# ChenFengYe/motion-latent-diffusion

Measured on NVIDIA H100. Metric: motions/sec @ 50-step DDIM text-to-motion, batch 256, higher is better.
Workload: dtype f16x2-split (fp32-equivalent, fp32 accumulate)

## Files before the change

mld_b200/csrc/debug.cu:

```cuda
#include "engine.h"

#include <string.h>

#include "gemm_tc.h"
#include "misc_kernels.cuh"

extern "C" int mldb_profile_op(mldb_handle* h, const char* op, int32_t B, int32_t S_ctx, int32_t iters,
                               float* avg_ms_out) {
  TRY(check_ready(h, false));
  DeviceGuard guard(h->device);
  if (!op || !avg_ms_out || iters <= 0) FAIL(MLDB_ERR_INVALID, "bad argument");
  const mldb_config& c = h->cfg;
  if (c.num_layers == 0 || c.arch != MLDB_ARCH_TRANS_ENC) FAIL(MLDB_ERR_UNSUPPORTED, "needs the trans_enc denoiser");
  const bool cfg_on = c.guidance_scale > 1.0f;
  Plan* p = nullptr;
  TRY(enc_plan(h, PLAN_REVERSE, B, cfg_on ? 2 * B : B, S_ctx, &p));
  cudaStream_t st = h->cap_stream;
  StackWs& ws = p->ws;
  const EncW& w = h->den.enc[0];
  const int d = ws.d;
  SeqInfo si;
  auto run = [&]() -> int {
    if (!strcmp(op, "qkv")) {
      GemmArgs g; g.a1 = ws.x0; g.K1 = d; g.M = ws.M; g.w = w.in_proj; g.out = ws.qkv; op_gemm(h, g, st);
    } else if (!strcmp(op, "attn")) {
      AttnArgs a; a.q = ws.qkv; a.Lq = ws.L; a.kv = ws.qkv; a.k_col0 = d; a.v_col0 = 2 * d; a.Lk = ws.L;
      a.nseq = ws.nseq; a.heads = c.num_heads; a.hd = d / c.num_heads; a.out = ws.att; op_attn(h, a, st);
    } else if (!strcmp(op, "outproj_ln")) {
      out_proj_ln(h, w.out_proj, w.n1, ws.att, ws.x0, ws.x1, ws.M, d, ws.cf32, st);
    } else if (!strcmp(op, "ffn1")) {
      GemmArgs g; g.a1 = ws.x1; g.K1 = d; g.M = ws.M; g.w = w.l1; g.act = ACT_GELU; g.out = ws.h; op_gemm(h, g, st);
    } else if (!strcmp(op, "ffn2_ln")) {
      GemmArgs g; g.a1 = ws.h; g.K1 = ws.ff; g.M = ws.M; g.w = w.l2;
      LnArgs l; l.res = ws.x1; l.gamma = w.n2.g; l.beta = w.n2.b; l.M = ws.M; l.d = d; l.out = ws.cur[0];
      op_gemm_ln(h, g, l, ws.cf32, st);
    } else if (!strcmp(op, "ffn")) {
      ffn_block(h, w.l1, w.l2, w.n2, ws.x1, ws.cur[0], ws, ACT_GELU, st);
    } else if (!strcmp(op, "tail")) {
      op_tail(h, w.out_proj, w.n1, w.l1, w.l2, w.n2, ws.att, ws.x0, ws.x1, ws.h, ws.cur[0], ws.M, d, ws.ff, ws.cf32, st);
    } else if (!strcmp(op, "tail_fused")) {
      op_tail(h, w.out_proj, w.n1, w.l1, w.l2, w.n2, ws.att, ws.x0, ws.x1, ws.h, ws.cur[0], ws.M, d, ws.ff, ws.cf32, st, 2);
    } else if (!strcmp(op, "layer")) {
      enc_layer(h, h->den, w, ws.x0, ws.cur[0], ws, si, st);
    } else {
      FAIL(MLDB_ERR_INVALID, "unknown op %s", op);
    }
    return MLDB_OK;
  };
  cudaEvent_t e0, e1;
  CK(cudaEventCreate(&e0)); CK(cudaEventCreate(&e1));
  for (int i = 0; i < 3; ++i) TRY(run());
  CK(cudaEventRecord(e0, st));
  for (int i = 0; i < iters; ++i) TRY(run());
  CK(cudaEventRecord(e1, st));
  CK(cudaStreamSynchronize(st));
  float ms = 0.0f;
  CK(cudaEventElapsedTime(&ms, e0, e1));
  cudaEventDestroy(e0); cudaEventDestroy(e1);
  TRY(ops_done(h));
  *avg_ms_out = ms / (float)iters;
  return MLDB_OK;
}

extern "C" int mldb_profile_steps(mldb_handle* h, const void* cond, const float* init_noise, int32_t B, int32_t S_ctx,
                                  float* ms_out) {
  TRY(check_ready(h, true));
  DeviceGuard guard(h->device);
  if (!cond || !init_noise || !ms_out || B <= 0) FAIL(MLDB_ERR_INVALID, "bad argument");
  const mldb_config& c = h->cfg;
  if (c.num_layers == 0 || c.arch != MLDB_ARCH_TRANS_ENC) FAIL(MLDB_ERR_UNSUPPORTED, "needs the trans_enc denoiser");
  if (c.sched_kind != MLDB_SCHED_DDIM) FAIL(MLDB_ERR_UNSUPPORTED, "step profiling is built for the DDIM loop");
  const bool cfg_on = c.guidance_scale > 1.0f;
  Plan* p = nullptr;
  TRY(enc_plan(h, PLAN_REVERSE, B, cfg_on ? 2 * B : B, S_ctx, &p));
  cudaStream_t st = h->cap_stream;
  const int d = c.latent_dim, nsteps = (int)h->timesteps.size();
  const int64_t per = (int64_t)c.n_lat * d;
  TRY(place_condition(h, p, cond, st));
  CK(cudaMemcpyAsync(p->latents, init_noise, (size_t)B * per * sizeof(float), cudaMemcpyDeviceToDevice, st));
  std::vector<cudaEvent_t> ev(nsteps + 1);
  for (auto& e : ev) CK(cudaEventCreate(&e));
  CK(cudaEventRecord(ev[0], st));
  for (int i = 0; i < nsteps; ++i) {
    denoiser_pass(h, p, p->latents, B, h->d_tt + (size_t)i * d, p->eps, st);
    launch_pdl(k_cfg_sched, dim3(nblk(B * per)), dim3(256), 0, st, (const float*)p->eps, p->latents, (const float*)nullptr,
               (int64_t)(B * per), cfg_on ? 1 : 0, c.guidance_scale, (const StepCoef*)h->d_coefs, i, (const int*)nullptr);
    kcount(h, MLDB_KSTAT_MISC);
    CK(cudaEventRecord(ev[i + 1], st));
  }
  CK(cudaStreamSynchronize(st));
  for (int i = 0; i < nsteps; ++i) CK(cudaEventElapsedTime(&ms_out[i], ev[i], ev[i + 1]));
  for (auto& e : ev) cudaEventDestroy(e);
  return ops_done(h);
}

static int debug_exit(mldb_handle* h, size_t n_alloc0, cudaStream_t st, const char* what) {
  cudaError_t e = cudaStreamSynchronize(st);
  if (e == cudaSuccess) e = cudaGetLastError();
  while (h->allocs.size() > n_alloc0) { cudaFree(h->allocs.back()); h->allocs.pop_back(); }
  if (e != cudaSuccess) FAIL(MLDB_ERR_CUDA, "%s: %s", what, cudaGetErrorString(e));
  return check_ops(h);
}

extern "C" int mldb_debug_gemm(mldb_handle* h, const float* A, const float* W, const float* bias,
                               const float* gamma, const float* beta, const float* R, int32_t M, int32_t N,
                               int32_t K, int32_t K1, int32_t act, int32_t use_tc, int32_t split_out, float* out,
                               void* stream) {
  if (!h || !A || !W || !out || M <= 0 || N <= 0 || K <= 0) FAIL(MLDB_ERR_INVALID, "bad argument");
  DeviceGuard guard(h->device);
  cudaStream_t st = (cudaStream_t)stream;
  const size_t n_alloc0 = h->allocs.size();
  LinW w;
  TRY(pack_linear(h, W, N, K, bias, &w));
  if (K1 <= 0 || K1 >= K) K1 = K;
  ActBuf a1, a2{}, res{}, o{};
  TRY(alloc_act(h, M, K1, &a1));
  k_rows_to_split<<<nblk((int64_t)M * K1), 256, 0, st>>>(a1, A, K, M, K1, 1 << 30, 0, 0, 0, nullptr);
  if (K1 < K) {
    TRY(alloc_act(h, M, K - K1, &a2));
    k_rows_to_split<<<nblk((int64_t)M * (K - K1)), 256, 0, st>>>(a2, A + K1, K, M, K - K1, 1 << 30, 0, 0, 0, nullptr);
  }
  float *g = nullptr, *b = nullptr, *cf32 = nullptr;
  const bool saved = h->use_tc;
  h->use_tc = use_tc != 0;
  GemmArgs ga; ga.a1 = a1; ga.K1 = K1; ga.a2 = a2; ga.K2 = K - K1; ga.M = M; ga.w = w; ga.act = act; ga.wide_n = 1;
  if (gamma) {
    TRY(upload_f32(h, gamma, N, &g));
    TRY(upload_f32(h, beta, N, &b));
    TRY(dev_alloc(h, (void**)&cf32, (size_t)M * N * sizeof(float)));
    TRY(alloc_act(h, M, N, &o));
    if (R) {
      TRY(alloc_act(h, M, N, &res));
      k_rows_to_split<<<nblk((int64_t)M * N), 256, 0, st>>>(res, R, N, M, N, 1 << 30, 0, 0, 0, nullptr);
    }
    LnArgs l; l.res = res; l.gamma = g; l.beta = b; l.M = M; l.d = N; l.out = o;
    op_gemm_ln(h, ga, l, cf32, st);
    k_split_to_f32<<<nblk((int64_t)M * N), 256, 0, st>>>(o, out, (int64_t)M * N);
  } else if (R) {
    ga.res_f32 = R; ga.out_f32 = out; ga.ldc = N;
    op_gemm(h, ga, st);
  } else if (split_out && N % 8 == 0) {
    TRY(alloc_act(h, M, N, &o));
    ga.out = o;
    op_gemm(h, ga, st);
    k_split_to_f32<<<nblk((int64_t)M * N), 256, 0, st>>>(o, out, (int64_t)M * N);
  } else {
    ga.out_f32 = out; ga.ldc = N;
    op_gemm(h, ga, st);
  }
  h->use_tc = saved;
  return debug_exit(h, n_alloc0, st, "debug gemm");
}

extern "C" int mldb_debug_ffn(mldb_handle* h, const float* X, const float* W1, const float* b1, const float* W2,
                              const float* b2, const float* gamma, const float* beta, int32_t M, int32_t d,
                              int32_t ff, int32_t mode, float* out, void* stream) {
  if (!h || !X || !W1 || !W2 || !gamma || !beta || !out || M <= 0 || d <= 0 || ff <= 0)
    FAIL(MLDB_ERR_INVALID, "bad argument");
  DeviceGuard guard(h->device);
  cudaStream_t st = (cudaStream_t)stream;
  const size_t n_alloc0 = h->allocs.size();
  LinW l1, l2;
  LnW n;
  TRY(pack_linear(h, W1, ff, d, b1, &l1));
  TRY(pack_linear(h, W2, d, ff, b2, &l2));
  TRY(upload_f32(h, gamma, d, &n.g));
  TRY(upload_f32(h, beta, d, &n.b));
  StackWs ws;
  ws.M = M; ws.d = d; ws.ff = ff;
  ActBuf x, o;
  TRY(alloc_act(h, M, d, &x));
  TRY(alloc_act(h, M, d, &o));
  TRY(alloc_act(h, M, ff, &ws.h));
  TRY(dev_alloc(h, (void**)&ws.cf32, (size_t)M * d * sizeof(float)));
  k_rows_to_split<<<nblk((int64_t)M * d), 256, 0, st>>>(x, X, d, M, d, 1 << 30, 0, 0, 0, nullptr);
  const bool saved = h->use_tc;
  h->use_tc = mode != 0;
  const int saved_fused = tc_set_ffn_fused(h->tc, mode == 2);
  ffn_block(h, l1, l2, n, x, o, ws, ACT_GELU, st);
  h->use_tc = saved;
  tc_set_ffn_fused(h->tc, saved_fused);
  k_split_to_f32<<<nblk((int64_t)M * d), 256, 0, st>>>(o, out, (int64_t)M * d);
  return debug_exit(h, n_alloc0, st, "debug ffn");
}

extern "C" int mldb_debug_tail(mldb_handle* h, const float* att, const float* X, const float* Wo, const float* bo,
                               const float* gamma1, const float* beta1, const float* W1, const float* b1,
                               const float* W2, const float* b2, const float* gamma2, const float* beta2, int32_t M,
                               int32_t d, int32_t ff, int32_t mode, int32_t out_rows, float* out, void* stream) {
  if (!h || !att || !X || !Wo || !gamma1 || !beta1 || !W1 || !W2 || !gamma2 || !beta2 || !out || M <= 0 || d <= 0 ||
      ff <= 0 || out_rows < M)
    FAIL(MLDB_ERR_INVALID, "bad argument");
  DeviceGuard guard(h->device);
  cudaStream_t st = (cudaStream_t)stream;
  const size_t n_alloc0 = h->allocs.size();
  LinW wo, l1, l2;
  LnW n1, n2;
  TRY(pack_linear(h, Wo, d, d, bo, &wo));
  TRY(pack_linear(h, W1, ff, d, b1, &l1));
  TRY(pack_linear(h, W2, d, ff, b2, &l2));
  TRY(upload_f32(h, gamma1, d, &n1.g));
  TRY(upload_f32(h, beta1, d, &n1.b));
  TRY(upload_f32(h, gamma2, d, &n2.g));
  TRY(upload_f32(h, beta2, d, &n2.b));
  ActBuf a, x, x1, hb, o;
  float* cf32 = nullptr;
  TRY(alloc_act(h, M, d, &a));
  TRY(alloc_act(h, M, d, &x));
  TRY(alloc_act(h, M, d, &x1));
  TRY(alloc_act(h, M, ff, &hb));
  TRY(alloc_act(h, out_rows, d, &o));
  TRY(dev_alloc(h, (void**)&cf32, (size_t)M * d * sizeof(float)));
  k_rows_to_split<<<nblk((int64_t)out_rows * d), 256, 0, st>>>(o, out, d, out_rows, d, 1 << 30, 0, 0, 0, nullptr);
  k_rows_to_split<<<nblk((int64_t)M * d), 256, 0, st>>>(a, att, d, M, d, 1 << 30, 0, 0, 0, nullptr);
  k_rows_to_split<<<nblk((int64_t)M * d), 256, 0, st>>>(x, X, d, M, d, 1 << 30, 0, 0, 0, nullptr);
  const bool saved = h->use_tc;
  h->use_tc = mode != 0;
  const int saved_fused = tc_set_ffn_fused(h->tc, 1);
  op_tail(h, wo, n1, l1, l2, n2, a, x, x1, hb, o, M, d, ff, cf32, st, mode == 2 ? 2 : 0);
  h->use_tc = saved;
  tc_set_ffn_fused(h->tc, saved_fused);
  k_split_to_f32<<<nblk((int64_t)out_rows * d), 256, 0, st>>>(o, out, (int64_t)out_rows * d);
  return debug_exit(h, n_alloc0, st, "debug tail");
}

static int debug_attention(mldb_handle* h, const float* Q, const float* KV, const int32_t* lengths, int32_t kv_prefix,
                           int32_t nseq, int32_t Lq, int32_t Lk, int32_t heads, int32_t hd, int32_t mode, int causal,
                           float* out, void* stream) {
  if (!h || !Q || !out || nseq <= 0 || Lq <= 0 || Lk <= 0 || heads <= 0 || hd <= 0) FAIL(MLDB_ERR_INVALID, "bad argument");
  if (!KV && Lq != Lk) FAIL(MLDB_ERR_INVALID, "a packed QKV input is self-attention: Lq must equal Lk");
  if (causal && KV) FAIL(MLDB_ERR_INVALID, "causal attention is self-attention: pass a packed QKV input (KV == NULL)");
  DeviceGuard guard(h->device);
  cudaStream_t st = (cudaStream_t)stream;
  const size_t n_alloc0 = h->allocs.size();
  const int d = heads * hd, Mq = nseq * Lq, Mk = nseq * Lk;
  ActBuf qb, kvb, o;
  TRY(alloc_act(h, Mq, KV ? d : 3 * d, &qb));
  TRY(alloc_act(h, Mq, d, &o));
  rows_to_split(h, qb, Q, qb.cols, Mq, qb.cols, 1 << 30, 0, 0, 0, nullptr, 0, st);
  AttnArgs a; a.q = qb; a.q_col0 = 0; a.Lq = Lq; a.Lk = Lk;
  if (KV) {
    TRY(alloc_act(h, Mk, 2 * d, &kvb));
    rows_to_split(h, kvb, KV, 2 * d, Mk, 2 * d, 1 << 30, 0, 0, 0, nullptr, 0, st);
    a.kv = kvb; a.k_col0 = 0; a.v_col0 = d;
  } else {
    a.kv = qb; a.k_col0 = d; a.v_col0 = 2 * d;
  }
  a.nseq = nseq; a.heads = heads; a.hd = hd; a.lengths = lengths; a.kv_prefix = kv_prefix; a.out = o;
  a.causal = causal;
  int rc = MLDB_OK;
  if (mode == 0 && simt_attention_supported(hd)) { if (!simt_attention(a, st)) rc = MLDB_ERR_UNSUPPORTED; }
  else if (mode == 1 && mma_attention_supported(a)) mma_attention(a, st);
  else if (mode == 2 && tc_attention_supported(a)) { if (!tc_attention(a, h->sm_count, st)) rc = MLDB_ERR_CUDA; }
  else rc = MLDB_ERR_UNSUPPORTED;
  if (rc == MLDB_OK) k_split_to_f32<<<nblk((int64_t)Mq * d), 256, 0, st>>>(o, out, (int64_t)Mq * d);
  TRY(debug_exit(h, n_alloc0, st, "debug attention"));
  if (rc == MLDB_ERR_UNSUPPORTED) FAIL(rc, "attention mode %d does not support this shape", mode);
  return rc;
}
extern "C" int mldb_debug_attention(mldb_handle* h, const float* Q, const float* KV, const int32_t* lengths,
                                    int32_t kv_prefix, int32_t nseq, int32_t Lq, int32_t Lk, int32_t heads, int32_t hd,
                                    int32_t mode, float* out, void* stream) {
  return debug_attention(h, Q, KV, lengths, kv_prefix, nseq, Lq, Lk, heads, hd, mode, 0, out, stream);
}
extern "C" int mldb_debug_attention_causal(mldb_handle* h, const float* Q, const float* KV, const int32_t* lengths,
                                           int32_t kv_prefix, int32_t nseq, int32_t Lq, int32_t Lk, int32_t heads,
                                           int32_t hd, int32_t mode, float* out, void* stream) {
  return debug_attention(h, Q, KV, lengths, kv_prefix, nseq, Lq, Lk, heads, hd, mode, 1, out, stream);
}

static long long* g_timeline = nullptr;
namespace tc { long long* mldb_timeline_buffer() { return g_timeline; } }
extern "C" int mldb_debug_timeline(int32_t enable, int64_t* out, int32_t cap, int32_t* count) {
  constexpr int WARPS = 32, CAPW = 512;
  constexpr size_t BYTES = (size_t)WARPS * CAPW * 2 * sizeof(long long);
  if (enable) {
    if (!g_timeline && cudaMalloc((void**)&g_timeline, BYTES) != cudaSuccess) FAIL(MLDB_ERR_CUDA, "timeline buffer");
    CK(cudaMemset(g_timeline, 0, BYTES));
    return MLDB_OK;
  }
  if (!g_timeline) FAIL(MLDB_ERR_STATE, "no timeline is being recorded");
  if (!out || !count || cap <= 0) FAIL(MLDB_ERR_INVALID, "bad argument");
  CK(cudaDeviceSynchronize());
  std::vector<long long> hbuf((size_t)WARPS * CAPW * 2);
  CK(cudaMemcpy(hbuf.data(), g_timeline, BYTES, cudaMemcpyDeviceToHost));
  int n = 0;
  for (int w = 0; w < WARPS; ++w)
    for (int i = 0; i < CAPW && n < cap; ++i) {
      const long long tag = hbuf[((size_t)w * CAPW + i) * 2], clk = hbuf[((size_t)w * CAPW + i) * 2 + 1];
      if (clk == 0) break;
      out[2 * n] = tag | ((long long)w << 16);
      out[2 * n + 1] = clk;
      ++n;
    }
  *count = n;
  cudaFree(g_timeline);
  g_timeline = nullptr;
  return MLDB_OK;
}
```

mld_b200/csrc/engine.h:

```cpp
#pragma once
#include <cuda_runtime.h>
#include <stdio.h>

#include <functional>
#include <map>
#include <string>
#include <vector>

#include "../../include/mldb.h"
#include "ops.cuh"

#define CK(call)                                                                      \
  do {                                                                                \
    cudaError_t e__ = (call);                                                         \
    if (e__ != cudaSuccess) {                                                         \
      char buf__[512];                                                                \
      snprintf(buf__, sizeof buf__, "%s:%d: %s failed: %s", __FILE__, __LINE__, #call, \
               cudaGetErrorString(e__));                                              \
      mldb_set_err(buf__);                                                            \
      return MLDB_ERR_CUDA;                                                           \
    }                                                                                 \
  } while (0)

#define FAIL(code, ...)                         \
  do {                                          \
    char buf__[512];                            \
    snprintf(buf__, sizeof buf__, __VA_ARGS__); \
    mldb_set_err(buf__);                        \
    return (code);                              \
  } while (0)

#define TRY(expr)                 \
  do {                            \
    int rc__ = (expr);            \
    if (rc__ != MLDB_OK) return rc__; \
  } while (0)

struct DeviceGuard {
  int prev = -1;
  explicit DeviceGuard(int dev) {
    if (cudaGetDevice(&prev) != cudaSuccess) prev = -1;
    if (prev != dev) cudaSetDevice(dev); else prev = -1;
  }
  ~DeviceGuard() { if (prev >= 0) cudaSetDevice(prev); }
  DeviceGuard(const DeviceGuard&) = delete;
  DeviceGuard& operator=(const DeviceGuard&) = delete;
};

inline ActBuf split16_at(void* p, int rows, int cols) {
  const int64_t rp = ((int64_t)rows + 127) / 128 * 128;
  return ActBuf{(__half*)p, rp * cols, rows, cols};
}
inline size_t split16_bytes(int rows, int cols) { return 2 * sizeof(__half) * split16_at(nullptr, rows, cols).plane_stride; }
inline ActBuf rows_of(ActBuf b, int64_t row0, int rows) { b.hi += row0 * b.cols; b.rows = rows; return b; }
inline unsigned nblk(int64_t n, int t = 256) { return (unsigned)((n + t - 1) / t); }

struct GrowBuf {
  void* p = nullptr;
  size_t cap = 0;
  GrowBuf() = default;
  GrowBuf(const GrowBuf&) = delete;
  GrowBuf& operator=(const GrowBuf&) = delete;
  ~GrowBuf() { cudaFree(p); }
};

struct GruState { GrowBuf h_split, h_f32, gh; };

struct LnW { float* g = nullptr; float* b = nullptr; };

struct EncW {
  LinW in_proj, out_proj, l1, l2;
  LnW n1, n2;
  LinW q_only, kv_only;
};
struct DecW {
  LinW sa_in, sa_out, ca_q, ca_kv, ca_v, ca_out, l1, l2;
  LnW n1, n2, n3;
};
enum StackKind { STACK_SKIP_ENC = 0, STACK_SKIP_DEC = 1, STACK_PLAIN_DEC = 2, STACK_PLAIN_ENC = 3 };
struct StackW {
  int kind = STACK_SKIP_ENC;
  int d = 0, ff = 0, heads = 0, layers = 0;
  std::vector<EncW> enc;
  std::vector<DecW> dec;
  std::vector<LinW> skip;
  LnW norm;
};

struct TextLayerW {
  LinW qkv, out, fc1, fc2;
  LnW ln1, ln2;
};
struct TextW {
  bool on = false;
  mldb_text_config cfg{};
  std::vector<TextLayerW> layers;
  LnW final_ln;
  LinW proj;
  float* tok = nullptr;
  float* pos = nullptr;
  GrowBuf x;
  GrowBuf a, qkv, att, h;
  GrowBuf pooled;
};

struct GruW {
  int H = 0;
  LinW w_ih[2];
  LinW w_hh;
  float* b_hh = nullptr;
  float* h0 = nullptr;
  LinW head1, head2;
  LnW ln;
};
struct T2mW {
  bool on = false;
  mldb_t2m_config cfg{};
  LinW pos_emb, text_in;
  LinW conv1, conv2, move_out;
  LinW motion_in;
  GruW text_gru, motion_gru;
  int chunk = 0;
  GrowBuf in;
  GrowBuf f32;
  GrowBuf emb;
  GrowBuf mid;
  GrowBuf words;
  GruState gru;
  GrowBuf head_f32, head_ln;
};

struct A2mLayerW {
  LinW w_ih;
  LinW w_hh;
  float* b_hh = nullptr;
};
struct A2mW {
  bool on = false;
  mldb_a2m_config cfg{};
  std::vector<A2mLayerW> layers;
  float *l1w = nullptr, *l1b = nullptr, *l2w = nullptr, *l2b = nullptr;
  int chunk = 0;
  GrowBuf x;
  GrowBuf gi;
  GrowBuf seq;
  GruState gru;
};

constexpr int kStgcnBlocks = 10;
struct StgcnBlockW {
  LinW gcn;
  float* gcn_tab = nullptr;
  LinW tcn;
};
struct StgcnW {
  bool on = false;
  mldb_stgcn_config cfg{};
  StgcnBlockW blocks[kStgcnBlocks];
  float* adj = nullptr;
  float *bn_scale = nullptr, *bn_shift = nullptr;
  float *fcn_w = nullptr, *fcn_b = nullptr;
  int chunk = 0;
  GrowBuf z;
  GrowBuf y;
  GrowBuf x[2];
  GrowBuf last;
  GrowBuf col, acc;
};

struct RawTensor {
  std::vector<float> host;
  std::vector<int64_t> shape;
  bool loaded = false;
};

struct StackWs {
  int nseq = 0, L = 0, M = 0, d = 0, ff = 0, Lmem = 0;
  ActBuf x0, cur[2], x1, x2, att, qkv, qc, kvm, h, cat;
  int n_sel = 0;
  ActBuf sx, sq, satt, sx1, sh, sout;
  ActBuf vrow;
  float* cvec = nullptr;
  std::vector<ActBuf> ys;
  float* cf32 = nullptr;
};

struct TcCtx;

enum PlanKind {
  PLAN_REVERSE = 0,
  PLAN_VAE_DECODE = 1,
  PLAN_VAE_ENCODE = 2,
  PLAN_DENOISE = 3,
  PLAN_DENOISE_DEC = 4,
  PLAN_REVERSE_DEC = 5,
};

struct Plan {
  int kind = PLAN_REVERSE;
  int B = 0, S = 0, T = 0, Bx = 0, Ntok = 0;
  StackWs ws;
  ActBuf mem;
  float* latents = nullptr;
  float* eps = nullptr;
  float* stage_f32 = nullptr;
  float* tt_single = nullptr;
  float* feats = nullptr;
  ActBuf ctx_split;
  float* cond_f = nullptr;
  size_t cond_cap = 0;
  int64_t* cond_i = nullptr;
  float* noise_in = nullptr;
  float* step_noise = nullptr;
  size_t noise_cap = 0;
  const float* noise_ptr = nullptr;
  int* d_step = nullptr;
  ActBuf in_split;
  int32_t* lengths = nullptr;
  float* joints = nullptr;
  float* joints_all = nullptr;
  cudaGraphExec_t exec = nullptr;
  int64_t graph_nodes = 0;
  int sched_epoch = -1;
};

struct mldb_handle {
  mldb_config cfg;
  int device = 0;
  int sm_count = 0;
  bool finalized = false;
  std::map<std::string, RawTensor> raw;
  std::vector<void*> allocs;
  StackW den;
  StackW vdec, venc;
  LinW time_l1, time_l2, emb_proj, pose_embd, pose_proj, skel_emb, final_layer;
  float* action_emb = nullptr;
  float* query_pe = nullptr;
  float* mem_pe = nullptr;
  float* vae_dec_pe = nullptr;
  int vae_dec_pe_rows = 0;
  float* vae_enc_pe = nullptr;
  int vae_enc_pe_rows = 0;
  float* global_token = nullptr;
  float* mean = nullptr; float* stdv = nullptr; int nstat = 0;
  TextW text;
  T2mW t2m;
  A2mW a2m;
  StgcnW stgcn;
  std::vector<float> alphas_cumprod;
  std::vector<int64_t> timesteps;
  std::vector<StepCoef> coefs_host;
  int64_t* d_timesteps = nullptr;
  StepCoef* d_coefs = nullptr;
  float* d_tt = nullptr;
  float* d_tfeats = nullptr;
  float* d_thid = nullptr;
  int sched_epoch = 0;
  cudaStream_t cap_stream = nullptr;
  std::map<std::string, Plan*> plans;
  int64_t launches = 0;
  int64_t capture_nodes = 0;
  bool capturing = false;
  bool use_tc = true;
  bool use_graph = true;
  int branches = 2;
  int attn_kind = 0;
  int64_t kstat[MLDB_KSTAT_COUNT] = {};
  bool op_failed = false;
  static constexpr int MAX_BRANCHES = 4;
  cudaStream_t br_stream[MAX_BRANCHES - 1] = {};
  float* ffn_scratch[MAX_BRANCHES] = {};
  int* ffn_flags[MAX_BRANCHES] = {};
  cudaEvent_t ev_fork = nullptr, ev_join[MAX_BRANCHES - 1] = {};
  TcCtx* tc = nullptr;
  void* nccl_comm = nullptr;
  bool comm_owned = false;
  int comm_world = 1, comm_rank = 0;
  cudaStream_t comm_stream = nullptr;
  cudaEvent_t ev_local_done = nullptr, ev_gather_done[2] = {};
  int64_t gather_count = 0;
};

struct SeqInfo {
  const int32_t* lengths = nullptr;
  int kv_prefix = 0;
  int len_mod = 0;
};

inline void kcount(mldb_handle* h, int kind) {
  h->kstat[kind]++;
  if (h->capturing) h->capture_nodes++; else h->launches++;
}
int check_ready(mldb_handle* h, bool need_sched);
int check_ops(mldb_handle* h);
inline int ops_done(mldb_handle* h) {
  CK(cudaGetLastError());
  return check_ops(h);
}
int may_configure(const mldb_handle* h, int abi_version, int expected, bool on, const char* name, const char* what);
int check_configured(const mldb_handle* h, bool on, const char* name, const char* what);
int eval_chunk(int option, int B, size_t per_seq, int round);
int dev_alloc(mldb_handle* h, void** p, size_t bytes);
int grow(GrowBuf& b, size_t bytes);
int grow_act(GrowBuf& b, int rows, int cols, ActBuf* out);
int upload_f32(mldb_handle* h, const float* src, size_t n, float** out);
int upload_pe(mldb_handle* h, const std::string& key, float** out, int* rows = nullptr);
const RawTensor& rt(mldb_handle* h, const std::string& k);
void spec_add(mldb_handle* h, const std::string& key, std::vector<int64_t> shape);
void spec_ln(mldb_handle* h, const std::string& p, int d);
int pack_linear(mldb_handle* h, const float* W, int N, int K, const float* bias, LinW* out, int Kpad = 0);
int pack_named(mldb_handle* h, const std::string& wkey, const std::string& bkey, LinW* out, int row0 = 0,
               int nrows = -1, bool pad_k = false);
int pack_ln(mldb_handle* h, const std::string& p, int d, LnW* out);
int time_tokens(mldb_handle* h, const int64_t* d_ts, int64_t t_scalar, int n, const float* pe_row, float* out,
                float* scratch_feats, float* scratch_h, cudaStream_t st);
Plan* find_plan(mldb_handle* h, PlanKind kind, int B, int S, int T);
Plan* add_plan(mldb_handle* h, PlanKind kind, int B, int S, int T);
int run_graphed(mldb_handle* h, Plan* p, cudaStream_t st, const std::function<void(cudaStream_t)>& record);

void op_gemm(mldb_handle* h, const GemmArgs& g, cudaStream_t st);
void op_gemm_ln(mldb_handle* h, GemmArgs g, LnArgs l, float* cf32, cudaStream_t st);
void op_ln(mldb_handle* h, const LnArgs& l, cudaStream_t st);
void op_attn(mldb_handle* h, const AttnArgs& a, cudaStream_t st);
int op_gru(mldb_handle* h, ActBuf x, const LinW* w_ih, const LinW& w_hh, const float* b_hh, const float* h0,
           int64_t h0_ld, const int32_t* lengths, int n, int L, int H, int dirs, GrowBuf& gi, GruState& ws,
           ActBuf seq_out, ActBuf* fin, const float** fin_f32, cudaStream_t st);
void op_tail(mldb_handle* h, const LinW& wo, const LnW& n1, const LinW& l1, const LinW& l2, const LnW& n2, ActBuf att,
             ActBuf x, ActBuf x1, ActBuf hbuf, ActBuf xout, int M, int d, int ff, float* cf32, cudaStream_t st,
             int fuse = 1);
void rows_to_split(mldb_handle* h, ActBuf X, const float* src, int ld_src, int M, int d, int in_group, int out_group,
                   int out_off, int src_bcast, const float* tab, int relu, cudaStream_t st);
int alloc_act(mldb_handle* h, int rows, int cols, ActBuf* out);
int alloc_stack_ws(mldb_handle* h, const StackW& sw, int nseq, int L, int Lmem, StackWs* ws, int n_sel = 0);
StackWs ws_slice(const StackWs& ws, int s0, int n);
void out_proj_ln(mldb_handle* h, const LinW& w, const LnW& n, ActBuf att, ActBuf res, ActBuf xout, int M, int d,
                 float* cf32, cudaStream_t st);
void ffn_block(mldb_handle* h, const LinW& l1, const LinW& l2, const LnW& n, ActBuf xin, ActBuf xout, StackWs& ws,
               int act, cudaStream_t st);
void enc_layer(mldb_handle* h, const StackW& sw, const EncW& w, ActBuf xin, ActBuf xout, StackWs& ws,
               const SeqInfo& si, cudaStream_t st);
ActBuf run_stack(mldb_handle* h, const StackW& sw, ActBuf x0, ActBuf mem, StackWs& ws, const SeqInfo& si,
                 cudaStream_t st);

int enc_plan(mldb_handle* h, PlanKind kind, int B, int Bx, int S, Plan** out);
int place_condition(mldb_handle* h, Plan* p, const void* cond, cudaStream_t st);
void denoiser_pass(mldb_handle* h, Plan* p, const float* latents, int lat_mod, const float* tt, float* eps_out,
                   cudaStream_t st);
int dec_plan(mldb_handle* h, int B, int T, Plan** out);
int run_decode(mldb_handle* h, const float* z, const int32_t* lengths, int B, int T, float* feats_out, cudaStream_t st,
               Plan** plan_out);
int run_f2j(mldb_handle* h, const float* feats, int B, int T, float* joints, cudaStream_t st);
int pack_text(mldb_handle* h);
int pack_t2m(mldb_handle* h);
int pack_a2m(mldb_handle* h);
int pack_stgcn(mldb_handle* h);

void mldb_comm_release(mldb_handle* h);
int mldb_gather_begin(mldb_handle* h, cudaStream_t stream);
int mldb_gather_async(mldb_handle* h, float* global, int64_t count, cudaStream_t stream);
```

mld_b200/csrc/gemm_tc.cu:

```cuda
#include "gemm_tc.h"

#include <algorithm>

#include "tc_common.cuh"

namespace {
using namespace tc;

constexpr int BM = 128, BK = 64;
constexpr int NUM_THREADS = 384;
constexpr int MMA_THREADS = 256;
constexpr int CONSUMER_WARPS = 8;
constexpr int MAX_N = 1024;
constexpr int MAX_N_WIDE = 4096;

struct TcParams {
  int M, N, kblocks, kb1;
  int m_tiles, n_tiles;
  float inv_scale;
  const float* bias;
  const float* addtab;
  int act;
  __half* out_hi; __half* out_lo; int ld_out, out_col0;
  float* out_f32; int ldc;
  const float* res_f32;
  int in_group, out_group, out_off;
  const int32_t* zero_lengths;
  const __half* res_hi; const __half* res_lo; int ld_res;
  const float* gamma; const float* beta;
  long long* tl;
};

enum { EPI_FAST = 0, EPI_LN = 1, EPI_GENERIC = 2, EPI_RES = 3, EPI_F32 = 4 };

template <int BN>
struct TileCfg {
  static constexpr int A_BYTES = BM * BK * 2;
  static constexpr int W_BYTES = BN * BK * 2;
  static constexpr int STAGE_BYTES = 2 * A_BYTES + 2 * W_BYTES;
  static constexpr int STAGES = BN == 256 ? 2 : 3;
  static constexpr int SMEM_BYTES = STAGES * STAGE_BYTES + 256 + 1024;
  static_assert(SMEM_BYTES <= 232448, "shared memory budget");
};

__device__ __forceinline__ void store_split2(__half* hi, __half* lo, int64_t o, float x0, float x1) {
  uint32_t h, l;
  split2(x0, x1, h, l);
  *reinterpret_cast<uint32_t*>(hi + o) = h;
  *reinterpret_cast<uint32_t*>(lo + o) = l;
}

template <int ACT, int N>
__device__ __forceinline__ void fast_group(const float (&d)[N], int j, float sc, float2 b, float (&x)[4]) {
  x[0] = fmaf(d[4 * j], sc, b.x); x[1] = fmaf(d[4 * j + 1], sc, b.y);
  x[2] = fmaf(d[4 * j + 2], sc, b.x); x[3] = fmaf(d[4 * j + 3], sc, b.y);
#pragma unroll
  for (int e = 0; e < 4; ++e) {
    if (ACT == ACT_GELU) x[e] = gelu_fast(x[e]);
    if (ACT == ACT_QUICKGELU) x[e] = quick_gelu_f(x[e]);
    if (ACT == ACT_LEAKY) x[e] = apply_act(x[e], ACT_LEAKY);
  }
}

__device__ __forceinline__ void quad_transpose(uint32_t (&v)[4], int l) {
  const bool b2 = l & 2, b1 = l & 1;
  uint32_t r0 = __shfl_xor_sync(0xffffffffu, b2 ? v[0] : v[2], 2), r1 = __shfl_xor_sync(0xffffffffu, b2 ? v[1] : v[3], 2);
  if (b2) { v[0] = r0; v[1] = r1; } else { v[2] = r0; v[3] = r1; }
  r0 = __shfl_xor_sync(0xffffffffu, b1 ? v[0] : v[1], 1); r1 = __shfl_xor_sync(0xffffffffu, b1 ? v[2] : v[3], 1);
  if (b1) { v[0] = r0; v[2] = r1; } else { v[1] = r0; v[3] = r1; }
}

template <class Load>
__device__ __forceinline__ void ring_produce(int& q_next, int total, int need, const uint64_t* bar_empty, int stages,
                                             Load&& load) {
  while (q_next < total) {
    const uint32_t bar = smem_u32(&bar_empty[q_next % stages]), par = (((uint32_t)(q_next / stages)) & 1u) ^ 1u;
    if (q_next <= need) mbar_wait(bar, par);
    else if (!__shfl_sync(0xffffffffu, (int)mbar_test(bar, par), 0)) break;
    load(q_next++);
  }
}

template <class Res, class Out>
__device__ __forceinline__ void ln_rows(float (&d)[128], float sc, const float* bias, const float* gamma,
                                        const float* beta, int cp, Res&& res, Out&& out) {
  float s0 = 0.0f, s1 = 0.0f;
#pragma unroll
  for (int j = 0; j < 32; ++j) {
    const int n = 8 * j + cp;
    const float2 b = bias ? __ldg(reinterpret_cast<const float2*>(bias + n)) : make_float2(0.0f, 0.0f);
    float x[4] = {fmaf(d[4 * j], sc, b.x), fmaf(d[4 * j + 1], sc, b.y), fmaf(d[4 * j + 2], sc, b.x),
                  fmaf(d[4 * j + 3], sc, b.y)};
    res(j, x);
    d[4 * j] = x[0]; d[4 * j + 1] = x[1]; d[4 * j + 2] = x[2]; d[4 * j + 3] = x[3];
    s0 += x[0] + x[1]; s1 += x[2] + x[3];
  }
  const float mean0 = quad_sum(s0) * (1.0f / 256), mean1 = quad_sum(s1) * (1.0f / 256);
  float q0 = 0.0f, q1 = 0.0f;
#pragma unroll
  for (int j = 0; j < 32; ++j) {
    const float a0 = d[4 * j] - mean0, a1 = d[4 * j + 1] - mean0, a2 = d[4 * j + 2] - mean1, a3 = d[4 * j + 3] - mean1;
    d[4 * j] = a0; d[4 * j + 1] = a1; d[4 * j + 2] = a2; d[4 * j + 3] = a3;
    q0 = fmaf(a0, a0, fmaf(a1, a1, q0));
    q1 = fmaf(a2, a2, fmaf(a3, a3, q1));
  }
  const float rstd0 = rsqrtf(quad_sum(q0) * (1.0f / 256) + 1e-5f), rstd1 = rsqrtf(quad_sum(q1) * (1.0f / 256) + 1e-5f);
#pragma unroll
  for (int j = 0; j < 32; ++j) {
    const int n = 8 * j + cp;
    const float2 g = __ldg(reinterpret_cast<const float2*>(gamma + n)), be = __ldg(reinterpret_cast<const float2*>(beta + n));
    const float y[4] = {fmaf(d[4 * j] * rstd0, g.x, be.x), fmaf(d[4 * j + 1] * rstd0, g.y, be.y),
                        fmaf(d[4 * j + 2] * rstd1, g.x, be.x), fmaf(d[4 * j + 3] * rstd1, g.y, be.y)};
    out(j, y);
  }
}

__device__ __forceinline__ void ln_epilogue(float (&d)[128], float sc, const float* bias, const __half* res_hi,
                                            const __half* res_lo, int ld_res, const float* gamma, const float* beta,
                                            __half* out_hi, __half* out_lo, int ld_out, int r_lo, int M, int cp) {
  const bool ok0 = r_lo < M, ok1 = r_lo + 8 < M;
  ln_rows(d, sc, bias, gamma, beta, cp,
          [&](int j, float (&x)[4]) {
            if (!res_hi) return;
            const int n = 8 * j + cp;
            if (ok0) {
              const int64_t o = (int64_t)r_lo * ld_res + n;
              const float2 h = __half22float2(*reinterpret_cast<const __half2*>(res_hi + o));
              const float2 l = __half22float2(*reinterpret_cast<const __half2*>(res_lo + o));
              x[0] = (x[0] + h.x) + l.x; x[1] = (x[1] + h.y) + l.y;
            }
            if (ok1) {
              const int64_t o = (int64_t)(r_lo + 8) * ld_res + n;
              const float2 h = __half22float2(*reinterpret_cast<const __half2*>(res_hi + o));
              const float2 l = __half22float2(*reinterpret_cast<const __half2*>(res_lo + o));
              x[2] = (x[2] + h.x) + l.x; x[3] = (x[3] + h.y) + l.y;
            }
          },
          [&](int j, const float (&y)[4]) {
            const int n = 8 * j + cp;
            if (ok0) store_split2(out_hi, out_lo, (int64_t)r_lo * ld_out + n, y[0], y[1]);
            if (ok1) store_split2(out_hi, out_lo, (int64_t)(r_lo + 8) * ld_out + n, y[2], y[3]);
          });
}

__device__ __forceinline__ void ln_tile(float (&d)[128], float sc, const float* bias, const float* gamma,
                                        const float* beta, uint8_t* tile, int rl, int lane, int cp) {
  uint8_t* const row0 = tile + rl * 128 + cp * 2;
  const int sw = lane >> 2;
  auto at = [&](int j, int h, int plane) {
    return reinterpret_cast<__half2*>(row0 + plane * 65536 + h * 1024 + (j >> 3) * 16384 + (((j & 7) ^ sw) << 4));
  };
  ln_rows(d, sc, bias, gamma, beta, cp,
          [&](int j, float (&x)[4]) {
#pragma unroll
            for (int h = 0; h < 2; ++h) {
              const float2 hi = __half22float2(*at(j, h, 0)), lo = __half22float2(*at(j, h, 1));
              x[2 * h] = (x[2 * h] + hi.x) + lo.x; x[2 * h + 1] = (x[2 * h + 1] + hi.y) + lo.y;
            }
          },
          [&](int j, const float (&y)[4]) {
#pragma unroll
            for (int h = 0; h < 2; ++h) {
              uint32_t hi, lo;
              split2(y[2 * h], y[2 * h + 1], hi, lo);
              *reinterpret_cast<uint32_t*>(at(j, h, 0)) = hi;
              *reinterpret_cast<uint32_t*>(at(j, h, 1)) = lo;
            }
          });
}

template <int BN, int EPI, int ACT = ACT_NONE>
__global__ void __launch_bounds__(NUM_THREADS, 1)
k_gemm_tc(const __grid_constant__ CUtensorMap tmA1h, const __grid_constant__ CUtensorMap tmA1l,
          const __grid_constant__ CUtensorMap tmA2h, const __grid_constant__ CUtensorMap tmA2l,
          const __grid_constant__ CUtensorMap tmWh, const __grid_constant__ CUtensorMap tmWl, const TcParams p) {
  static_assert(EPI != EPI_LN || BN == 256, "the LayerNorm epilogue covers a full 256-wide row");
  using Cfg = TileCfg<BN>;
  constexpr int STAGES = Cfg::STAGES;
  extern __shared__ uint8_t smem_raw[];
  uint8_t* smem = smem_raw + smem_pad1024(smem_raw);
  uint64_t* bar_full = reinterpret_cast<uint64_t*>(smem + STAGES * Cfg::STAGE_BYTES);
  uint64_t* bar_empty = bar_full + STAGES;

  const int warp = __shfl_sync(0xffffffffu, (int)(threadIdx.x >> 5), 0), lane = threadIdx.x & 31;
  int tl_n = 0;
  tl_event(p.tl, tl_n, 40);
  const int ntiles = p.m_tiles * p.n_tiles;
  const int nlocal = (ntiles - (int)blockIdx.x + (int)gridDim.x - 1) / (int)gridDim.x;
  auto decode = [&](int j, int& m0, int& n0) {
    const int t = (int)blockIdx.x + j * (int)gridDim.x;
    m0 = (t / p.n_tiles) * BM;
    n0 = (t % p.n_tiles) * BN;
  };

  if (threadIdx.x == 0) {
    for (int s = 0; s < STAGES; ++s) {
      mbar_init(smem_u32(&bar_full[s]), 1);
      mbar_init(smem_u32(&bar_empty[s]), CONSUMER_WARPS);
    }
    asm volatile("fence.mbarrier_init.release.cluster;" ::: "memory");
    tma_prefetch_desc(&tmA1h); tma_prefetch_desc(&tmA1l); tma_prefetch_desc(&tmWh); tma_prefetch_desc(&tmWl);
  }
  pdl_trigger();
  __syncthreads();
  pdl_wait();
  tl_event(p.tl, tl_n, 41);

  if (warp < 4) {
    reg_dec<40>();
    if (warp != 0) return;
    int kbg = 0;
    for (int j = 0; j < nlocal; ++j) {
      int m0, n0;
      decode(j, m0, n0);
      tl_event(p.tl, tl_n, 1, j);
      for (int kb = 0; kb < p.kblocks; ++kb, ++kbg) {
        const int s = kbg % STAGES;
        mbar_wait(smem_u32(&bar_empty[s]), (((uint32_t)(kbg / STAGES)) & 1u) ^ 1u);
        if (elect_one()) {
          if (kb == 0 && j + 1 < nlocal) {
            int m1, n1;
            decode(j + 1, m1, n1);
            if (m1 != m0) {
              for (int k2 = 0; k2 < p.kblocks; ++k2) {
                if (k2 < p.kb1) { tma_prefetch_2d(&tmA1h, k2 * BK, m1); tma_prefetch_2d(&tmA1l, k2 * BK, m1); }
                else { tma_prefetch_2d(&tmA2h, (k2 - p.kb1) * BK, m1); tma_prefetch_2d(&tmA2l, (k2 - p.kb1) * BK, m1); }
              }
            }
          }
          const uint32_t full = smem_u32(&bar_full[s]);
          mbar_expect_tx(full, Cfg::STAGE_BYTES);
          const uint32_t sAh = smem_u32(smem + s * Cfg::STAGE_BYTES), sAl = sAh + Cfg::A_BYTES;
          const uint32_t sWh = sAl + Cfg::A_BYTES, sWl = sWh + Cfg::W_BYTES;
          if (kb < p.kb1) {
            tma_load_2d(sAh, &tmA1h, full, kb * BK, m0);
            tma_load_2d(sAl, &tmA1l, full, kb * BK, m0);
          } else {
            tma_load_2d(sAh, &tmA2h, full, (kb - p.kb1) * BK, m0);
            tma_load_2d(sAl, &tmA2l, full, (kb - p.kb1) * BK, m0);
          }
          tma_load_2d(sWh, &tmWh, full, kb * BK, n0);
          tma_load_2d(sWl, &tmWl, full, kb * BK, n0);
        }
        __syncwarp();
      }
    }
    return;
  }
  reg_inc<232>();
  const int cw = (warp >> 2) - 1;
  const int cp = 2 * (lane & 3);
  float d[BN / 2];
  int kbg = 0;
  for (int it = 0; it < nlocal; ++it) {
    int m0, n0;
    decode(it, m0, n0);
    tl_event(p.tl, tl_n, 2, it);
    for (int kb = 0; kb < p.kblocks; ++kb, ++kbg) {
      const int s = kbg % STAGES;
      mbar_wait(smem_u32(&bar_full[s]), ((uint32_t)(kbg / STAGES)) & 1u);
      const uint32_t sAh = smem_u32(smem + s * Cfg::STAGE_BYTES) + cw * (64 * 128), sAl = sAh + Cfg::A_BYTES;
      const uint32_t sWh = smem_u32(smem + s * Cfg::STAGE_BYTES) + 2 * Cfg::A_BYTES, sWl = sWh + Cfg::W_BYTES;
      wg_fence();
      kblock_ss<BN>(d, sAh, sAl, sWh, sWl, kb == 0);
      wg_commit();
      if (kb > 0) {
        wg_wait<1>();
        if (lane == 0) mbar_arrive(smem_u32(&bar_empty[(kbg - 1) % STAGES]));
      }
    }
    wg_wait<0>();
    acc_fence(d);
    if (lane == 0) mbar_arrive(smem_u32(&bar_empty[(kbg - 1) % STAGES]));
    tl_event(p.tl, tl_n, 4, it);

    const int r_lo = m0 + cw * 64 + (warp & 3) * 16 + (lane >> 2);
    if constexpr (EPI == EPI_LN) {
      ln_epilogue(d, p.inv_scale, p.bias, p.res_hi, p.res_lo, p.ld_res, p.gamma, p.beta, p.out_hi, p.out_lo, p.ld_out,
                  r_lo, p.M, cp);
    } else if constexpr (EPI == EPI_FAST) {
      const bool ok0 = r_lo < p.M, ok1 = r_lo + 8 < p.M;
      const int64_t o0 = (int64_t)r_lo * p.ld_out + p.out_col0 + n0 + cp, o1 = o0 + (int64_t)8 * p.ld_out;
#pragma unroll
      for (int j = 0; j < BN / 8; ++j) {
        float x[4];
        fast_group<ACT>(d, j, p.inv_scale, __ldg(reinterpret_cast<const float2*>(p.bias + n0 + 8 * j + cp)), x);
        if (ok0) store_split2(p.out_hi, p.out_lo, o0 + 8 * j, x[0], x[1]);
        if (ok1) store_split2(p.out_hi, p.out_lo, o1 + 8 * j, x[2], x[3]);
      }
    } else if constexpr (EPI == EPI_RES) {
      const float sc = p.inv_scale;
#pragma unroll
      for (int j = 0; j < BN / 8; ++j) {
        const int n = n0 + 8 * j + cp;
        if (n >= p.N) continue;
        const float2 b = p.bias ? __ldg(reinterpret_cast<const float2*>(p.bias + n)) : make_float2(0.0f, 0.0f);
#pragma unroll
        for (int h = 0; h < 2; ++h) {
          if (r_lo + 8 * h >= p.M) continue;
          const int64_t o = (int64_t)(r_lo + 8 * h) * p.ldc + n;
          const float2 r = *reinterpret_cast<const float2*>(p.res_f32 + o);
          *reinterpret_cast<float2*>(p.out_f32 + o) =
              make_float2(fmaf(d[4 * j + 2 * h], sc, b.x) + r.x, fmaf(d[4 * j + 2 * h + 1], sc, b.y) + r.y);
        }
      }
    } else if constexpr (EPI == EPI_F32) {
      const float sc = p.inv_scale;
#pragma unroll
      for (int j = 0; j < BN / 8; ++j) {
        const int n = n0 + 8 * j + cp;
        if (n >= p.N) continue;
        const float2 b = p.bias ? __ldg(reinterpret_cast<const float2*>(p.bias + n)) : make_float2(0.0f, 0.0f);
#pragma unroll
        for (int h = 0; h < 2; ++h) {
          if (r_lo + 8 * h >= p.M) continue;
          const float x0 = apply_act(fmaf(d[4 * j + 2 * h], sc, b.x), ACT), x1 = apply_act(fmaf(d[4 * j + 2 * h + 1], sc, b.y), ACT);
          *reinterpret_cast<float2*>(p.out_f32 + (int64_t)(r_lo + 8 * h) * p.ldc + n) = make_float2(x0, x1);
        }
      }
    } else {
#pragma unroll
      for (int h = 0; h < 2; ++h) {
        const int m = r_lo + 8 * h;
        if (m >= p.M) continue;
        int seq = 0, pos = m;
        if (p.in_group < p.M) { seq = m / p.in_group; pos = m - seq * p.in_group; }
        const int64_t orow = (int64_t)seq * p.out_group + p.out_off + pos;
        const bool zero = p.zero_lengths != nullptr && pos >= p.zero_lengths[seq];
        const float* tab = p.addtab ? p.addtab + (int64_t)(p.out_off + pos) * p.N : nullptr;
#pragma unroll
        for (int j = 0; j < BN / 8; ++j) {
#pragma unroll
          for (int e = 0; e < 2; ++e) {
            const int n = n0 + 8 * j + cp + e;
            if (n >= p.N) continue;
            float x = d[4 * j + 2 * h + e] * p.inv_scale + (p.bias ? p.bias[n] : 0.0f);
            if (tab) x += tab[n];
            x = zero ? 0.0f : apply_act(x, p.act);
            if (p.out_hi) {
              __half hh, ll;
              split_f32(x, hh, ll);
              const int64_t o = orow * p.ld_out + p.out_col0 + n;
              p.out_hi[o] = hh; p.out_lo[o] = ll;
            }
            if (p.out_f32) p.out_f32[orow * p.ldc + n] = x;
          }
        }
      }
    }
    tl_event(p.tl, tl_n, 5, it);
  }
  tl_event(p.tl, tl_n, 42);
}

struct FfnParams {
  int M, m_tiles, n_chunks;
  int full, left, parts;
  float* scratch;
  int* flags;
  int reverse;
  int prefix;
  long long* tl;
  float inv_s0, inv_s1, inv_s2;
  const float* b0; const float* gamma1; const float* beta1;
  const float* b1; const float* b2; const float* gamma; const float* beta;
};
struct FfnCfg {
  static constexpr int CHUNK = 64;
  static constexpr int X_BYTES = 2 * 4 * BM * 128;
  static constexpr int STAGE_BYTES = 32768, STAGES = 3;
  static constexpr int SMEM_BYTES = X_BYTES + STAGES * STAGE_BYTES + 256 + 1024;
  static_assert(SMEM_BYTES <= 232448, "shared memory budget");
};

__global__ void __launch_bounds__(MMA_THREADS, 1)
k_ffn_tc(const __grid_constant__ CUtensorMap tmXh, const __grid_constant__ CUtensorMap tmXl,
         const __grid_constant__ CUtensorMap tmW1h, const __grid_constant__ CUtensorMap tmW1l,
         const __grid_constant__ CUtensorMap tmW2h, const __grid_constant__ CUtensorMap tmW2l,
         const __grid_constant__ CUtensorMap tmAh, const __grid_constant__ CUtensorMap tmAl,
         const __grid_constant__ CUtensorMap tmWoh, const __grid_constant__ CUtensorMap tmWol,
         const __grid_constant__ CUtensorMap tmYh, const __grid_constant__ CUtensorMap tmYl, const FfnParams p) {
  using Cfg = FfnCfg;
  constexpr int STAGES = Cfg::STAGES;
  extern __shared__ uint8_t smem_raw[];
  uint8_t* smem = smem_raw + smem_pad1024(smem_raw);
  uint8_t* ring = smem + Cfg::X_BYTES;
  uint64_t* bar_full = reinterpret_cast<uint64_t*>(ring + STAGES * Cfg::STAGE_BYTES);
  uint64_t* bar_empty = bar_full + STAGES;
  uint64_t* bar_xfull = bar_empty + STAGES;
  uint64_t* bar_xempty = bar_xfull + 4;

  const int warp = __shfl_sync(0xffffffffu, (int)(threadIdx.x >> 5), 0), lane = threadIdx.x & 31;
  int tl_n = 0;
  tl_event(p.tl, tl_n, 40);
  const int ncta = (int)gridDim.x, cid = (int)blockIdx.x;
  const int NC = p.n_chunks;
  struct Item { int mt, c0, c1, mode, piece0; };
  auto rev = [&](int t) { return p.reverse ? p.m_tiles - 1 - t : t; };
  const int nlocal = p.full + (cid < p.left * p.parts ? 1 : 0);
  auto item = [&](int j) -> Item {
    if (j < p.full) return Item{rev(cid + j * ncta), 0, NC, 0, 0};
    const int t = cid / p.parts, part = cid - t * p.parts;
    const int c0 = (part * NC + p.parts - 1) / p.parts, c1 = ((part + 1) * NC + p.parts - 1) / p.parts;
    const int slot0 = t * (p.parts - 1);
    return Item{rev(p.full * ncta + t), c0, c1, p.parts == 1 ? 0 : (part == p.parts - 1 ? 2 : 1),
                p.parts == 1 ? 0 : slot0 + (part == p.parts - 1 ? 0 : part)};
  };
  const int PRE = p.prefix ? 8 : 0;
  const int per_tile = PRE + 4 * NC;
  int total = p.full * per_tile;
  if (nlocal > p.full) {
    const Item it = item(p.full);
    total += PRE + 4 * (it.c1 - it.c0);
  }
  const int XG = p.prefix ? 2 : 1;
  const int xtotal = nlocal * 4 * XG;

  if (threadIdx.x == 0) {
    for (int s = 0; s < STAGES; ++s) {
      mbar_init(smem_u32(&bar_full[s]), 1);
      mbar_init(smem_u32(&bar_empty[s]), CONSUMER_WARPS);
    }
    for (int kb = 0; kb < 4; ++kb) {
      mbar_init(smem_u32(&bar_xfull[kb]), 1);
      mbar_init(smem_u32(&bar_xempty[kb]), CONSUMER_WARPS);
    }
    asm volatile("fence.mbarrier_init.release.cluster;" ::: "memory");
    tma_prefetch_desc(&tmXh); tma_prefetch_desc(&tmXl); tma_prefetch_desc(&tmW1h);
    tma_prefetch_desc(&tmW1l); tma_prefetch_desc(&tmW2h); tma_prefetch_desc(&tmW2l);
    tma_prefetch_desc(&tmYh); tma_prefetch_desc(&tmYl);
    if (p.prefix) { tma_prefetch_desc(&tmAh); tma_prefetch_desc(&tmAl); tma_prefetch_desc(&tmWoh); tma_prefetch_desc(&tmWol); }
  }
  pdl_trigger();
  __syncthreads();
  pdl_wait();
  tl_event(p.tl, tl_n, 41);

  int q_next = 0, x_next = 0;
  auto load_slot = [&](int q) {
    const int j = min(q / per_tile, p.full);
    const Item it = item(j);
    const int r = q - j * per_tile;
    if (elect_one()) {
      const uint32_t full = smem_u32(&bar_full[q % STAGES]);
      const uint32_t dst = smem_u32(ring + (q % STAGES) * Cfg::STAGE_BYTES);
      mbar_expect_tx(full, Cfg::STAGE_BYTES);
      if (r < PRE) {
        tma_load_2d(dst, (r & 1) ? &tmWol : &tmWoh, full, (r >> 1) * BK, 0);
      } else {
        const int c = it.c0 + ((r - PRE) >> 2), k = (r - PRE) & 3;
        if (k < 2) {
          for (int kk = 0; kk < 2; ++kk) {
            tma_load_2d(dst + kk * 8192, &tmW1h, full, (2 * k + kk) * BK, c * Cfg::CHUNK);
            tma_load_2d(dst + 16384 + kk * 8192, &tmW1l, full, (2 * k + kk) * BK, c * Cfg::CHUNK);
          }
        } else {
          tma_load_2d(dst, k == 3 ? &tmW2l : &tmW2h, full, c * Cfg::CHUNK, 0);
        }
      }
    }
    __syncwarp();
  };
  auto load_x = [&](int v) {
    if (elect_one()) {
      const int j = v / (4 * XG), kb = v & 3;
      const bool att = p.prefix && (v >> 2) == j * XG;
      const int m0 = item(j).mt * BM;
      const uint32_t full = smem_u32(&bar_xfull[kb]);
      mbar_expect_tx(full, 2 * BM * 128);
      tma_load_2d(smem_u32(smem + kb * 16384), att ? &tmAh : &tmXh, full, kb * BK, m0);
      tma_load_2d(smem_u32(smem + 65536 + kb * 16384), att ? &tmAl : &tmXl, full, kb * BK, m0);
      if (att && kb == 0)
        for (int k2 = 0; k2 < 4; ++k2) { tma_prefetch_2d(&tmXh, k2 * BK, m0); tma_prefetch_2d(&tmXl, k2 * BK, m0); }
      if (v % (4 * XG) == 0 && j + 1 < nlocal) {
        const int m1 = item(j + 1).mt * BM;
        for (int k2 = 0; k2 < 4; ++k2) {
          tma_prefetch_2d(&tmXh, k2 * BK, m1); tma_prefetch_2d(&tmXl, k2 * BK, m1);
          if (p.prefix) { tma_prefetch_2d(&tmAh, k2 * BK, m1); tma_prefetch_2d(&tmAl, k2 * BK, m1); }
        }
      }
    }
    __syncwarp();
  };
  auto produce = [&](int need, int need_x) {
    ring_produce(x_next, xtotal, need_x, bar_xempty, 4, load_x);
    ring_produce(q_next, total, need, bar_empty, STAGES, load_slot);
  };

  const int cw = warp >> 2;
  const int cp = 2 * (lane & 3);
  const int rl = cw * 64 + (warp & 3) * 16 + (lane >> 2);
  const uint32_t sX = smem_u32(smem) + cw * (64 * 128);
  float acc2[128];
  float acc1[32];
  uint32_t hh[4][4], hl[4][4];
  int rc = 0;
  auto slot_full = [&](int r) { mbar_wait(smem_u32(&bar_full[r % STAGES]), ((uint32_t)(r / STAGES)) & 1u); };
  auto slot_free = [&](int r) { if (lane == 0) mbar_arrive(smem_u32(&bar_empty[r % STAGES])); };
  auto x_full = [&](int kb, uint32_t par) { mbar_wait(smem_u32(&bar_xfull[kb]), par); };
  auto x_free = [&](int kb) { if (lane == 0) mbar_arrive(smem_u32(&bar_xempty[kb])); };
  for (int j = 0; j < nlocal; ++j) {
    const Item it = item(j);
    const int m0 = it.mt * BM;
    const uint32_t xpar = (uint32_t)(j * XG) & 1u;
    if (warp == 0) produce(-1, 4 * j * XG + 3);
    if (p.prefix) {
#pragma unroll
      for (int kb = 0; kb < 4; ++kb) {
        if (warp == 0) produce(rc + 1, -1);
        x_full(kb, xpar);
        slot_full(rc); slot_full(rc + 1);
        const uint32_t wh = smem_u32(ring + (rc % STAGES) * Cfg::STAGE_BYTES);
        const uint32_t wl = smem_u32(ring + ((rc + 1) % STAGES) * Cfg::STAGE_BYTES);
        wg_fence();
        kblock_ss<256>(acc2, sX + kb * 16384, sX + 65536 + kb * 16384, wh, wl, kb == 0);
        wg_commit();
        wg_wait<0>();
        slot_free(rc); slot_free(rc + 1); x_free(kb);
        rc += 2;
        if (warp == 0) produce(-1, -1);
        tl_event(p.tl, tl_n, 60, kb);
      }
      acc_fence(acc2);
      if (warp == 0) produce(-1, 4 * j * XG + 7);
#pragma unroll
      for (int kb = 0; kb < 4; ++kb) x_full(kb, xpar ^ 1u);
      ln_tile(acc2, p.inv_s0, p.b0, p.gamma1, p.beta1, smem, rl, lane, cp);
      fence_async_smem();
      named_bar_sync(2 + cw, 128);
      tl_event(p.tl, tl_n, 61, j);
    } else {
#pragma unroll
      for (int kb = 0; kb < 4; ++kb) x_full(kb, xpar);
    }
    tl_event(p.tl, tl_n, 2, j);
    int pend = -1;
    for (int c = it.c0; c < it.c1; ++c) {
#pragma unroll
      for (int half = 0; half < 2; ++half) {
        if (warp == 0) produce(rc + half, -1);
        slot_full(rc + half);
        tl_event(p.tl, tl_n, 10 + half, c);
        const uint32_t w = smem_u32(ring + ((rc + half) % STAGES) * Cfg::STAGE_BYTES);
        wg_fence();
#pragma unroll
        for (int k = 0; k < 2; ++k) {
          const uint32_t xh = sX + (2 * half + k) * 16384;
          kblock_ss<64>(acc1, xh, xh + 65536, w + k * 8192, w + 16384 + k * 8192, half == 0 && k == 0);
        }
        wg_commit();
      }
      wg_wait<0>();
      acc_fence(acc1);
      tl_event(p.tl, tl_n, 13, c);
      if (pend >= 0) slot_free(pend);
      slot_free(rc); slot_free(rc + 1);
      rc += 2;
      if (c == it.c1 - 1 && it.mode == 1)
        for (int kb = 0; kb < 4; ++kb) x_free(kb);
      if (warp == 0) produce(-1, -1);
#pragma unroll
      for (int ks = 0; ks < 4; ++ks) {
#pragma unroll
        for (int g = 0; g < 2; ++g) {
          const int jj = 2 * ks + g, n = c * Cfg::CHUNK + 8 * jj + cp;
          const float2 b = p.b1 ? __ldg(reinterpret_cast<const float2*>(p.b1 + n)) : make_float2(0.0f, 0.0f);
          split2(gelu_fast(fmaf(acc1[4 * jj], p.inv_s1, b.x)), gelu_fast(fmaf(acc1[4 * jj + 1], p.inv_s1, b.y)),
                 hh[ks][2 * g], hl[ks][2 * g]);
          split2(gelu_fast(fmaf(acc1[4 * jj + 2], p.inv_s1, b.x)), gelu_fast(fmaf(acc1[4 * jj + 3], p.inv_s1, b.y)),
                 hh[ks][2 * g + 1], hl[ks][2 * g + 1]);
        }
      }
      tl_event(p.tl, tl_n, 14, c);
      if (warp == 0) produce(rc, -1);
      slot_full(rc);
      tl_event(p.tl, tl_n, 12, c);
      wg_fence();
      {
        const uint64_t wd = make_desc(smem_u32(ring + (rc % STAGES) * Cfg::STAGE_BYTES));
#pragma unroll
        for (int ks = 0; ks < 4; ++ks) {
          wgmma_rs_n256(acc2, hl[ks], wd + 2 * ks, (c == it.c0 && ks == 0) ? 0u : 1u);
          wgmma_rs_n256(acc2, hh[ks], wd + 2 * ks, 1u);
        }
      }
      wg_commit();
      if (warp == 0) produce(rc + 1, -1);
      slot_full(rc + 1);
      {
        const uint64_t wd = make_desc(smem_u32(ring + ((rc + 1) % STAGES) * Cfg::STAGE_BYTES));
#pragma unroll
        for (int ks = 0; ks < 4; ++ks) wgmma_rs_n256(acc2, hh[ks], wd + 2 * ks, 1u);
      }
      wg_commit();
      wg_wait<1>();
      slot_free(rc);
      pend = rc + 1;
      rc += 2;
      if (warp == 0) produce(-1, -1);
    }
    wg_wait<0>();
    acc_fence(acc2);
    if (pend >= 0) slot_free(pend);
    if (warp == 0) produce(-1, -1);
    tl_event(p.tl, tl_n, 4, j);
    if (it.mode == 1) {
      float* const dst = p.scratch + (size_t)it.piece0 * (BM * 256);
#pragma unroll
      for (int jj = 0; jj < 32; ++jj) {
        *reinterpret_cast<float2*>(dst + rl * 256 + 8 * jj + cp) = make_float2(acc2[4 * jj], acc2[4 * jj + 1]);
        *reinterpret_cast<float2*>(dst + (rl + 8) * 256 + 8 * jj + cp) = make_float2(acc2[4 * jj + 2], acc2[4 * jj + 3]);
      }
      __threadfence();
      named_bar_sync(1, MMA_THREADS);
      if (threadIdx.x == 0) asm volatile("st.release.gpu.global.u32 [%0], %1;" ::"l"(p.flags + it.piece0), "r"(1) : "memory");
      continue;
    }
    const int nparts = it.mode == 2 ? p.parts - 1 : 0;
    if (nparts > 0) {
      if (lane == 0) {
        for (int pp = 0; pp < nparts; ++pp) {
          const int* f = p.flags + it.piece0 + pp;
          uint32_t v = 0;
          long long t_end = clock64() + 4000000000ll;
          do {
            asm volatile("ld.acquire.gpu.global.u32 %0, [%1];" : "=r"(v) : "l"(f) : "memory");
            if (v == 0 && clock64() > t_end) __trap();
          } while (v == 0);
        }
      }
      __syncwarp();
      for (int pp = 0; pp < nparts; ++pp) {
        const float* src = p.scratch + (size_t)(it.piece0 + pp) * (BM * 256);
#pragma unroll
        for (int jj = 0; jj < 32; ++jj) {
          const float2 a = __ldcg(reinterpret_cast<const float2*>(src + rl * 256 + 8 * jj + cp));
          const float2 b = __ldcg(reinterpret_cast<const float2*>(src + (rl + 8) * 256 + 8 * jj + cp));
          acc2[4 * jj] += a.x; acc2[4 * jj + 1] += a.y; acc2[4 * jj + 2] += b.x; acc2[4 * jj + 3] += b.y;
        }
      }
      named_bar_sync(1, MMA_THREADS);
      if (threadIdx.x == 0)
        for (int pp = 0; pp < nparts; ++pp) p.flags[it.piece0 + pp] = 0;
    }
    ln_tile(acc2, p.inv_s2, p.b2, p.gamma, p.beta, smem, rl, lane, cp);
    fence_async_smem();
    named_bar_sync(2 + cw, 128);
    tl_event(p.tl, tl_n, 62, j);
    if ((warp & 3) == 0) {
      if (elect_one()) {
        if (m0 + cw * 64 < p.M) {
#pragma unroll
          for (int kb = 0; kb < 4; ++kb) {
            const uint32_t src = smem_u32(smem + kb * 16384 + cw * 8192);
            tma_store_2d(&tmYh, src, kb * BK, m0 + cw * 64);
            tma_store_2d(&tmYl, src + 65536, kb * BK, m0 + cw * 64);
          }
          bulk_commit();
          bulk_wait_read<0>();
        }
#pragma unroll
        for (int kb = 0; kb < 4; ++kb) mbar_arrive_cnt(smem_u32(&bar_xempty[kb]), 4);
      }
      __syncwarp();
      tl_event(p.tl, tl_n, 63, j);
    }
  }
  tl_event(p.tl, tl_n, 42);
}

struct ProjParams {
  int M, n_chunks, items;
  float inv_scale;
  const float* bias;
  __half* out_hi; __half* out_lo; int ld_out, out_col0;
  long long* tl;
};
struct ProjCfg {
  static constexpr int CHUNK = 128;
  static constexpr int A_BYTES = 2 * 4 * BM * 128;
  static constexpr int STAGE_BYTES = 2 * CHUNK * 128, STAGES = 3;
  static constexpr int SMEM_BYTES = A_BYTES + STAGES * STAGE_BYTES + 256 + 1024;
  static_assert(SMEM_BYTES <= 232448, "shared memory budget");
};

template <int ACT>
__global__ void __launch_bounds__(MMA_THREADS, 1)
k_proj_tc(const __grid_constant__ CUtensorMap tmAh, const __grid_constant__ CUtensorMap tmAl,
          const __grid_constant__ CUtensorMap tmWh, const __grid_constant__ CUtensorMap tmWl, const ProjParams p) {
  using Cfg = ProjCfg;
  constexpr int STAGES = Cfg::STAGES;
  extern __shared__ uint8_t smem_raw[];
  uint8_t* smem = smem_raw + smem_pad1024(smem_raw);
  uint8_t* ring = smem + Cfg::A_BYTES;
  uint64_t* bar_full = reinterpret_cast<uint64_t*>(ring + STAGES * Cfg::STAGE_BYTES);
  uint64_t* bar_empty = bar_full + STAGES;
  uint64_t* bar_afull = bar_empty + STAGES;
  uint64_t* bar_aempty = bar_afull + 4;

  const int warp = __shfl_sync(0xffffffffu, (int)(threadIdx.x >> 5), 0), lane = threadIdx.x & 31;
  int tl_n = 0;
  tl_event(p.tl, tl_n, 40);
  const int NC = p.n_chunks;
  const int t0 = (int)((long long)blockIdx.x * p.items / gridDim.x);
  const int n = (int)((long long)(blockIdx.x + 1) * p.items / gridDim.x) - t0;
  const int mt0 = t0 / NC, ntiles = (t0 + n - 1) / NC - mt0 + 1;
  auto tile_of = [&](int i) { return (t0 + i) / NC - mt0; };
  auto first_of_tile = [&](int i) { return i == 0 || (t0 + i) % NC == 0; };
  auto last_of_tile = [&](int i) { return i == n - 1 || (t0 + i + 1) % NC == 0; };

  if (threadIdx.x == 0) {
    for (int s = 0; s < STAGES; ++s) {
      mbar_init(smem_u32(&bar_full[s]), 1);
      mbar_init(smem_u32(&bar_empty[s]), CONSUMER_WARPS);
    }
    for (int k = 0; k < 4; ++k) {
      mbar_init(smem_u32(&bar_afull[k]), 1);
      mbar_init(smem_u32(&bar_aempty[k]), CONSUMER_WARPS);
    }
    asm volatile("fence.mbarrier_init.release.cluster;" ::: "memory");
    tma_prefetch_desc(&tmAh); tma_prefetch_desc(&tmAl); tma_prefetch_desc(&tmWh); tma_prefetch_desc(&tmWl);
  }
  pdl_trigger();
  __syncthreads();
  pdl_wait();
  tl_event(p.tl, tl_n, 41);

  int q_next = 0, a_next = 0;
  auto load_w = [&](int q) {
    if (elect_one()) {
      const int c = (t0 + (q >> 2)) % NC, k = q & 3;
      const uint32_t full = smem_u32(&bar_full[q % STAGES]);
      const uint32_t dst = smem_u32(ring + (q % STAGES) * Cfg::STAGE_BYTES);
      mbar_expect_tx(full, Cfg::STAGE_BYTES);
      tma_load_2d(dst, &tmWh, full, k * BK, c * Cfg::CHUNK);
      tma_load_2d(dst + Cfg::STAGE_BYTES / 2, &tmWl, full, k * BK, c * Cfg::CHUNK);
    }
    __syncwarp();
  };
  auto load_a = [&](int a) {
    if (elect_one()) {
      const int j = a >> 2, k = a & 3, m0 = (mt0 + j) * BM;
      const uint32_t full = smem_u32(&bar_afull[k]);
      mbar_expect_tx(full, 2 * BM * 128);
      tma_load_2d(smem_u32(smem + k * 16384), &tmAh, full, k * BK, m0);
      tma_load_2d(smem_u32(smem + 65536 + k * 16384), &tmAl, full, k * BK, m0);
      if (k == 0 && j + 1 < ntiles)
        for (int k2 = 0; k2 < 4; ++k2) { tma_prefetch_2d(&tmAh, k2 * BK, m0 + BM); tma_prefetch_2d(&tmAl, k2 * BK, m0 + BM); }
    }
    __syncwarp();
  };
  auto produce = [&](int need_w, int need_a) {
    ring_produce(a_next, 4 * ntiles, need_a, bar_aempty, 4, load_a);
    ring_produce(q_next, 4 * n, need_w, bar_empty, STAGES, load_w);
  };

  const int cw = warp >> 2;
  const int cp = 2 * (lane & 3);
  const uint32_t sA = smem_u32(smem) + cw * (64 * 128);
  float acc0[64], acc1[64];
  auto retire = [&](int q) {
    if (lane == 0) {
      mbar_arrive(smem_u32(&bar_empty[q % STAGES]));
      if (last_of_tile(q >> 2)) mbar_arrive(smem_u32(&bar_aempty[q & 3]));
    }
  };
  auto epilogue = [&](const float (&d)[64], int i) {
    const int t = t0 + i, r_lo = (t / NC) * BM + cw * 64 + (warp & 3) * 16 + (lane >> 2), n0 = (t % NC) * Cfg::CHUNK;
    const int l = lane & 3;
    const bool ok0 = r_lo < p.M, ok1 = r_lo + 8 < p.M;
    const int64_t o0 = (int64_t)r_lo * p.ld_out + p.out_col0 + n0 + 8 * l, o1 = o0 + (int64_t)8 * p.ld_out;
    tl_event(p.tl, tl_n, 52, i);
#pragma unroll
    for (int jb = 0; jb < Cfg::CHUNK / 32; ++jb) {
      uint32_t h0[4], l0[4], h1[4], l1[4];
#pragma unroll
      for (int g = 0; g < 4; ++g) {
        const int j = 4 * jb + g;
        float x[4];
        fast_group<ACT>(d, j, p.inv_scale, __ldg(reinterpret_cast<const float2*>(p.bias + n0 + 8 * j + cp)), x);
        split2(x[0], x[1], h0[g], l0[g]);
        split2(x[2], x[3], h1[g], l1[g]);
      }
      quad_transpose(h0, l); quad_transpose(l0, l); quad_transpose(h1, l); quad_transpose(l1, l);
      if (ok0) {
        *reinterpret_cast<uint4*>(p.out_hi + o0 + 32 * jb) = make_uint4(h0[0], h0[1], h0[2], h0[3]);
        *reinterpret_cast<uint4*>(p.out_lo + o0 + 32 * jb) = make_uint4(l0[0], l0[1], l0[2], l0[3]);
      }
      if (ok1) {
        *reinterpret_cast<uint4*>(p.out_hi + o1 + 32 * jb) = make_uint4(h1[0], h1[1], h1[2], h1[3]);
        *reinterpret_cast<uint4*>(p.out_lo + o1 + 32 * jb) = make_uint4(l1[0], l1[1], l1[2], l1[3]);
      }
    }
    tl_event(p.tl, tl_n, 53, i);
  };
  auto step = [&](int i, float (&cur)[64], float (&prev)[64]) {
    const bool fresh = first_of_tile(i);
    const int j = tile_of(i);
    tl_event(p.tl, tl_n, 50, i);
#pragma unroll
    for (int k = 0; k < 4; ++k) {
      const int q = 4 * i + k;
      if (warp == 0) produce(q, fresh ? 4 * j + k : -1);
      if (fresh) {
        mbar_wait(smem_u32(&bar_afull[k]), (uint32_t)j & 1u);
        if (k == 0) tl_event(p.tl, tl_n, 51, j);
      }
      mbar_wait(smem_u32(&bar_full[q % STAGES]), ((uint32_t)(q / STAGES)) & 1u);
      const uint32_t w = smem_u32(ring + (q % STAGES) * Cfg::STAGE_BYTES), a = sA + k * 16384;
      wg_fence();
      kblock_ss<128>(cur, a, a + 65536, w, w + Cfg::STAGE_BYTES / 2, k == 0);
      wg_commit();
      if (k == 2) {
        if (warp == 0) produce(q + 1, -1);
        if (i > 0) epilogue(prev, i - 1);
      }
      if (q > 0) {
        wg_wait<1>();
        retire(q - 1);
      }
      if (k == 0 && i > 0) acc_fence(prev);
    }
  };
  for (int i = 0; i < n; i += 2) {
    step(i, acc0, acc1);
    if (i + 1 < n) step(i + 1, acc1, acc0);
  }
  wg_wait<0>();
  retire(4 * n - 1);
  if ((n - 1) & 1) {
    acc_fence(acc1);
    epilogue(acc1, n - 1);
  } else {
    acc_fence(acc0);
    epilogue(acc0, n - 1);
  }
  tl_event(p.tl, tl_n, 42);
}

}

struct TcCtx {
  int device = 0;
  int sm_count = 132;
  int ffn_fused = 1;
  int ffn_split = 1;
};

TcCtx* tc_create(int device) {
  if (!tc::tmap_encoder()) return nullptr;
  TcCtx* c = new TcCtx();
  c->device = device;
  cudaDeviceGetAttribute(&c->sm_count, cudaDevAttrMultiProcessorCount, device);
  bool ok = true;
  auto opt_in = [&](auto kernel, int bytes) { ok = ok && smem_opt_in(kernel, bytes, "k_gemm_tc"); };
  opt_in(k_gemm_tc<256, EPI_FAST>, TileCfg<256>::SMEM_BYTES); opt_in(k_gemm_tc<128, EPI_FAST>, TileCfg<128>::SMEM_BYTES);
  opt_in(k_gemm_tc<256, EPI_FAST, ACT_GELU>, TileCfg<256>::SMEM_BYTES); opt_in(k_gemm_tc<128, EPI_FAST, ACT_GELU>, TileCfg<128>::SMEM_BYTES);
  opt_in(k_gemm_tc<256, EPI_GENERIC>, TileCfg<256>::SMEM_BYTES); opt_in(k_gemm_tc<128, EPI_GENERIC>, TileCfg<128>::SMEM_BYTES);
  opt_in(k_gemm_tc<256, EPI_FAST, ACT_QUICKGELU>, TileCfg<256>::SMEM_BYTES);
  opt_in(k_gemm_tc<128, EPI_FAST, ACT_QUICKGELU>, TileCfg<128>::SMEM_BYTES);
  opt_in(k_gemm_tc<256, EPI_RES>, TileCfg<256>::SMEM_BYTES); opt_in(k_gemm_tc<128, EPI_RES>, TileCfg<128>::SMEM_BYTES);
  opt_in(k_gemm_tc<256, EPI_LN>, TileCfg<256>::SMEM_BYTES);
  opt_in(k_gemm_tc<256, EPI_FAST, ACT_LEAKY>, TileCfg<256>::SMEM_BYTES); opt_in(k_gemm_tc<128, EPI_FAST, ACT_LEAKY>, TileCfg<128>::SMEM_BYTES);
  opt_in(k_gemm_tc<256, EPI_F32>, TileCfg<256>::SMEM_BYTES); opt_in(k_gemm_tc<128, EPI_F32>, TileCfg<128>::SMEM_BYTES);
  opt_in(k_gemm_tc<256, EPI_F32, ACT_LEAKY>, TileCfg<256>::SMEM_BYTES); opt_in(k_gemm_tc<128, EPI_F32, ACT_LEAKY>, TileCfg<128>::SMEM_BYTES);
  opt_in(k_ffn_tc, FfnCfg::SMEM_BYTES);
  opt_in(k_proj_tc<ACT_NONE>, ProjCfg::SMEM_BYTES); opt_in(k_proj_tc<ACT_GELU>, ProjCfg::SMEM_BYTES);
  opt_in(k_proj_tc<ACT_QUICKGELU>, ProjCfg::SMEM_BYTES); opt_in(k_proj_tc<ACT_LEAKY>, ProjCfg::SMEM_BYTES);
  if (!ok) {
    delete c;
    return nullptr;
  }
  return c;
}
void tc_destroy(TcCtx* c) { delete c; }

static int pick_bn(const GemmArgs& g) { return (g.w.N % 256 == 0) ? 256 : 128; }

bool tc_gemm_supported(const TcCtx* c, const GemmArgs& g) {
  if (!c) return false;
  if (g.a_kind != A_SPLIT || g.M < 1 || g.w.N > (g.wide_n ? MAX_N_WIDE : MAX_N)) return false;
  if (g.K1 <= 0 || g.K1 % BK || g.K2 % BK || g.a1.cols != g.K1) return false;
  if (g.K2 > 0 && g.a2.cols != g.K2) return false;
  if (g.w.K != g.K1 + g.K2) return false;
  if (((uintptr_t)g.a1.hi & 15) || ((uintptr_t)g.w.w & 15)) return false;
  if (g.out.hi && ((g.out.cols % 8) || (g.out_col0 % 8))) return false;
  if (g.res_f32 && (!g.out_f32 || g.out.hi || g.act != ACT_NONE || g.addtab || g.zero_lengths || g.in_group < g.M ||
                    g.out_group != 0 || g.out_off != 0 || (g.w.N % 2) || (g.ldc % 2) || ((uintptr_t)g.out_f32 & 7) ||
                    ((uintptr_t)g.res_f32 & 7)))
    return false;
  return true;
}

bool tc_gemm_ln_supported(const TcCtx* c, const GemmArgs& g, const LnArgs& l) {
  if (!tc_gemm_supported(c, g)) return false;
  if (g.w.N != 256 || l.d != 256 || g.act != ACT_NONE) return false;
  if (l.in_group != 0 || l.c != nullptr || l.out_f32 != nullptr || !l.out.hi) return false;
  if (l.out.cols != 256 || (l.res.hi && l.res.cols != 256)) return false;
  if (l.gamma2 || l.rowvec) return false;
  if (g.addtab || g.zero_lengths || g.in_group < g.M || g.out_group != 0 || g.out_off != 0) return false;
  return true;
}

static void fill_params(const GemmArgs& g, const LnArgs* ln, int bn, TcParams* out) {
  TcParams p{};
  p.M = g.M; p.N = g.w.N; p.kblocks = g.w.K / BK; p.kb1 = g.K1 / BK;
  p.inv_scale = g.w.inv_scale; p.bias = g.w.bias; p.addtab = g.addtab; p.act = g.act;
  p.in_group = g.in_group; p.out_group = g.out_group; p.out_off = g.out_off; p.zero_lengths = g.zero_lengths;
  if (ln) {
    p.out_hi = ln->out.hi; p.out_lo = ln->out.lo(); p.ld_out = ln->out.cols; p.out_col0 = 0;
    p.res_hi = ln->res.hi; p.res_lo = ln->res.hi ? ln->res.lo() : nullptr; p.ld_res = ln->res.cols;
    p.gamma = ln->gamma; p.beta = ln->beta;
  } else {
    p.out_hi = g.out.hi; p.out_lo = g.out.hi ? g.out.lo() : nullptr; p.ld_out = g.out.cols; p.out_col0 = g.out_col0;
    p.out_f32 = g.out_f32; p.ldc = g.ldc; p.res_f32 = g.res_f32;
  }
  p.m_tiles = (g.M + BM - 1) / BM;
  p.n_tiles = (g.w.N + bn - 1) / bn;
  p.tl = tc::mldb_timeline_buffer();
  *out = p;
}

static bool tc_proj(TcCtx* c, const GemmArgs& g, cudaStream_t st) {
  CUtensorMap mAh, mAl, mWh, mWl;
  const bool ok = make_map(&mAh, g.a1.hi, g.M, g.K1, BM) && make_map(&mAl, g.a1.lo(), g.M, g.K1, BM) &&
                  make_map(&mWh, g.w.w, g.w.N, g.w.K, ProjCfg::CHUNK) &&
                  make_map(&mWl, g.w.w + g.w.plane_stride, g.w.N, g.w.K, ProjCfg::CHUNK);
  if (!ok) return false;
  ProjParams p{};
  p.M = g.M; p.n_chunks = g.w.N / ProjCfg::CHUNK; p.items = (g.M + BM - 1) / BM * p.n_chunks;
  p.inv_scale = g.w.inv_scale; p.bias = g.w.bias;
  p.out_hi = g.out.hi; p.out_lo = g.out.lo(); p.ld_out = g.out.cols; p.out_col0 = g.out_col0;
  p.tl = tc::mldb_timeline_buffer();
  const dim3 grid(p.items < c->sm_count ? p.items : c->sm_count);
  switch (g.act) {
    case ACT_GELU: launch_pdl(k_proj_tc<ACT_GELU>, grid, dim3(MMA_THREADS), ProjCfg::SMEM_BYTES, st, mAh, mAl, mWh, mWl, p); break;
    case ACT_QUICKGELU: launch_pdl(k_proj_tc<ACT_QUICKGELU>, grid, dim3(MMA_THREADS), ProjCfg::SMEM_BYTES, st, mAh, mAl, mWh, mWl, p); break;
    case ACT_LEAKY: launch_pdl(k_proj_tc<ACT_LEAKY>, grid, dim3(MMA_THREADS), ProjCfg::SMEM_BYTES, st, mAh, mAl, mWh, mWl, p); break;
    default: launch_pdl(k_proj_tc<ACT_NONE>, grid, dim3(MMA_THREADS), ProjCfg::SMEM_BYTES, st, mAh, mAl, mWh, mWl, p); break;
  }
  return true;
}

bool tc_gemm(TcCtx* c, const GemmArgs& g, const LnArgs* ln, cudaStream_t st) {
  const int bn = ln ? 256 : pick_bn(g);
  const bool fast = !ln && g.out.hi && !g.out_f32 && !g.addtab && !g.zero_lengths && g.in_group >= g.M &&
                    g.out_group == 0 && g.out_off == 0 && g.w.N % bn == 0 && g.w.bias != nullptr &&
                    (g.act == ACT_NONE || g.act == ACT_GELU || g.act == ACT_QUICKGELU || g.act == ACT_LEAKY);
  if (fast && g.K1 == 256 && g.K2 == 0 && ((uintptr_t)g.out.hi & 15) == 0 && ((uintptr_t)g.out.lo() & 15) == 0)
    return tc_proj(c, g, st);
  CUtensorMap mA1h, mA1l, mA2h, mA2l, mWh, mWl;
  bool ok = make_map(&mA1h, g.a1.hi, g.M, g.K1, BM) && make_map(&mA1l, g.a1.lo(), g.M, g.K1, BM);
  if (g.K2 > 0) ok = ok && make_map(&mA2h, g.a2.hi, g.M, g.K2, BM) && make_map(&mA2l, g.a2.lo(), g.M, g.K2, BM);
  else { mA2h = mA1h; mA2l = mA1l; }
  ok = ok && make_map(&mWh, g.w.w, g.w.N, g.w.K, bn) && make_map(&mWl, g.w.w + g.w.plane_stride, g.w.N, g.w.K, bn);
  if (!ok) return false;
  TcParams p;
  fill_params(g, ln, bn, &p);
  const bool f32 = !ln && g.vec_f32 && !g.out.hi && g.out_f32 && !g.res_f32 && !g.addtab && !g.zero_lengths &&
                   g.in_group >= g.M && g.out_group == 0 && g.out_off == 0 && g.w.N % 2 == 0 && g.ldc % 2 == 0 &&
                   ((uintptr_t)g.out_f32 & 7) == 0 && (g.act == ACT_NONE || g.act == ACT_LEAKY);
  const int ntiles = p.m_tiles * p.n_tiles;
  dim3 grid(ntiles < c->sm_count ? ntiles : c->sm_count);
#define MLDB_LAUNCH(BN_, ...)                                                                                      \
  launch_pdl(k_gemm_tc<BN_, __VA_ARGS__>, grid, dim3(NUM_THREADS), TileCfg<BN_>::SMEM_BYTES, st, mA1h, mA1l, mA2h, \
             mA2l, mWh, mWl, p)
#define MLDB_LAUNCH_SHAPE(...)                                                       \
  do {                                                                               \
    if (bn == 256) MLDB_LAUNCH(256, __VA_ARGS__); else MLDB_LAUNCH(128, __VA_ARGS__); \
  } while (0)
  if (ln)                             MLDB_LAUNCH(256, EPI_LN);
  else if (g.res_f32)                 MLDB_LAUNCH_SHAPE(EPI_RES);
  else if (fast && g.act == ACT_GELU) MLDB_LAUNCH_SHAPE(EPI_FAST, ACT_GELU);
  else if (fast && g.act == ACT_QUICKGELU) MLDB_LAUNCH_SHAPE(EPI_FAST, ACT_QUICKGELU);
  else if (fast && g.act == ACT_LEAKY) MLDB_LAUNCH_SHAPE(EPI_FAST, ACT_LEAKY);
  else if (f32 && g.act == ACT_LEAKY) MLDB_LAUNCH_SHAPE(EPI_F32, ACT_LEAKY);
  else if (f32)                       MLDB_LAUNCH_SHAPE(EPI_F32);
  else if (fast)                      MLDB_LAUNCH_SHAPE(EPI_FAST);
  else                                MLDB_LAUNCH_SHAPE(EPI_GENERIC);
#undef MLDB_LAUNCH_SHAPE
#undef MLDB_LAUNCH
  return true;
}

int tc_set_ffn_split(TcCtx* c, int on) {
  if (!c) return 0;
  const int old = c->ffn_split;
  c->ffn_split = on;
  return old;
}
int tc_set_ffn_fused(TcCtx* c, int on) {
  if (!c) return 0;
  const int old = c->ffn_fused;
  c->ffn_fused = on;
  return old;
}
static bool planes_aligned16(const ActBuf& b) { return ((uintptr_t)b.hi & 15) == 0 && ((uintptr_t)b.lo() & 15) == 0; }

bool tc_ffn_supported(const TcCtx* c, const GemmArgs& g1, const GemmArgs& g2, const LnArgs& l2) {
  if (!c || !c->ffn_fused) return false;
  if (!tc_gemm_supported(c, g1) || !tc_gemm_ln_supported(c, g2, l2)) return false;
  if (g1.K1 != 256 || g1.K2 > 0 || g2.K2 > 0 || g1.M != g2.M) return false;
  if (g1.w.N % FfnCfg::CHUNK || g1.w.N > MAX_N || g1.w.N != g2.K1) return false;
  if (g1.act != ACT_GELU || g1.out_f32 || g1.addtab || g1.zero_lengths) return false;
  if (g1.in_group < g1.M || g1.out_group != 0 || g1.out_off != 0) return false;
  if (l2.res.hi != g1.a1.hi || l2.res.plane_stride != g1.a1.plane_stride) return false;
  if (!planes_aligned16(g1.a1) || !planes_aligned16(l2.out)) return false;
  return true;
}
bool tc_tail_supported(const TcCtx* c, const GemmArgs& go, const LnArgs& l1, const GemmArgs& g1, const GemmArgs& g2,
                       const LnArgs& l2) {
  if (!tc_gemm_ln_supported(c, go, l1) || !tc_ffn_supported(c, g1, g2, l2)) return false;
  if (go.K1 != 256 || go.K2 > 0 || go.M != g1.M || !l1.res.hi) return false;
  if (g1.a1.hi != l1.out.hi || g1.a1.plane_stride != l1.out.plane_stride) return false;
  return planes_aligned16(go.a1) && planes_aligned16(l1.res);
}

static bool launch_ffn(TcCtx* c, const GemmArgs* go, const LnArgs* l1, const GemmArgs& g1, const GemmArgs& g2,
                       const LnArgs& l2, float* scratch, int* flags, cudaStream_t st) {
  CUtensorMap mXh, mXl, mW1h, mW1l, mW2h, mW2l, mAh, mAl, mWoh, mWol, mYh, mYl;
  const int M = g1.M, m_tiles = (M + BM - 1) / BM;
  const ActBuf x = go ? l1->res : g1.a1;
  bool ok = make_map(&mXh, x.hi, M, 256, BM) && make_map(&mXl, x.lo(), M, 256, BM) &&
            make_map(&mW1h, g1.w.w, g1.w.N, g1.w.K, FfnCfg::CHUNK) &&
            make_map(&mW1l, g1.w.w + g1.w.plane_stride, g1.w.N, g1.w.K, FfnCfg::CHUNK) &&
            make_map(&mW2h, g2.w.w, g2.w.N, g2.w.K, 256) &&
            make_map(&mW2l, g2.w.w + g2.w.plane_stride, g2.w.N, g2.w.K, 256) &&
            make_map(&mYh, l2.out.hi, M, 256, 64) && make_map(&mYl, l2.out.lo(), M, 256, 64);
  if (go) {
    ok = ok && make_map(&mAh, go->a1.hi, M, 256, BM) && make_map(&mAl, go->a1.lo(), M, 256, BM) &&
         make_map(&mWoh, go->w.w, go->w.N, go->w.K, 256) && make_map(&mWol, go->w.w + go->w.plane_stride, go->w.N, go->w.K, 256);
  } else {
    mAh = mXh; mAl = mXl; mWoh = mW2h; mWol = mW2l;
  }
  if (!ok) return false;
  FfnParams p{};
  p.M = M; p.m_tiles = m_tiles; p.n_chunks = g1.w.N / FfnCfg::CHUNK;
  p.tl = tc::mldb_timeline_buffer();
  p.prefix = go ? 1 : 0;
  if (go) { p.inv_s0 = go->w.inv_scale; p.b0 = go->w.bias; p.gamma1 = l1->gamma; p.beta1 = l1->beta; }
  p.inv_s1 = g1.w.inv_scale; p.inv_s2 = g2.w.inv_scale;
  p.b1 = g1.w.bias; p.b2 = g2.w.bias; p.gamma = l2.gamma; p.beta = l2.beta;
  const int ncta_max = c->sm_count;
  p.full = m_tiles / ncta_max; p.left = m_tiles % ncta_max; p.parts = 1;
  p.scratch = scratch; p.flags = flags;
  if (p.left > 0 && scratch && flags && c->ffn_split) {
    const int parts = std::min(p.n_chunks, ncta_max / p.left);
    if (parts >= 2 && (size_t)p.left * (parts - 1) * (BM * 256 * 4) <= TC_FFN_SCRATCH_BYTES) p.parts = parts;
  }
  const int ncta = p.full > 0 ? ncta_max : p.left * p.parts;
  p.reverse = tc::snake_order();
  launch_pdl(k_ffn_tc, dim3(ncta), dim3(MMA_THREADS), FfnCfg::SMEM_BYTES, st, mXh, mXl, mW1h, mW1l, mW2h, mW2l, mAh,
             mAl, mWoh, mWol, mYh, mYl, p);
  return true;
}
bool tc_ffn(TcCtx* c, const GemmArgs& g1, const GemmArgs& g2, const LnArgs& l2, float* scratch, int* flags, cudaStream_t st) {
  return launch_ffn(c, nullptr, nullptr, g1, g2, l2, scratch, flags, st);
}
bool tc_tail(TcCtx* c, const GemmArgs& go, const LnArgs& l1, const GemmArgs& g1, const GemmArgs& g2, const LnArgs& l2,
             float* scratch, int* flags, cudaStream_t st) {
  return launch_ffn(c, &go, &l1, g1, g2, l2, scratch, flags, st);
}
```

mld_b200/csrc/gemm_tc.h:

```cpp
#pragma once
#include "ops.cuh"

struct TcCtx;
TcCtx* tc_create(int device);
void tc_destroy(TcCtx* c);
bool tc_gemm_supported(const TcCtx* c, const GemmArgs& g);
bool tc_gemm_ln_supported(const TcCtx* c, const GemmArgs& g, const LnArgs& l);
bool tc_gemm(TcCtx* c, const GemmArgs& g, const LnArgs* ln, cudaStream_t st);
bool tc_ffn_supported(const TcCtx* c, const GemmArgs& g1, const GemmArgs& g2, const LnArgs& l2);
constexpr size_t TC_FFN_SCRATCH_BYTES = (size_t)160 * 128 * 256 * 4, TC_FFN_FLAG_BYTES = 160 * 4;
bool tc_ffn(TcCtx* c, const GemmArgs& g1, const GemmArgs& g2, const LnArgs& l2, float* scratch, int* flags, cudaStream_t st);
bool tc_tail_supported(const TcCtx* c, const GemmArgs& go, const LnArgs& l1, const GemmArgs& g1, const GemmArgs& g2,
                       const LnArgs& l2);
bool tc_tail(TcCtx* c, const GemmArgs& go, const LnArgs& l1, const GemmArgs& g1, const GemmArgs& g2, const LnArgs& l2,
             float* scratch, int* flags, cudaStream_t st);
int tc_set_ffn_split(TcCtx* c, int on);
int tc_set_ffn_fused(TcCtx* c, int on);
```

mld_b200/csrc/ops.cuh:

```cuda
#pragma once
#include "common.cuh"

struct LinW {
  __half* w = nullptr;
  int64_t plane_stride = 0;
  float* bias = nullptr;
  int N = 0, K = 0;
  float inv_scale = 1.0f;
  int id = -1;
};

enum AKind { A_SPLIT = 0, A_F32 = 1, A_F32_RELU = 2 };

struct GemmArgs {
  int a_kind = A_SPLIT;
  ActBuf a1{}; int K1 = 0;
  ActBuf a2{}; int K2 = 0;
  const float* a_f32 = nullptr; int lda = 0;
  int M = 0;
  LinW w{};
  int act = ACT_NONE;
  ActBuf out{};
  int out_col0 = 0;
  float* out_f32 = nullptr; int ldc = 0;
  int in_group = 1 << 30, out_group = 0, out_off = 0;
  const float* addtab = nullptr;
  const int32_t* zero_lengths = nullptr;
  const float* res_f32 = nullptr;
  int wide_n = 0;
  int vec_f32 = 0;
};

struct LnArgs {
  const float* c = nullptr; int ldc = 0;
  ActBuf res{};
  const float* rowvec = nullptr; int rv_group = 1;
  const float* gamma = nullptr; const float* beta = nullptr;
  const float* gamma2 = nullptr; const float* beta2 = nullptr;
  int M = 0, d = 0;
  int sel_group = 1 << 30, in_group = 0;
  ActBuf out{}; float* out_f32 = nullptr; int ld_out = 0;
  int act = ACT_NONE;
};

struct AttnArgs {
  ActBuf q{}; int q_col0 = 0; int Lq = 0;
  ActBuf kv{}; int k_col0 = 0, v_col0 = 0; int Lk = 0;
  int nseq = 0, heads = 0, hd = 0;
  const int32_t* lengths = nullptr;
  int kv_prefix = 0;
  int len_mod = 0;
  int seq0 = 0;
  int causal = 0;
  ActBuf out{};
};

struct StepCoef {
  float c0, c1, c2, c3;
  float sigma;
  int kind;
  int clip;
};

void simt_gemm(const GemmArgs& a, cudaStream_t st);
void simt_ln(const LnArgs& a, cudaStream_t st);
bool simt_attention(const AttnArgs& a, cudaStream_t st);
bool simt_attention_supported(int hd);
bool mma_attention_supported(const AttnArgs& a);
bool mma_attention_init();
void mma_attention(const AttnArgs& a, cudaStream_t st);
bool tc_attention_init();
bool tc_attention_supported(const AttnArgs& a);
bool tc_attention(const AttnArgs& a, int sm_count, cudaStream_t st);
bool simt_init();
enum TextLnMode { TEXT_LN_ROWS = 0, TEXT_LN_EMBED = 1, TEXT_LN_EOS = 2 };
struct TextLnArgs {
  int mode = TEXT_LN_ROWS;
  float* x = nullptr;
  const int64_t* ids = nullptr; int L = 0;
  const float* tok = nullptr; const float* pos = nullptr; int vocab = 0;
  int eos_id = 0;
  const float* gamma = nullptr; const float* beta = nullptr; float eps = 1e-5f;
  int M = 0, d = 0;
  ActBuf out{};
  float* out_f32 = nullptr;
};
bool text_ln_supported(int d);
void text_ln(const TextLnArgs& a, cudaStream_t st);
struct GruStepArgs {
  ActBuf h_in{}, h_out{};
  const float* hf_in = nullptr;
  float* hf_out = nullptr;
  const float* gi = nullptr;
  const float* gh = nullptr;
  const float* b_hh = nullptr;
  const int32_t* lengths = nullptr;
  const __half* w_hh = nullptr;
  int64_t w_plane_stride = 0;
  float w_inv_scale = 1.0f;
  int rows = 0, rows_pad = 0, L = 0, H = 0, step = 0;
  int dirs = 2;
  int64_t h0_ld = 0;
  ActBuf seq_out{};
};
struct GruSeqArgs {
  const float* gi = nullptr;
  const float* b_hh = nullptr;
  const float* h0 = nullptr;
  const int32_t* lengths = nullptr;
  const __half* w_hh = nullptr;
  int64_t w_plane_stride = 0;
  float w_inv_scale = 1.0f;
  ActBuf seq_out{};
  float* h_last = nullptr;
  int rows = 0, L = 0, H = 0;
};
__host__ __device__ __forceinline__ int gru_packed_col(int g, int u) {
  const int t = u >> 5, uu = u & 31;
  return t * 96 + (3 * (uu >> 3) + g) * 8 + (uu & 7);
}
bool gru_tc_init();
bool gru_shape_supported(int H);
bool gru_step_tc(const GruStepArgs& a, cudaStream_t st);
void gru_gate_simt(const GruStepArgs& a, cudaStream_t st);
void gru_init_state(const GruStepArgs& a, const float* h0, cudaStream_t st);
bool gru_seq_supported(int H);
bool gru_seq_tc(const GruSeqArgs& a, int sm_count, cudaStream_t st);
void im2col_k4s2(ActBuf X, const float* src, int64_t ld, int T_in, int C, int Cp, int T_out, int rows, cudaStream_t st);
struct TconvArgs {
  ActBuf x{};
  ActBuf res{};
  int res_conv = 0;
  LinW w{};
  int nseq = 0, T_in = 0, T_out = 0, C = 0, C_res = 0, stride = 1;
  ActBuf out{};
  float* out_f32 = nullptr;
};
bool tconv_tc_init();
bool tconv_tc_supported(const TconvArgs& a);
bool tconv_tc(const TconvArgs& a, int sm_count, cudaStream_t st);
struct TcCtx;
```

mld_b200/csrc/stack.cu:

```cuda
#include "engine.h"
#include "gemm_tc.h"
#include "misc_kernels.cuh"

void op_gemm(mldb_handle* h, const GemmArgs& g, cudaStream_t st) {
  if (h->use_tc && tc_gemm_supported(h->tc, g)) {
    if (!tc_gemm(h->tc, g, nullptr, st)) h->op_failed = true;
    kcount(h, MLDB_KSTAT_GEMM_TC);
    return;
  }
  simt_gemm(g, st);
  kcount(h, MLDB_KSTAT_GEMM_SIMT);
}
void op_gemm_ln(mldb_handle* h, GemmArgs g, LnArgs l, float* cf32, cudaStream_t st) {
  if (h->use_tc && tc_gemm_ln_supported(h->tc, g, l)) {
    if (!tc_gemm(h->tc, g, &l, st)) h->op_failed = true;
    kcount(h, MLDB_KSTAT_GEMM_LN_TC);
    return;
  }
  g.out = ActBuf{}; g.out_f32 = cf32; g.ldc = g.w.N;
  op_gemm(h, g, st);
  l.c = cf32; l.ldc = g.w.N;
  simt_ln(l, st);
  kcount(h, h->use_tc ? MLDB_KSTAT_LN_UNFUSED : MLDB_KSTAT_LN_SIMT);
}
void op_ln(mldb_handle* h, const LnArgs& l, cudaStream_t st) { simt_ln(l, st); kcount(h, MLDB_KSTAT_LN_SIMT); }
void op_attn(mldb_handle* h, const AttnArgs& a, cudaStream_t st) {
  if (h->use_tc && h->attn_kind == 0 && tc_attention_supported(a)) {
    if (!tc_attention(a, h->sm_count, st)) h->op_failed = true;
    kcount(h, MLDB_KSTAT_ATTN_TC);
  } else if (h->use_tc && h->attn_kind <= 1 && mma_attention_supported(a)) {
    mma_attention(a, st);
    kcount(h, MLDB_KSTAT_ATTN_MMA);
  } else {
    if (!simt_attention(a, st)) {
      mldb_set_err("CUDA-core attention: head_dim " + std::to_string(a.hd) + " does not fit shared memory");
      h->op_failed = true;
    }
    kcount(h, MLDB_KSTAT_ATTN_SIMT);
  }
}
int op_gru(mldb_handle* h, ActBuf x, const LinW* w_ih, const LinW& w_hh, const float* b_hh, const float* h0,
           int64_t h0_ld, const int32_t* lengths, int n, int L, int H, int dirs, GrowBuf& gi, GruState& ws,
           ActBuf seq_out, ActBuf* fin, const float** fin_f32, cudaStream_t st) {
  TRY(grow(gi, (size_t)n * L * dirs * 3 * H * sizeof(float)));
  float* gif = (float*)gi.p;
  for (int d = 0; d < dirs; ++d) {
    GemmArgs g; g.a1 = x; g.K1 = x.cols; g.M = n * L; g.w = w_ih[d]; g.out_f32 = gif + (size_t)d * 3 * H;
    g.ldc = dirs * 3 * H; g.wide_n = 1; g.vec_f32 = 1;
    op_gemm(h, g, st);
  }
  if (h->use_tc && dirs == 1) {
    GruSeqArgs s;
    s.gi = gif; s.b_hh = b_hh; s.h0 = h0; s.lengths = lengths; s.w_hh = w_hh.w; s.w_plane_stride = w_hh.plane_stride;
    s.w_inv_scale = w_hh.inv_scale; s.rows = n; s.L = L; s.H = H; s.seq_out = seq_out;
    if (fin_f32) {
      TRY(grow(ws.h_f32, (size_t)n * H * sizeof(float)));
      *fin_f32 = s.h_last = (float*)ws.h_f32.p;
    }
    if (!gru_seq_supported(H) || !gru_seq_tc(s, h->sm_count, st)) h->op_failed = true;
    kcount(h, MLDB_KSTAT_GRU_TC);
    return MLDB_OK;
  }
  const int rows_pad = (n + 127) / 128 * 128;
  const size_t plane = (size_t)dirs * rows_pad * H, state_bytes = split16_bytes(dirs * rows_pad, H);
  TRY(grow(ws.h_split, 2 * state_bytes));
  TRY(grow(ws.h_f32, 2 * plane * sizeof(float)));
  if (!h->use_tc) TRY(grow(ws.gh, plane * 3 * sizeof(float)));
  float *hf = (float*)ws.h_f32.p, *gh = (float*)ws.gh.p;
  auto state = [&](int b) { return split16_at((char*)ws.h_split.p + b * state_bytes, dirs * rows_pad, H); };
  GruStepArgs a;
  a.gi = gif; a.gh = gh; a.b_hh = b_hh; a.lengths = lengths; a.w_hh = w_hh.w; a.w_plane_stride = w_hh.plane_stride;
  a.w_inv_scale = w_hh.inv_scale; a.rows = n; a.rows_pad = rows_pad; a.L = L; a.H = H; a.dirs = dirs; a.h0_ld = h0_ld;
  a.seq_out = seq_out;
  a.h_out = state(0); a.hf_out = hf;
  gru_init_state(a, h0, st);
  kcount(h, MLDB_KSTAT_MISC);
  for (int s = 0; s < L; ++s) {
    a.step = s;
    a.h_in = state(s & 1); a.hf_in = hf + (s & 1) * plane;
    a.h_out = state((s + 1) & 1); a.hf_out = hf + ((s + 1) & 1) * plane;
    if (h->use_tc) {
      if (!gru_step_tc(a, st)) h->op_failed = true;
      kcount(h, MLDB_KSTAT_GRU_TC);
    } else {
      for (int d = 0; d < dirs; ++d) {
        LinW w = w_hh;
        w.w += (size_t)d * 3 * H * H; w.N = 3 * H;
        GemmArgs g; g.a1 = rows_of(a.h_in, (int64_t)d * rows_pad, n); g.K1 = H; g.M = n; g.w = w;
        g.out_f32 = gh + (size_t)d * rows_pad * 3 * H; g.ldc = 3 * H; g.wide_n = 1;
        op_gemm(h, g, st);
      }
      gru_gate_simt(a, st);
      kcount(h, MLDB_KSTAT_MISC);
    }
  }
  if (fin) *fin = state(L & 1);
  if (fin_f32) *fin_f32 = hf + (L & 1) * plane;
  return MLDB_OK;
}
static int ffn_scratch_slot(const mldb_handle* h, cudaStream_t st) {
  int k = 0;
  for (int i = 0; i < mldb_handle::MAX_BRANCHES - 1; ++i) if (st == h->br_stream[i]) k = i + 1;
  return k;
}
static void op_ffn(mldb_handle* h, const GemmArgs& g1, const GemmArgs& g2, const LnArgs& l2, float* cf32, cudaStream_t st) {
  if (h->use_tc && tc_ffn_supported(h->tc, g1, g2, l2)) {
    const int k = ffn_scratch_slot(h, st);
    if (!tc_ffn(h->tc, g1, g2, l2, h->ffn_scratch[k], h->ffn_flags[k], st)) h->op_failed = true;
    kcount(h, MLDB_KSTAT_FFN_TC);
    return;
  }
  op_gemm(h, g1, st);
  op_gemm_ln(h, g2, l2, cf32, st);
}
void op_tail(mldb_handle* h, const LinW& wo, const LnW& n1, const LinW& l1, const LinW& l2, const LnW& n2, ActBuf att,
             ActBuf x, ActBuf x1, ActBuf hbuf, ActBuf xout, int M, int d, int ff, float* cf32, cudaStream_t st, int fuse) {
  GemmArgs go; go.a1 = att; go.K1 = d; go.M = M; go.w = wo;
  LnArgs ln1; ln1.res = x; ln1.gamma = n1.g; ln1.beta = n1.b; ln1.M = M; ln1.d = d; ln1.out = x1;
  GemmArgs g1; g1.a1 = x1; g1.K1 = d; g1.M = M; g1.w = l1; g1.act = ACT_GELU; g1.out = hbuf;
  GemmArgs g2; g2.a1 = hbuf; g2.K1 = ff; g2.M = M; g2.w = l2;
  LnArgs ln2; ln2.res = x1; ln2.gamma = n2.g; ln2.beta = n2.b; ln2.M = M; ln2.d = d; ln2.out = xout;
  constexpr int FUSE_MAX_TILES = 2;
  const bool small = (M + 127) / 128 <= FUSE_MAX_TILES;
  if (fuse && (fuse == 2 || small) && h->use_tc && tc_tail_supported(h->tc, go, ln1, g1, g2, ln2)) {
    const int k = ffn_scratch_slot(h, st);
    if (!tc_tail(h->tc, go, ln1, g1, g2, ln2, h->ffn_scratch[k], h->ffn_flags[k], st)) h->op_failed = true;
    kcount(h, MLDB_KSTAT_FFN_TC);
    return;
  }
  op_gemm_ln(h, go, ln1, cf32, st);
  op_ffn(h, g1, g2, ln2, cf32, st);
}
void rows_to_split(mldb_handle* h, ActBuf X, const float* src, int ld_src, int M, int d, int in_group, int out_group,
                   int out_off, int src_bcast, const float* tab, int relu, cudaStream_t st) {
  const bool vec = d % 8 == 0 && X.cols % 8 == 0 && (!src || (ld_src % 4 == 0 && ((uintptr_t)src & 15) == 0)) &&
                   (!tab || ((uintptr_t)tab & 15) == 0) && ((uintptr_t)X.hi & 15) == 0 && X.plane_stride % 8 == 0;
  if (vec)
    k_rows_to_split8<<<nblk((int64_t)M * (d / 8)), 256, 0, st>>>(X, src, ld_src, M, d, in_group, out_group, out_off,
                                                                 src_bcast, tab, relu);
  else
    k_rows_to_split<<<nblk((int64_t)M * d), 256, 0, st>>>(X, src, ld_src, M, d, in_group, out_group, out_off, src_bcast,
                                                          tab, relu);
  kcount(h, MLDB_KSTAT_MISC);
}

int alloc_act(mldb_handle* h, int rows, int cols, ActBuf* out) {
  void* p = nullptr;
  TRY(dev_alloc(h, &p, split16_bytes(rows, cols)));
  CK(cudaMemset(p, 0, split16_bytes(rows, cols)));
  *out = split16_at(p, rows, cols);
  return MLDB_OK;
}
int alloc_stack_ws(mldb_handle* h, const StackW& sw, int nseq, int L, int Lmem, StackWs* ws, int n_sel) {
  ws->nseq = nseq; ws->L = L; ws->M = nseq * L; ws->d = sw.d; ws->ff = sw.ff; ws->Lmem = Lmem;
  const int M = ws->M, d = sw.d;
  TRY(alloc_act(h, M, d, &ws->x0));
  TRY(alloc_act(h, M, d, &ws->cur[0]));
  TRY(alloc_act(h, M, d, &ws->cur[1]));
  TRY(alloc_act(h, M, d, &ws->x1));
  TRY(alloc_act(h, M, d, &ws->att));
  TRY(alloc_act(h, M, 3 * d, &ws->qkv));
  TRY(alloc_act(h, M, sw.ff, &ws->h));
  const bool enc = sw.kind == STACK_SKIP_ENC || sw.kind == STACK_PLAIN_ENC;
  if (!enc) {
    TRY(alloc_act(h, M, d, &ws->x2));
    TRY(alloc_act(h, M, d, &ws->qc));
    TRY(alloc_act(h, nseq * Lmem, 2 * d, &ws->kvm));
    TRY(alloc_act(h, nseq, d, &ws->vrow));
    TRY(dev_alloc(h, (void**)&ws->cvec, (size_t)nseq * d * sizeof(float)));
  }
  if (sw.kind == STACK_SKIP_ENC || sw.kind == STACK_SKIP_DEC) {
    TRY(alloc_act(h, M, d, &ws->cat));
    const int nb = (sw.layers - 1) / 2;
    ws->ys.resize(nb);
    for (int i = 0; i < nb; ++i) TRY(alloc_act(h, M, d, &ws->ys[i]));
  }
  TRY(dev_alloc(h, (void**)&ws->cf32, (size_t)M * d * sizeof(float)));
  if (enc && n_sel > 0) {
    ws->n_sel = n_sel;
    const int R = nseq * n_sel;
    TRY(alloc_act(h, R, d, &ws->sx));
    TRY(alloc_act(h, R, d, &ws->sq));
    TRY(alloc_act(h, R, d, &ws->satt));
    TRY(alloc_act(h, R, d, &ws->sx1));
    TRY(alloc_act(h, R, sw.ff, &ws->sh));
    TRY(alloc_act(h, R, d, &ws->sout));
  }
  return MLDB_OK;
}

StackWs ws_slice(const StackWs& ws, int s0, int n) {
  StackWs w = ws;
  w.nseq = n; w.M = n * ws.L;
  auto tok = [&](ActBuf b) { return b.hi ? rows_of(b, (int64_t)s0 * ws.L, n * ws.L) : b; };
  auto sel = [&](ActBuf b) { return b.hi ? rows_of(b, (int64_t)s0 * ws.n_sel, n * ws.n_sel) : b; };
  w.x0 = tok(ws.x0); w.cur[0] = tok(ws.cur[0]); w.cur[1] = tok(ws.cur[1]); w.x1 = tok(ws.x1); w.x2 = tok(ws.x2);
  w.att = tok(ws.att); w.qkv = tok(ws.qkv); w.qc = tok(ws.qc); w.h = tok(ws.h); w.cat = tok(ws.cat);
  for (auto& y : w.ys) y = tok(y);
  if (ws.kvm.hi) w.kvm = rows_of(ws.kvm, (int64_t)s0 * ws.Lmem, n * ws.Lmem);
  if (ws.vrow.hi) w.vrow = rows_of(ws.vrow, s0, n);
  if (ws.cvec) w.cvec = ws.cvec + (size_t)s0 * ws.d;
  if (ws.cf32) w.cf32 = ws.cf32 + (size_t)s0 * ws.L * ws.d;
  w.sx = sel(ws.sx); w.sq = sel(ws.sq); w.satt = sel(ws.satt); w.sx1 = sel(ws.sx1); w.sh = sel(ws.sh); w.sout = sel(ws.sout);
  return w;
}
void out_proj_ln(mldb_handle* h, const LinW& w, const LnW& n, ActBuf att, ActBuf res, ActBuf xout, int M, int d,
                 float* cf32, cudaStream_t st) {
  GemmArgs g; g.a1 = att; g.K1 = d; g.M = M; g.w = w;
  LnArgs l; l.res = res; l.gamma = n.g; l.beta = n.b; l.M = M; l.d = d; l.out = xout;
  op_gemm_ln(h, g, l, cf32, st);
}
static void self_attn(mldb_handle* h, const LinW& in_proj, ActBuf xin, StackWs& ws, const SeqInfo& si, int heads,
                      cudaStream_t st) {
  const int d = ws.d;
  GemmArgs g; g.a1 = xin; g.K1 = d; g.M = ws.M; g.w = in_proj; g.out = ws.qkv;
  op_gemm(h, g, st);
  AttnArgs a; a.q = ws.qkv; a.q_col0 = 0; a.Lq = ws.L; a.kv = ws.qkv; a.k_col0 = d; a.v_col0 = 2 * d;
  a.Lk = ws.L; a.nseq = ws.nseq; a.heads = heads; a.hd = d / heads;
  a.lengths = si.lengths; a.kv_prefix = si.kv_prefix; a.len_mod = si.len_mod; a.seq0 = 0; a.out = ws.att;
  op_attn(h, a, st);
}
static void self_attn_block(mldb_handle* h, const LinW& in_proj, const LinW& out_proj, const LnW& n,
                            ActBuf xin, ActBuf xout, StackWs& ws, const SeqInfo& si, int heads,
                            cudaStream_t st) {
  self_attn(h, in_proj, xin, ws, si, heads, st);
  out_proj_ln(h, out_proj, n, ws.att, xin, xout, ws.M, ws.d, ws.cf32, st);
}
void ffn_block(mldb_handle* h, const LinW& l1, const LinW& l2, const LnW& n, ActBuf xin, ActBuf xout, StackWs& ws,
               int act, cudaStream_t st) {
  GemmArgs g; g.a1 = xin; g.K1 = ws.d; g.M = ws.M; g.w = l1; g.act = act; g.out = ws.h;
  GemmArgs g2; g2.a1 = ws.h; g2.K1 = ws.ff; g2.M = ws.M; g2.w = l2;
  LnArgs l; l.res = xin; l.gamma = n.g; l.beta = n.b; l.M = ws.M; l.d = ws.d; l.out = xout;
  op_ffn(h, g, g2, l, ws.cf32, st);
}
void enc_layer(mldb_handle* h, const StackW& sw, const EncW& w, ActBuf xin, ActBuf xout, StackWs& ws,
               const SeqInfo& si, cudaStream_t st) {
  self_attn(h, w.in_proj, xin, ws, si, sw.heads, st);
  op_tail(h, w.out_proj, w.n1, w.l1, w.l2, w.n2, ws.att, xin, ws.x1, ws.h, xout, ws.M, ws.d, ws.ff, ws.cf32, st);
}
static void dec_layer(mldb_handle* h, const StackW& sw, const DecW& w, ActBuf xin, ActBuf xout,
                      ActBuf mem, StackWs& ws, const SeqInfo& si, cudaStream_t st) {
  const int d = ws.d;
  self_attn_block(h, w.sa_in, w.sa_out, w.n1, xin, ws.x1, ws, si, sw.heads, st);
  if (ws.Lmem == 1) {
    GemmArgs gv; gv.a1 = mem; gv.K1 = d; gv.M = ws.nseq; gv.w = w.ca_v; gv.out = ws.vrow;
    op_gemm(h, gv, st);
    GemmArgs gc; gc.a1 = ws.vrow; gc.K1 = d; gc.M = ws.nseq; gc.w = w.ca_out; gc.out_f32 = ws.cvec; gc.ldc = d;
    op_gemm(h, gc, st);
    LnArgs lc; lc.res = ws.x1; lc.rowvec = ws.cvec; lc.rv_group = ws.L; lc.gamma = w.n2.g; lc.beta = w.n2.b;
    lc.M = ws.M; lc.d = d; lc.out = ws.x2;
    op_ln(h, lc, st);
    ffn_block(h, w.l1, w.l2, w.n3, ws.x2, xout, ws, ACT_GELU, st);
    return;
  }
  GemmArgs gq; gq.a1 = ws.x1; gq.K1 = d; gq.M = ws.M; gq.w = w.ca_q; gq.out = ws.qc;
  op_gemm(h, gq, st);
  GemmArgs gk; gk.a1 = mem; gk.K1 = d; gk.M = ws.nseq * ws.Lmem; gk.w = w.ca_kv; gk.out = ws.kvm;
  op_gemm(h, gk, st);
  AttnArgs a; a.q = ws.qc; a.q_col0 = 0; a.Lq = ws.L; a.kv = ws.kvm; a.k_col0 = 0; a.v_col0 = d;
  a.Lk = ws.Lmem; a.nseq = ws.nseq; a.heads = sw.heads; a.hd = d / sw.heads; a.out = ws.att;
  op_attn(h, a, st);
  out_proj_ln(h, w.ca_out, w.n2, ws.att, ws.x1, ws.x2, ws.M, d, ws.cf32, st);
  ffn_block(h, w.l1, w.l2, w.n3, ws.x2, xout, ws, ACT_GELU, st);
}
static void any_layer(mldb_handle* h, const StackW& sw, int li, ActBuf xin, ActBuf xout, ActBuf mem,
                      StackWs& ws, const SeqInfo& si, cudaStream_t st) {
  if (sw.kind == STACK_SKIP_ENC) enc_layer(h, sw, sw.enc[li], xin, xout, ws, si, st);
  else dec_layer(h, sw, sw.dec[li], xin, xout, mem, ws, si, st);
}
__global__ void k_gather_rows(ActBuf src, ActBuf dst, int L, int n_sel, int nrows_out, int d) {
  pdl_trigger();
  pdl_wait();
  const int64_t idx = (int64_t)blockIdx.x * blockDim.x + threadIdx.x;
  if (idx >= (int64_t)nrows_out * (d / 8)) return;
  const int c = (int)(idx % (d / 8));
  const int r = (int)(idx / (d / 8));
  const int64_t srow = (int64_t)(r / n_sel) * L + r % n_sel;
  const uint4* sh = reinterpret_cast<const uint4*>(src.hi + srow * src.cols) + c;
  const uint4* sl = reinterpret_cast<const uint4*>(src.lo() + srow * src.cols) + c;
  reinterpret_cast<uint4*>(dst.hi + (int64_t)r * dst.cols)[c] = *sh;
  reinterpret_cast<uint4*>(dst.lo() + (int64_t)r * dst.cols)[c] = *sl;
}

static ActBuf enc_layer_selected(mldb_handle* h, const StackW& sw, const EncW& w, ActBuf xin, StackWs& ws,
                                 const SeqInfo& si, cudaStream_t st) {
  const int d = ws.d, R = ws.nseq * ws.n_sel;
  GemmArgs gk; gk.a1 = xin; gk.K1 = d; gk.M = ws.M; gk.w = w.kv_only; gk.out = ws.qkv;
  op_gemm(h, gk, st);
  launch_pdl(k_gather_rows, dim3(nblk((int64_t)R * (d / 8))), dim3(256), 0, st, xin, ws.sx, ws.L, ws.n_sel, R, d);
  kcount(h, MLDB_KSTAT_MISC);
  GemmArgs gq; gq.a1 = ws.sx; gq.K1 = d; gq.M = R; gq.w = w.q_only; gq.out = ws.sq;
  op_gemm(h, gq, st);
  AttnArgs a; a.q = ws.sq; a.q_col0 = 0; a.Lq = ws.n_sel; a.kv = ws.qkv; a.k_col0 = 0; a.v_col0 = d;
  a.Lk = ws.L; a.nseq = ws.nseq; a.heads = sw.heads; a.hd = d / sw.heads; a.lengths = si.lengths;
  a.kv_prefix = si.kv_prefix; a.len_mod = si.len_mod; a.out = ws.satt;
  op_attn(h, a, st);
  op_tail(h, w.out_proj, w.n1, w.l1, w.l2, w.n2, ws.satt, ws.sx, ws.sx1, ws.sh, ws.sout, R, d, ws.ff, ws.cf32, st);
  return ws.sout;
}

ActBuf run_stack(mldb_handle* h, const StackW& sw, ActBuf x0, ActBuf mem, StackWs& ws, const SeqInfo& si,
                 cudaStream_t st) {
  if (sw.kind == STACK_PLAIN_ENC) {
    ActBuf x = x0;
    for (int i = 0; i + 1 < sw.layers; ++i) {
      enc_layer(h, sw, sw.enc[i], x, ws.cur[i & 1], ws, si, st);
      x = ws.cur[i & 1];
    }
    return enc_layer_selected(h, sw, sw.enc.back(), x, ws, si, st);
  }
  if (sw.kind == STACK_PLAIN_DEC) {
    ActBuf x = x0;
    for (int i = 0; i < sw.layers; ++i) {
      any_layer(h, sw, i, x, ws.cur[i & 1], mem, ws, si, st);
      x = ws.cur[i & 1];
    }
    return x;
  }
  const int nb = (sw.layers - 1) / 2;
  ActBuf x = x0;
  for (int i = 0; i < nb; ++i) {
    any_layer(h, sw, i, x, ws.ys[i], mem, ws, si, st);
    x = ws.ys[i];
  }
  any_layer(h, sw, nb, x, ws.cur[0], mem, ws, si, st);
  x = ws.cur[0];
  for (int i = 0; i < nb; ++i) {
    GemmArgs g; g.a1 = x; g.K1 = sw.d; g.a2 = ws.ys[nb - 1 - i]; g.K2 = sw.d; g.M = ws.M;
    g.w = sw.skip[i]; g.out = ws.cat;
    op_gemm(h, g, st);
    if (i == nb - 1 && sw.kind == STACK_SKIP_ENC && ws.n_sel > 0)
      return enc_layer_selected(h, sw, sw.enc[nb + 1 + i], ws.cat, ws, si, st);
    any_layer(h, sw, nb + 1 + i, ws.cat, ws.cur[(i + 1) & 1], mem, ws, si, st);
    x = ws.cur[(i + 1) & 1];
  }
  return x;
}
```

mld_b200/csrc/tc_common.cuh:

```cuda
#pragma once
#include <cuda.h>
#include <stdio.h>
#include <stdlib.h>
#include <string.h>

#include <string>

#include "common.cuh"

namespace tc {

__device__ __forceinline__ uint32_t smem_u32(const void* p) { return (uint32_t)__cvta_generic_to_shared(p); }
__device__ __forceinline__ uint32_t smem_pad1024(const void* raw) { return (1024u - (smem_u32(raw) & 1023u)) & 1023u; }

__device__ __forceinline__ void mbar_init(uint32_t bar, uint32_t count) {
  asm volatile("mbarrier.init.shared::cta.b64 [%0], %1;" ::"r"(bar), "r"(count) : "memory");
}
__device__ __forceinline__ void mbar_expect_tx(uint32_t bar, uint32_t bytes) {
  asm volatile("mbarrier.arrive.expect_tx.shared::cta.b64 _, [%0], %1;" ::"r"(bar), "r"(bytes) : "memory");
}
__device__ __forceinline__ void mbar_arrive(uint32_t bar) {
  asm volatile("mbarrier.arrive.shared::cta.b64 _, [%0];" ::"r"(bar) : "memory");
}
__device__ __forceinline__ void mbar_arrive_cnt(uint32_t bar, uint32_t n) {
  asm volatile("mbarrier.arrive.shared::cta.b64 _, [%0], %1;" ::"r"(bar), "r"(n) : "memory");
}
__device__ __forceinline__ void mbar_wait(uint32_t bar, uint32_t parity) {
  uint32_t done = 0, spins = 0;
  long long t0 = 0;
  do {
    asm volatile(
        "{\n\t.reg .pred p;\n\t"
        "mbarrier.try_wait.parity.shared::cta.b64 p, [%1], %2;\n\t"
        "selp.u32 %0, 1, 0, p;\n\t}"
        : "=r"(done)
        : "r"(bar), "r"(parity)
        : "memory");
    if (!done && (++spins & 1023u) == 0) {
      const long long now = clock64();
      if (t0 == 0) t0 = now;
      else if (now - t0 > 4000000000ll) __trap();
    }
  } while (!done);
}
__device__ __forceinline__ bool mbar_test(uint32_t bar, uint32_t parity) {
  uint32_t done;
  asm volatile(
      "{\n\t.reg .pred p;\n\t"
      "mbarrier.test_wait.parity.shared::cta.b64 p, [%1], %2;\n\t"
      "selp.u32 %0, 1, 0, p;\n\t}"
      : "=r"(done)
      : "r"(bar), "r"(parity)
      : "memory");
  return done != 0;
}

__device__ __forceinline__ void tma_load_2d(uint32_t dst, const CUtensorMap* map, uint32_t bar, int c0, int c1) {
  asm volatile(
      "cp.async.bulk.tensor.2d.shared::cluster.global.mbarrier::complete_tx::bytes [%0], [%1, {%3, %4}], [%2];"
      ::"r"(dst), "l"(reinterpret_cast<uint64_t>(map)), "r"(bar), "r"(c0), "r"(c1)
      : "memory");
}
__device__ __forceinline__ void tma_load_3d(uint32_t dst, const CUtensorMap* map, uint32_t bar, int c0, int c1, int c2) {
  asm volatile(
      "cp.async.bulk.tensor.3d.shared::cluster.global.mbarrier::complete_tx::bytes [%0], [%1, {%3, %4, %5}], [%2];"
      ::"r"(dst), "l"(reinterpret_cast<uint64_t>(map)), "r"(bar), "r"(c0), "r"(c1), "r"(c2)
      : "memory");
}
__device__ __forceinline__ void tma_load_4d(uint32_t dst, const CUtensorMap* map, uint32_t bar, int c0, int c1, int c2,
                                            int c3) {
  asm volatile(
      "cp.async.bulk.tensor.4d.shared::cluster.global.mbarrier::complete_tx::bytes [%0], [%1, {%3, %4, %5, %6}], [%2];"
      ::"r"(dst), "l"(reinterpret_cast<uint64_t>(map)), "r"(bar), "r"(c0), "r"(c1), "r"(c2), "r"(c3)
      : "memory");
}
__device__ __forceinline__ void tma_prefetch_2d(const CUtensorMap* map, int c0, int c1) {
  asm volatile("cp.async.bulk.prefetch.tensor.2d.L2.global.tile [%0, {%1, %2}];"
               ::"l"(reinterpret_cast<uint64_t>(map)), "r"(c0), "r"(c1) : "memory");
}
__device__ __forceinline__ void tma_prefetch_desc(const CUtensorMap* map) {
  asm volatile("prefetch.tensormap [%0];" ::"l"(reinterpret_cast<uint64_t>(map)) : "memory");
}
__device__ __forceinline__ void tma_store_2d(const CUtensorMap* map, uint32_t src, int c0, int c1) {
  asm volatile("cp.async.bulk.tensor.2d.global.shared::cta.bulk_group [%0, {%2, %3}], [%1];"
               ::"l"(reinterpret_cast<uint64_t>(map)), "r"(src), "r"(c0), "r"(c1) : "memory");
}
__device__ __forceinline__ void bulk_commit() { asm volatile("cp.async.bulk.commit_group;" ::: "memory"); }
template <int N> __device__ __forceinline__ void bulk_wait_read() {
  asm volatile("cp.async.bulk.wait_group.read %0;" ::"n"(N) : "memory");
}
__device__ __forceinline__ void fence_async_smem() { asm volatile("fence.proxy.async.shared::cta;" ::: "memory"); }

__device__ __forceinline__ bool elect_one() {
  uint32_t pred;
  asm volatile("{\n\t.reg .pred p;\n\telect.sync _|p, 0xffffffff;\n\tselp.u32 %0, 1, 0, p;\n\t}" : "=r"(pred));
  return pred != 0;
}

template <int N> __device__ __forceinline__ void reg_dec() { asm volatile("setmaxnreg.dec.sync.aligned.u32 %0;" ::"n"(N)); }
template <int N> __device__ __forceinline__ void reg_inc() { asm volatile("setmaxnreg.inc.sync.aligned.u32 %0;" ::"n"(N)); }
__device__ __forceinline__ void named_bar_sync(int id, int threads) {
  asm volatile("bar.sync %0, %1;" ::"r"(id), "r"(threads) : "memory");
}

__device__ __forceinline__ void wg_fence() { asm volatile("wgmma.fence.sync.aligned;" ::: "memory"); }
__device__ __forceinline__ void wg_commit() { asm volatile("wgmma.commit_group.sync.aligned;" ::: "memory"); }
template <int N> __device__ __forceinline__ void wg_wait() { asm volatile("wgmma.wait_group.sync.aligned %0;" ::"n"(N) : "memory"); }

template <int N> __device__ __forceinline__ void acc_fence(float (&d)[N]) {
#pragma unroll
  for (int i = 0; i < N; ++i) asm volatile("" : "+f"(d[i])::"memory");
}

__device__ __forceinline__ uint64_t make_desc(uint32_t saddr) {
  return (uint64_t)((saddr >> 4) & 0x3FFF) | ((uint64_t)1 << 16) | ((uint64_t)(1024 >> 4) << 32) | ((uint64_t)1 << 62);
}
__device__ __forceinline__ void wgmma_ss_n256(float (&d)[128], uint64_t adesc, uint64_t bdesc, uint32_t acc) {
  asm volatile(
      "{\n\t.reg .pred p;\n\t"
      "setp.ne.b32 p, %130, 0;\n\t"
      "wgmma.mma_async.sync.aligned.m64n256k16.f32.f16.f16 "
      "{%0, %1, %2, %3, %4, %5, %6, %7, %8, %9, %10, %11, %12, %13, %14, %15, "
      "%16, %17, %18, %19, %20, %21, %22, %23, %24, %25, %26, %27, %28, %29, %30, %31, "
      "%32, %33, %34, %35, %36, %37, %38, %39, %40, %41, %42, %43, %44, %45, %46, %47, "
      "%48, %49, %50, %51, %52, %53, %54, %55, %56, %57, %58, %59, %60, %61, %62, %63, "
      "%64, %65, %66, %67, %68, %69, %70, %71, %72, %73, %74, %75, %76, %77, %78, %79, "
      "%80, %81, %82, %83, %84, %85, %86, %87, %88, %89, %90, %91, %92, %93, %94, %95, "
      "%96, %97, %98, %99, %100, %101, %102, %103, %104, %105, %106, %107, %108, %109, %110, %111, "
      "%112, %113, %114, %115, %116, %117, %118, %119, %120, %121, %122, %123, %124, %125, %126, %127}, "
      "%128, %129, p, 1, 1, 0, 0;\n\t}"
      : "+f"(d[0]), "+f"(d[1]), "+f"(d[2]), "+f"(d[3]), "+f"(d[4]), "+f"(d[5]), "+f"(d[6]), "+f"(d[7]),
        "+f"(d[8]), "+f"(d[9]), "+f"(d[10]), "+f"(d[11]), "+f"(d[12]), "+f"(d[13]), "+f"(d[14]), "+f"(d[15]),
        "+f"(d[16]), "+f"(d[17]), "+f"(d[18]), "+f"(d[19]), "+f"(d[20]), "+f"(d[21]), "+f"(d[22]), "+f"(d[23]),
        "+f"(d[24]), "+f"(d[25]), "+f"(d[26]), "+f"(d[27]), "+f"(d[28]), "+f"(d[29]), "+f"(d[30]), "+f"(d[31]),
        "+f"(d[32]), "+f"(d[33]), "+f"(d[34]), "+f"(d[35]), "+f"(d[36]), "+f"(d[37]), "+f"(d[38]), "+f"(d[39]),
        "+f"(d[40]), "+f"(d[41]), "+f"(d[42]), "+f"(d[43]), "+f"(d[44]), "+f"(d[45]), "+f"(d[46]), "+f"(d[47]),
        "+f"(d[48]), "+f"(d[49]), "+f"(d[50]), "+f"(d[51]), "+f"(d[52]), "+f"(d[53]), "+f"(d[54]), "+f"(d[55]),
        "+f"(d[56]), "+f"(d[57]), "+f"(d[58]), "+f"(d[59]), "+f"(d[60]), "+f"(d[61]), "+f"(d[62]), "+f"(d[63]),
        "+f"(d[64]), "+f"(d[65]), "+f"(d[66]), "+f"(d[67]), "+f"(d[68]), "+f"(d[69]), "+f"(d[70]), "+f"(d[71]),
        "+f"(d[72]), "+f"(d[73]), "+f"(d[74]), "+f"(d[75]), "+f"(d[76]), "+f"(d[77]), "+f"(d[78]), "+f"(d[79]),
        "+f"(d[80]), "+f"(d[81]), "+f"(d[82]), "+f"(d[83]), "+f"(d[84]), "+f"(d[85]), "+f"(d[86]), "+f"(d[87]),
        "+f"(d[88]), "+f"(d[89]), "+f"(d[90]), "+f"(d[91]), "+f"(d[92]), "+f"(d[93]), "+f"(d[94]), "+f"(d[95]),
        "+f"(d[96]), "+f"(d[97]), "+f"(d[98]), "+f"(d[99]), "+f"(d[100]), "+f"(d[101]), "+f"(d[102]), "+f"(d[103]),
        "+f"(d[104]), "+f"(d[105]), "+f"(d[106]), "+f"(d[107]), "+f"(d[108]), "+f"(d[109]), "+f"(d[110]), "+f"(d[111]),
        "+f"(d[112]), "+f"(d[113]), "+f"(d[114]), "+f"(d[115]), "+f"(d[116]), "+f"(d[117]), "+f"(d[118]), "+f"(d[119]),
        "+f"(d[120]), "+f"(d[121]), "+f"(d[122]), "+f"(d[123]), "+f"(d[124]), "+f"(d[125]), "+f"(d[126]), "+f"(d[127])
      : "l"(adesc), "l"(bdesc), "r"(acc)
      : "memory");
}
__device__ __forceinline__ void wgmma_ss_n128(float (&d)[64], uint64_t adesc, uint64_t bdesc, uint32_t acc) {
  asm volatile(
      "{\n\t.reg .pred p;\n\t"
      "setp.ne.b32 p, %66, 0;\n\t"
      "wgmma.mma_async.sync.aligned.m64n128k16.f32.f16.f16 "
      "{%0, %1, %2, %3, %4, %5, %6, %7, %8, %9, %10, %11, %12, %13, %14, %15, "
      "%16, %17, %18, %19, %20, %21, %22, %23, %24, %25, %26, %27, %28, %29, %30, %31, "
      "%32, %33, %34, %35, %36, %37, %38, %39, %40, %41, %42, %43, %44, %45, %46, %47, "
      "%48, %49, %50, %51, %52, %53, %54, %55, %56, %57, %58, %59, %60, %61, %62, %63}, "
      "%64, %65, p, 1, 1, 0, 0;\n\t}"
      : "+f"(d[0]), "+f"(d[1]), "+f"(d[2]), "+f"(d[3]), "+f"(d[4]), "+f"(d[5]), "+f"(d[6]), "+f"(d[7]),
        "+f"(d[8]), "+f"(d[9]), "+f"(d[10]), "+f"(d[11]), "+f"(d[12]), "+f"(d[13]), "+f"(d[14]), "+f"(d[15]),
        "+f"(d[16]), "+f"(d[17]), "+f"(d[18]), "+f"(d[19]), "+f"(d[20]), "+f"(d[21]), "+f"(d[22]), "+f"(d[23]),
        "+f"(d[24]), "+f"(d[25]), "+f"(d[26]), "+f"(d[27]), "+f"(d[28]), "+f"(d[29]), "+f"(d[30]), "+f"(d[31]),
        "+f"(d[32]), "+f"(d[33]), "+f"(d[34]), "+f"(d[35]), "+f"(d[36]), "+f"(d[37]), "+f"(d[38]), "+f"(d[39]),
        "+f"(d[40]), "+f"(d[41]), "+f"(d[42]), "+f"(d[43]), "+f"(d[44]), "+f"(d[45]), "+f"(d[46]), "+f"(d[47]),
        "+f"(d[48]), "+f"(d[49]), "+f"(d[50]), "+f"(d[51]), "+f"(d[52]), "+f"(d[53]), "+f"(d[54]), "+f"(d[55]),
        "+f"(d[56]), "+f"(d[57]), "+f"(d[58]), "+f"(d[59]), "+f"(d[60]), "+f"(d[61]), "+f"(d[62]), "+f"(d[63])
      : "l"(adesc), "l"(bdesc), "r"(acc)
      : "memory");
}
__device__ __forceinline__ void wgmma_ss_n96(float (&d)[48], uint64_t adesc, uint64_t bdesc, uint32_t acc) {
  asm volatile(
      "{\n\t.reg .pred p;\n\t"
      "setp.ne.b32 p, %50, 0;\n\t"
      "wgmma.mma_async.sync.aligned.m64n96k16.f32.f16.f16 "
      "{%0, %1, %2, %3, %4, %5, %6, %7, %8, %9, %10, %11, %12, %13, %14, %15, "
      "%16, %17, %18, %19, %20, %21, %22, %23, %24, %25, %26, %27, %28, %29, %30, %31, "
      "%32, %33, %34, %35, %36, %37, %38, %39, %40, %41, %42, %43, %44, %45, %46, %47}, "
      "%48, %49, p, 1, 1, 0, 0;\n\t}"
      : "+f"(d[0]), "+f"(d[1]), "+f"(d[2]), "+f"(d[3]), "+f"(d[4]), "+f"(d[5]), "+f"(d[6]), "+f"(d[7]),
        "+f"(d[8]), "+f"(d[9]), "+f"(d[10]), "+f"(d[11]), "+f"(d[12]), "+f"(d[13]), "+f"(d[14]), "+f"(d[15]),
        "+f"(d[16]), "+f"(d[17]), "+f"(d[18]), "+f"(d[19]), "+f"(d[20]), "+f"(d[21]), "+f"(d[22]), "+f"(d[23]),
        "+f"(d[24]), "+f"(d[25]), "+f"(d[26]), "+f"(d[27]), "+f"(d[28]), "+f"(d[29]), "+f"(d[30]), "+f"(d[31]),
        "+f"(d[32]), "+f"(d[33]), "+f"(d[34]), "+f"(d[35]), "+f"(d[36]), "+f"(d[37]), "+f"(d[38]), "+f"(d[39]),
        "+f"(d[40]), "+f"(d[41]), "+f"(d[42]), "+f"(d[43]), "+f"(d[44]), "+f"(d[45]), "+f"(d[46]), "+f"(d[47])
      : "l"(adesc), "l"(bdesc), "r"(acc)
      : "memory");
}
__device__ __forceinline__ void wgmma_ss_n64(float (&d)[32], uint64_t adesc, uint64_t bdesc, uint32_t acc) {
  asm volatile(
      "{\n\t.reg .pred p;\n\t"
      "setp.ne.b32 p, %34, 0;\n\t"
      "wgmma.mma_async.sync.aligned.m64n64k16.f32.f16.f16 "
      "{%0, %1, %2, %3, %4, %5, %6, %7, %8, %9, %10, %11, %12, %13, %14, %15, "
      "%16, %17, %18, %19, %20, %21, %22, %23, %24, %25, %26, %27, %28, %29, %30, %31}, "
      "%32, %33, p, 1, 1, 0, 0;\n\t}"
      : "+f"(d[0]), "+f"(d[1]), "+f"(d[2]), "+f"(d[3]), "+f"(d[4]), "+f"(d[5]), "+f"(d[6]), "+f"(d[7]),
        "+f"(d[8]), "+f"(d[9]), "+f"(d[10]), "+f"(d[11]), "+f"(d[12]), "+f"(d[13]), "+f"(d[14]), "+f"(d[15]),
        "+f"(d[16]), "+f"(d[17]), "+f"(d[18]), "+f"(d[19]), "+f"(d[20]), "+f"(d[21]), "+f"(d[22]), "+f"(d[23]),
        "+f"(d[24]), "+f"(d[25]), "+f"(d[26]), "+f"(d[27]), "+f"(d[28]), "+f"(d[29]), "+f"(d[30]), "+f"(d[31])
      : "l"(adesc), "l"(bdesc), "r"(acc)
      : "memory");
}
__device__ __forceinline__ void wgmma_rs_n256(float (&d)[128], const uint32_t (&a)[4], uint64_t bdesc, uint32_t acc) {
  asm volatile(
      "{\n\t.reg .pred p;\n\t"
      "setp.ne.b32 p, %133, 0;\n\t"
      "wgmma.mma_async.sync.aligned.m64n256k16.f32.f16.f16 "
      "{%0, %1, %2, %3, %4, %5, %6, %7, %8, %9, %10, %11, %12, %13, %14, %15, "
      "%16, %17, %18, %19, %20, %21, %22, %23, %24, %25, %26, %27, %28, %29, %30, %31, "
      "%32, %33, %34, %35, %36, %37, %38, %39, %40, %41, %42, %43, %44, %45, %46, %47, "
      "%48, %49, %50, %51, %52, %53, %54, %55, %56, %57, %58, %59, %60, %61, %62, %63, "
      "%64, %65, %66, %67, %68, %69, %70, %71, %72, %73, %74, %75, %76, %77, %78, %79, "
      "%80, %81, %82, %83, %84, %85, %86, %87, %88, %89, %90, %91, %92, %93, %94, %95, "
      "%96, %97, %98, %99, %100, %101, %102, %103, %104, %105, %106, %107, %108, %109, %110, %111, "
      "%112, %113, %114, %115, %116, %117, %118, %119, %120, %121, %122, %123, %124, %125, %126, %127}, "
      "{%128, %129, %130, %131}, %132, p, 1, 1, 0;\n\t}"
      : "+f"(d[0]), "+f"(d[1]), "+f"(d[2]), "+f"(d[3]), "+f"(d[4]), "+f"(d[5]), "+f"(d[6]), "+f"(d[7]),
        "+f"(d[8]), "+f"(d[9]), "+f"(d[10]), "+f"(d[11]), "+f"(d[12]), "+f"(d[13]), "+f"(d[14]), "+f"(d[15]),
        "+f"(d[16]), "+f"(d[17]), "+f"(d[18]), "+f"(d[19]), "+f"(d[20]), "+f"(d[21]), "+f"(d[22]), "+f"(d[23]),
        "+f"(d[24]), "+f"(d[25]), "+f"(d[26]), "+f"(d[27]), "+f"(d[28]), "+f"(d[29]), "+f"(d[30]), "+f"(d[31]),
        "+f"(d[32]), "+f"(d[33]), "+f"(d[34]), "+f"(d[35]), "+f"(d[36]), "+f"(d[37]), "+f"(d[38]), "+f"(d[39]),
        "+f"(d[40]), "+f"(d[41]), "+f"(d[42]), "+f"(d[43]), "+f"(d[44]), "+f"(d[45]), "+f"(d[46]), "+f"(d[47]),
        "+f"(d[48]), "+f"(d[49]), "+f"(d[50]), "+f"(d[51]), "+f"(d[52]), "+f"(d[53]), "+f"(d[54]), "+f"(d[55]),
        "+f"(d[56]), "+f"(d[57]), "+f"(d[58]), "+f"(d[59]), "+f"(d[60]), "+f"(d[61]), "+f"(d[62]), "+f"(d[63]),
        "+f"(d[64]), "+f"(d[65]), "+f"(d[66]), "+f"(d[67]), "+f"(d[68]), "+f"(d[69]), "+f"(d[70]), "+f"(d[71]),
        "+f"(d[72]), "+f"(d[73]), "+f"(d[74]), "+f"(d[75]), "+f"(d[76]), "+f"(d[77]), "+f"(d[78]), "+f"(d[79]),
        "+f"(d[80]), "+f"(d[81]), "+f"(d[82]), "+f"(d[83]), "+f"(d[84]), "+f"(d[85]), "+f"(d[86]), "+f"(d[87]),
        "+f"(d[88]), "+f"(d[89]), "+f"(d[90]), "+f"(d[91]), "+f"(d[92]), "+f"(d[93]), "+f"(d[94]), "+f"(d[95]),
        "+f"(d[96]), "+f"(d[97]), "+f"(d[98]), "+f"(d[99]), "+f"(d[100]), "+f"(d[101]), "+f"(d[102]), "+f"(d[103]),
        "+f"(d[104]), "+f"(d[105]), "+f"(d[106]), "+f"(d[107]), "+f"(d[108]), "+f"(d[109]), "+f"(d[110]), "+f"(d[111]),
        "+f"(d[112]), "+f"(d[113]), "+f"(d[114]), "+f"(d[115]), "+f"(d[116]), "+f"(d[117]), "+f"(d[118]), "+f"(d[119]),
        "+f"(d[120]), "+f"(d[121]), "+f"(d[122]), "+f"(d[123]), "+f"(d[124]), "+f"(d[125]), "+f"(d[126]), "+f"(d[127])
      : "r"(a[0]), "r"(a[1]), "r"(a[2]), "r"(a[3]), "l"(bdesc), "r"(acc)
      : "memory");
}
__device__ __forceinline__ void wgmma_rs_n48(float (&d)[24], const uint32_t (&a)[4], uint64_t bdesc, uint32_t acc) {
  asm volatile(
      "{\n\t.reg .pred p;\n\t"
      "setp.ne.b32 p, %29, 0;\n\t"
      "wgmma.mma_async.sync.aligned.m64n48k16.f32.f16.f16 "
      "{%0, %1, %2, %3, %4, %5, %6, %7, %8, %9, %10, %11, %12, %13, %14, %15, %16, %17, %18, %19, %20, %21, %22, %23}, "
      "{%24, %25, %26, %27}, %28, p, 1, 1, 0;\n\t}"
      : "+f"(d[0]), "+f"(d[1]), "+f"(d[2]), "+f"(d[3]), "+f"(d[4]), "+f"(d[5]), "+f"(d[6]), "+f"(d[7]),
        "+f"(d[8]), "+f"(d[9]), "+f"(d[10]), "+f"(d[11]), "+f"(d[12]), "+f"(d[13]), "+f"(d[14]), "+f"(d[15]),
        "+f"(d[16]), "+f"(d[17]), "+f"(d[18]), "+f"(d[19]), "+f"(d[20]), "+f"(d[21]), "+f"(d[22]), "+f"(d[23])
      : "r"(a[0]), "r"(a[1]), "r"(a[2]), "r"(a[3]), "l"(bdesc), "r"(acc)
      : "memory");
}
__device__ __forceinline__ void wgmma_rs_n64_tb(float (&d)[32], const uint32_t (&a)[4], uint64_t bdesc, uint32_t acc) {
  asm volatile(
      "{\n\t.reg .pred p;\n\t"
      "setp.ne.b32 p, %37, 0;\n\t"
      "wgmma.mma_async.sync.aligned.m64n64k16.f32.f16.f16 "
      "{%0, %1, %2, %3, %4, %5, %6, %7, %8, %9, %10, %11, %12, %13, %14, %15, "
      "%16, %17, %18, %19, %20, %21, %22, %23, %24, %25, %26, %27, %28, %29, %30, %31}, "
      "{%32, %33, %34, %35}, %36, p, 1, 1, 1;\n\t}"
      : "+f"(d[0]), "+f"(d[1]), "+f"(d[2]), "+f"(d[3]), "+f"(d[4]), "+f"(d[5]), "+f"(d[6]), "+f"(d[7]),
        "+f"(d[8]), "+f"(d[9]), "+f"(d[10]), "+f"(d[11]), "+f"(d[12]), "+f"(d[13]), "+f"(d[14]), "+f"(d[15]),
        "+f"(d[16]), "+f"(d[17]), "+f"(d[18]), "+f"(d[19]), "+f"(d[20]), "+f"(d[21]), "+f"(d[22]), "+f"(d[23]),
        "+f"(d[24]), "+f"(d[25]), "+f"(d[26]), "+f"(d[27]), "+f"(d[28]), "+f"(d[29]), "+f"(d[30]), "+f"(d[31])
      : "r"(a[0]), "r"(a[1]), "r"(a[2]), "r"(a[3]), "l"(bdesc), "r"(acc)
      : "memory");
}

template <int N>
__device__ __forceinline__ void wgmma_ss(float (&d)[N / 2], uint64_t a, uint64_t b, uint32_t acc) {
  static_assert(N == 256 || N == 128 || N == 96 || N == 64, "wgmma_ss width");
  if constexpr (N == 256) wgmma_ss_n256(d, a, b, acc);
  else if constexpr (N == 128) wgmma_ss_n128(d, a, b, acc);
  else if constexpr (N == 96) wgmma_ss_n96(d, a, b, acc);
  else wgmma_ss_n64(d, a, b, acc);
}
template <int N>
__device__ __forceinline__ void kblock_ss(float (&d)[N / 2], uint32_t sAh, uint32_t sAl, uint32_t sWh, uint32_t sWl, bool first) {
  uint64_t ah = make_desc(sAh), al = make_desc(sAl), wh = make_desc(sWh), wl = make_desc(sWl);
#pragma unroll
  for (int kk = 0; kk < 4; ++kk) {
    wgmma_ss<N>(d, al, wh, (first && kk == 0) ? 0u : 1u);
    wgmma_ss<N>(d, ah, wl, 1u);
    wgmma_ss<N>(d, ah, wh, 1u);
    ah += 2; al += 2; wh += 2; wl += 2;
  }
}

__device__ __forceinline__ float quad_sum(float v) {
  v += __shfl_xor_sync(0xffffffffu, v, 1);
  return v + __shfl_xor_sync(0xffffffffu, v, 2);
}

__device__ __forceinline__ void split2(float x0, float x1, uint32_t& hi, uint32_t& lo) {
  const __half2 h2 = __floats2half2_rn(x0, x1);
  const float2 hf = __half22float2(h2);
  const __half2 l2 = __floats2half2_rn(x0 - hf.x, x1 - hf.y);
  hi = *reinterpret_cast<const uint32_t*>(&h2);
  lo = *reinterpret_cast<const uint32_t*>(&l2);
}

constexpr int TL_CAPW = 512;
__device__ __forceinline__ void tl_event(long long* tl, int& n, int tag, int aux = 0) {
  if (tl != nullptr && blockIdx.x == 0 && (threadIdx.x & 31) == 0 && n < TL_CAPW) {
    long long* e = tl + ((size_t)(threadIdx.x >> 5) * TL_CAPW + n) * 2;
    e[0] = (long long)tag | ((long long)aux << 24);
    e[1] = clock64();
    ++n;
  }
}
long long* mldb_timeline_buffer();

typedef CUresult (*PFN_tmapEncodeTiled)(CUtensorMap*, CUtensorMapDataType, cuuint32_t, void*, const cuuint64_t*,
                                        const cuuint64_t*, const cuuint32_t*, const cuuint32_t*,
                                        CUtensorMapInterleave, CUtensorMapSwizzle, CUtensorMapL2promotion,
                                        CUtensorMapFloatOOBfill);

inline PFN_tmapEncodeTiled tmap_encoder() {
  static const PFN_tmapEncodeTiled fn = [] {
    void* p = nullptr;
    cudaDriverEntryPointQueryResult q;
    const cudaError_t e = cudaGetDriverEntryPoint("cuTensorMapEncodeTiled", &p, cudaEnableDefault, &q);
    return e == cudaSuccess && q == cudaDriverEntryPointSuccess ? (PFN_tmapEncodeTiled)p : nullptr;
  }();
  if (!fn) mldb_set_err("cuTensorMapEncodeTiled is not available from the driver");
  return fn;
}

inline bool encode_plane_map(CUtensorMap* m, const __half* base, int rank, const cuuint64_t* dims,
                             const cuuint64_t* strides, const cuuint32_t* box, const cuuint32_t* estr = nullptr) {
  const PFN_tmapEncodeTiled encode = tmap_encoder();
  if (!encode) return false;
  const cuuint32_t ones[5] = {1, 1, 1, 1, 1};
  const CUresult r = encode(m, CU_TENSOR_MAP_DATA_TYPE_FLOAT16, (cuuint32_t)rank, (void*)base, dims, strides, box,
                            estr ? estr : ones, CU_TENSOR_MAP_INTERLEAVE_NONE, CU_TENSOR_MAP_SWIZZLE_128B,
                            CU_TENSOR_MAP_L2_PROMOTION_L2_256B, CU_TENSOR_MAP_FLOAT_OOB_FILL_NONE);
  if (r != CUDA_SUCCESS) {
    std::string shape;
    for (int i = rank - 1; i >= 0; --i) shape += std::to_string(dims[i]) + (i ? " x " : "");
    char buf[96];
    snprintf(buf, sizeof buf, "(CUresult %d): fp16 plane at %p", (int)r, (const void*)base);
    mldb_set_err("cuTensorMapEncodeTiled failed " + std::string(buf) + ", [" + shape + "], box " +
                 std::to_string(box[1]) + " rows");
  }
  return r == CUDA_SUCCESS;
}
inline bool make_map(CUtensorMap* m, const __half* base, int rows, int cols, int box_rows) {
  const cuuint64_t dims[2] = {(cuuint64_t)cols, (cuuint64_t)rows};
  const cuuint64_t strides[1] = {(cuuint64_t)cols * sizeof(__half)};
  const cuuint32_t box[2] = {64u, (cuuint32_t)box_rows};
  return encode_plane_map(m, base, 2, dims, strides, box);
}
inline bool make_seq_map(CUtensorMap* m, const __half* base, int nseq, int L, int cols, int box_rows) {
  const cuuint64_t dims[3] = {(cuuint64_t)cols, (cuuint64_t)L, (cuuint64_t)nseq};
  const cuuint64_t strides[2] = {(cuuint64_t)cols * sizeof(__half), (cuuint64_t)L * cols * sizeof(__half)};
  const cuuint32_t box[3] = {64u, (cuuint32_t)box_rows, 1u};
  return encode_plane_map(m, base, 3, dims, strides, box);
}

inline int snake_order() {
  static const int on = [] { const char* e = getenv("MLDB_SNAKE"); return (e && !strcmp(e, "0")) ? 0 : 1; }();
  return on;
}

}
```

Measured before the change: 858.7.

## Move first LayerNorm from out-proj epilogue into fused FFN kernel for large M

For large row counts, the out-projection GEMM now adds the split16 residual and writes a plain fp32 pre-norm sum. A new FFN kernel variant loads that fp32 tile by TMA, applies LayerNorm1 in shared memory, and splits it to hi/lo planes before the FFN GEMMs. This removes the separate GEMM+LN pass and the round trip of the normalized x1 through global memory. In exchange it adds a template kernel variant, an fp32 tensor map and extra per-tile LN work inside the FFN kernel, and it relies on the new swizzled tile indexing being correct.

New measurement: 860.0, median of 6. About the same (+0.2%).

```diff
diff --git a/mld_b200/csrc/debug.cu b/mld_b200/csrc/debug.cu
--- a/mld_b200/csrc/debug.cu
+++ b/mld_b200/csrc/debug.cu
@@ -20,6 +20,11 @@
   const EncW& w = h->den.enc[0];
   const int d = ws.d;
   SeqInfo si;
+  auto tail = [&](int fuse, int part) {
+    op_tail(h, w.out_proj, w.n1, w.l1, w.l2, w.n2, ws.att, ws.x0, ws.x1, ws.h, ws.cur[0], ws.M, d, ws.ff, ws.cf32, st,
+            fuse, part);
+  };
+  if (!strcmp(op, "ffn")) tail(1, TAIL_OUTPROJ);
   auto run = [&]() -> int {
     if (!strcmp(op, "qkv")) {
       GemmArgs g; g.a1 = ws.x0; g.K1 = d; g.M = ws.M; g.w = w.in_proj; g.out = ws.qkv; op_gemm(h, g, st);
@@ -27,7 +32,7 @@
       AttnArgs a; a.q = ws.qkv; a.Lq = ws.L; a.kv = ws.qkv; a.k_col0 = d; a.v_col0 = 2 * d; a.Lk = ws.L;
       a.nseq = ws.nseq; a.heads = c.num_heads; a.hd = d / c.num_heads; a.out = ws.att; op_attn(h, a, st);
     } else if (!strcmp(op, "outproj_ln")) {
-      out_proj_ln(h, w.out_proj, w.n1, ws.att, ws.x0, ws.x1, ws.M, d, ws.cf32, st);
+      tail(1, TAIL_OUTPROJ);
     } else if (!strcmp(op, "ffn1")) {
       GemmArgs g; g.a1 = ws.x1; g.K1 = d; g.M = ws.M; g.w = w.l1; g.act = ACT_GELU; g.out = ws.h; op_gemm(h, g, st);
     } else if (!strcmp(op, "ffn2_ln")) {
@@ -35,11 +40,11 @@
       LnArgs l; l.res = ws.x1; l.gamma = w.n2.g; l.beta = w.n2.b; l.M = ws.M; l.d = d; l.out = ws.cur[0];
       op_gemm_ln(h, g, l, ws.cf32, st);
     } else if (!strcmp(op, "ffn")) {
-      ffn_block(h, w.l1, w.l2, w.n2, ws.x1, ws.cur[0], ws, ACT_GELU, st);
+      tail(1, TAIL_FFN);
     } else if (!strcmp(op, "tail")) {
-      op_tail(h, w.out_proj, w.n1, w.l1, w.l2, w.n2, ws.att, ws.x0, ws.x1, ws.h, ws.cur[0], ws.M, d, ws.ff, ws.cf32, st);
+      tail(1, TAIL_ALL);
     } else if (!strcmp(op, "tail_fused")) {
-      op_tail(h, w.out_proj, w.n1, w.l1, w.l2, w.n2, ws.att, ws.x0, ws.x1, ws.h, ws.cur[0], ws.M, d, ws.ff, ws.cf32, st, 2);
+      tail(2, TAIL_ALL);
     } else if (!strcmp(op, "layer")) {
       enc_layer(h, h->den, w, ws.x0, ws.cur[0], ws, si, st);
     } else {
diff --git a/mld_b200/csrc/engine.h b/mld_b200/csrc/engine.h
--- a/mld_b200/csrc/engine.h
+++ b/mld_b200/csrc/engine.h
@@ -325,9 +325,10 @@
 int op_gru(mldb_handle* h, ActBuf x, const LinW* w_ih, const LinW& w_hh, const float* b_hh, const float* h0,
            int64_t h0_ld, const int32_t* lengths, int n, int L, int H, int dirs, GrowBuf& gi, GruState& ws,
            ActBuf seq_out, ActBuf* fin, const float** fin_f32, cudaStream_t st);
+enum { TAIL_ALL = 0, TAIL_OUTPROJ = 1, TAIL_FFN = 2 };
 void op_tail(mldb_handle* h, const LinW& wo, const LnW& n1, const LinW& l1, const LinW& l2, const LnW& n2, ActBuf att,
              ActBuf x, ActBuf x1, ActBuf hbuf, ActBuf xout, int M, int d, int ff, float* cf32, cudaStream_t st,
-             int fuse = 1);
+             int fuse = 1, int part = TAIL_ALL);
 void rows_to_split(mldb_handle* h, ActBuf X, const float* src, int ld_src, int M, int d, int in_group, int out_group,
                    int out_off, int src_bcast, const float* tab, int relu, cudaStream_t st);
 int alloc_act(mldb_handle* h, int rows, int cols, ActBuf* out);
diff --git a/mld_b200/csrc/gemm_tc.cu b/mld_b200/csrc/gemm_tc.cu
--- a/mld_b200/csrc/gemm_tc.cu
+++ b/mld_b200/csrc/gemm_tc.cu
@@ -166,6 +166,38 @@
               *reinterpret_cast<uint32_t*>(at(j, h, 0)) = hi;
               *reinterpret_cast<uint32_t*>(at(j, h, 1)) = lo;
             }
+          });
+}
+
+__device__ __forceinline__ __half2* tile_at(uint8_t* tile, int rl, int lane, int cp, int j, int h, int plane) {
+  return reinterpret_cast<__half2*>(tile + rl * 128 + cp * 2 + plane * 65536 + h * 1024 + (j >> 3) * 16384 +
+                                    (((j & 7) ^ (lane >> 2)) << 4));
+}
+__device__ __forceinline__ void tile_store(uint8_t* tile, int rl, int lane, int cp, int j, const float (&y)[4]) {
+#pragma unroll
+  for (int h = 0; h < 2; ++h) {
+    uint32_t hi, lo;
+    split2(y[2 * h], y[2 * h + 1], hi, lo);
+    *reinterpret_cast<uint32_t*>(tile_at(tile, rl, lane, cp, j, h, 0)) = hi;
+    *reinterpret_cast<uint32_t*>(tile_at(tile, rl, lane, cp, j, h, 1)) = lo;
+  }
+}
+__device__ __forceinline__ void ln1_tile(float (&d)[128], const float* gamma, const float* beta, uint8_t* tile, int rl,
+                                         int lane, int cp) {
+  const uint8_t* const row0 = tile + rl * 128 + (cp & 3) * 4;
+  const int sw = lane >> 2;
+  ln_rows(d, 1.0f, nullptr, gamma, beta, cp,
+          [&](int j, float (&x)[4]) {
+#pragma unroll
+            for (int h = 0; h < 2; ++h) {
+              const float2 z = *reinterpret_cast<const float2*>(row0 + ((j >> 2) & 1) * 65536 + (j >> 3) * 16384 +
+                                                                h * 1024 + (((2 * (j & 3) + (cp >> 2)) ^ sw) << 4));
+              x[2 * h] = z.x; x[2 * h + 1] = z.y;
+            }
+          },
+          [&](int j, const float (&y)[4]) {
+            if (j == 0) __syncwarp();
+            tile_store(tile, rl, lane, cp, j, y);
           });
 }
 
@@ -373,14 +405,14 @@
   static_assert(SMEM_BYTES <= 232448, "shared memory budget");
 };
 
-__global__ void __launch_bounds__(MMA_THREADS, 1)
-k_ffn_tc(const __grid_constant__ CUtensorMap tmXh, const __grid_constant__ CUtensorMap tmXl,
-         const __grid_constant__ CUtensorMap tmW1h, const __grid_constant__ CUtensorMap tmW1l,
-         const __grid_constant__ CUtensorMap tmW2h, const __grid_constant__ CUtensorMap tmW2l,
-         const __grid_constant__ CUtensorMap tmAh, const __grid_constant__ CUtensorMap tmAl,
-         const __grid_constant__ CUtensorMap tmWoh, const __grid_constant__ CUtensorMap tmWol,
-         const __grid_constant__ CUtensorMap tmYh, const __grid_constant__ CUtensorMap tmYl, const FfnParams p) {
+template <bool LN1>
+__device__ __forceinline__ void ffn_tc(const CUtensorMap& tmXh, const CUtensorMap& tmXl, const CUtensorMap& tmW1h,
+                                       const CUtensorMap& tmW1l, const CUtensorMap& tmW2h, const CUtensorMap& tmW2l,
+                                       const CUtensorMap& tmAh, const CUtensorMap& tmAl, const CUtensorMap& tmWoh,
+                                       const CUtensorMap& tmWol, const CUtensorMap& tmYh, const CUtensorMap& tmYl,
+                                       const FfnParams& p) {
   using Cfg = FfnCfg;
+  const bool prefix = !LN1 && p.prefix;
   constexpr int STAGES = Cfg::STAGES;
   extern __shared__ uint8_t smem_raw[];
   uint8_t* smem = smem_raw + smem_pad1024(smem_raw);
@@ -406,14 +438,14 @@
     return Item{rev(p.full * ncta + t), c0, c1, p.parts == 1 ? 0 : (part == p.parts - 1 ? 2 : 1),
                 p.parts == 1 ? 0 : slot0 + (part == p.parts - 1 ? 0 : part)};
   };
-  const int PRE = p.prefix ? 8 : 0;
+  const int PRE = prefix ? 8 : 0;
   const int per_tile = PRE + 4 * NC;
   int total = p.full * per_tile;
   if (nlocal > p.full) {
     const Item it = item(p.full);
     total += PRE + 4 * (it.c1 - it.c0);
   }
-  const int XG = p.prefix ? 2 : 1;
+  const int XG = prefix ? 2 : 1;
   const int xtotal = nlocal * 4 * XG;
 
   if (threadIdx.x == 0) {
@@ -429,7 +461,7 @@
     tma_prefetch_desc(&tmXh); tma_prefetch_desc(&tmXl); tma_prefetch_desc(&tmW1h);
     tma_prefetch_desc(&tmW1l); tma_prefetch_desc(&tmW2h); tma_prefetch_desc(&tmW2l);
     tma_prefetch_desc(&tmYh); tma_prefetch_desc(&tmYl);
-    if (p.prefix) { tma_prefetch_desc(&tmAh); tma_prefetch_desc(&tmAl); tma_prefetch_desc(&tmWoh); tma_prefetch_desc(&tmWol); }
+    if (prefix) { tma_prefetch_desc(&tmAh); tma_prefetch_desc(&tmAl); tma_prefetch_desc(&tmWoh); tma_prefetch_desc(&tmWol); }
   }
   pdl_trigger();
   __syncthreads();
@@ -464,19 +496,26 @@
   auto load_x = [&](int v) {
     if (elect_one()) {
       const int j = v / (4 * XG), kb = v & 3;
-      const bool att = p.prefix && (v >> 2) == j * XG;
+      const bool att = prefix && (v >> 2) == j * XG;
       const int m0 = item(j).mt * BM;
       const uint32_t full = smem_u32(&bar_xfull[kb]);
       mbar_expect_tx(full, 2 * BM * 128);
-      tma_load_2d(smem_u32(smem + kb * 16384), att ? &tmAh : &tmXh, full, kb * BK, m0);
-      tma_load_2d(smem_u32(smem + 65536 + kb * 16384), att ? &tmAl : &tmXl, full, kb * BK, m0);
-      if (att && kb == 0)
-        for (int k2 = 0; k2 < 4; ++k2) { tma_prefetch_2d(&tmXh, k2 * BK, m0); tma_prefetch_2d(&tmXl, k2 * BK, m0); }
-      if (v % (4 * XG) == 0 && j + 1 < nlocal) {
-        const int m1 = item(j + 1).mt * BM;
-        for (int k2 = 0; k2 < 4; ++k2) {
-          tma_prefetch_2d(&tmXh, k2 * BK, m1); tma_prefetch_2d(&tmXl, k2 * BK, m1);
-          if (p.prefix) { tma_prefetch_2d(&tmAh, k2 * BK, m1); tma_prefetch_2d(&tmAl, k2 * BK, m1); }
+      if constexpr (LN1) {
+        tma_load_2d(smem_u32(smem + kb * 16384), &tmXh, full, kb * BK, m0);
+        tma_load_2d(smem_u32(smem + 65536 + kb * 16384), &tmXh, full, kb * BK + 32, m0);
+        if (v % 4 == 0 && j + 1 < nlocal)
+          for (int c = 0; c < 8; ++c) tma_prefetch_2d(&tmXh, c * 32, item(j + 1).mt * BM);
+      } else {
+        tma_load_2d(smem_u32(smem + kb * 16384), att ? &tmAh : &tmXh, full, kb * BK, m0);
+        tma_load_2d(smem_u32(smem + 65536 + kb * 16384), att ? &tmAl : &tmXl, full, kb * BK, m0);
+        if (att && kb == 0)
+          for (int k2 = 0; k2 < 4; ++k2) { tma_prefetch_2d(&tmXh, k2 * BK, m0); tma_prefetch_2d(&tmXl, k2 * BK, m0); }
+        if (v % (4 * XG) == 0 && j + 1 < nlocal) {
+          const int m1 = item(j + 1).mt * BM;
+          for (int k2 = 0; k2 < 4; ++k2) {
+            tma_prefetch_2d(&tmXh, k2 * BK, m1); tma_prefetch_2d(&tmXl, k2 * BK, m1);
+            if (prefix) { tma_prefetch_2d(&tmAh, k2 * BK, m1); tma_prefetch_2d(&tmAl, k2 * BK, m1); }
+          }
         }
       }
     }
@@ -504,7 +543,7 @@
     const int m0 = it.mt * BM;
     const uint32_t xpar = (uint32_t)(j * XG) & 1u;
     if (warp == 0) produce(-1, 4 * j * XG + 3);
-    if (p.prefix) {
+    if (prefix) {
 #pragma unroll
       for (int kb = 0; kb < 4; ++kb) {
         if (warp == 0) produce(rc + 1, -1);
@@ -529,6 +568,13 @@
       fence_async_smem();
       named_bar_sync(2 + cw, 128);
       tl_event(p.tl, tl_n, 61, j);
+    } else if (LN1) {
+#pragma unroll
+      for (int kb = 0; kb < 4; ++kb) x_full(kb, xpar);
+      ln1_tile(acc2, p.gamma1, p.beta1, smem, rl, lane, cp);
+      fence_async_smem();
+      named_bar_sync(2 + cw, 128);
+      tl_event(p.tl, tl_n, 61, j);
     } else {
 #pragma unroll
       for (int kb = 0; kb < 4; ++kb) x_full(kb, xpar);
@@ -669,11 +715,28 @@
   tl_event(p.tl, tl_n, 42);
 }
 
+#define MLDB_FFN_PARAMS                                                                                          \
+  const __grid_constant__ CUtensorMap tmXh, const __grid_constant__ CUtensorMap tmXl,                          \
+      const __grid_constant__ CUtensorMap tmW1h, const __grid_constant__ CUtensorMap tmW1l,                    \
+      const __grid_constant__ CUtensorMap tmW2h, const __grid_constant__ CUtensorMap tmW2l,                    \
+      const __grid_constant__ CUtensorMap tmAh, const __grid_constant__ CUtensorMap tmAl,                      \
+      const __grid_constant__ CUtensorMap tmWoh, const __grid_constant__ CUtensorMap tmWol,                    \
+      const __grid_constant__ CUtensorMap tmYh, const __grid_constant__ CUtensorMap tmYl, const FfnParams p
+__global__ void __launch_bounds__(MMA_THREADS, 1) k_ffn_tc(MLDB_FFN_PARAMS) {
+  ffn_tc<false>(tmXh, tmXl, tmW1h, tmW1l, tmW2h, tmW2l, tmAh, tmAl, tmWoh, tmWol, tmYh, tmYl, p);
+}
+__global__ void __launch_bounds__(MMA_THREADS, 1) k_ffn_ln1_tc(MLDB_FFN_PARAMS) {
+  ffn_tc<true>(tmXh, tmXl, tmW1h, tmW1l, tmW2h, tmW2l, tmAh, tmAl, tmWoh, tmWol, tmYh, tmYl, p);
+}
+#undef MLDB_FFN_PARAMS
+
 struct ProjParams {
   int M, n_chunks, items;
   float inv_scale;
   const float* bias;
   __half* out_hi; __half* out_lo; int ld_out, out_col0;
+  const __half* res_hi; const __half* res_lo; int ld_res;
+  float* out_f32; int ldc;
   long long* tl;
 };
 struct ProjCfg {
@@ -684,10 +747,9 @@
   static_assert(SMEM_BYTES <= 232448, "shared memory budget");
 };
 
-template <int ACT>
-__global__ void __launch_bounds__(MMA_THREADS, 1)
-k_proj_tc(const __grid_constant__ CUtensorMap tmAh, const __grid_constant__ CUtensorMap tmAl,
-          const __grid_constant__ CUtensorMap tmWh, const __grid_constant__ CUtensorMap tmWl, const ProjParams p) {
+template <int ACT, bool RES>
+__device__ __forceinline__ void proj_tc(const CUtensorMap& tmAh, const CUtensorMap& tmAl, const CUtensorMap& tmWh,
+                                        const CUtensorMap& tmWl, const ProjParams& p) {
   using Cfg = ProjCfg;
   constexpr int STAGES = Cfg::STAGES;
   extern __shared__ uint8_t smem_raw[];
@@ -770,29 +832,65 @@
     const int l = lane & 3;
     const bool ok0 = r_lo < p.M, ok1 = r_lo + 8 < p.M;
     const int64_t o0 = (int64_t)r_lo * p.ld_out + p.out_col0 + n0 + 8 * l, o1 = o0 + (int64_t)8 * p.ld_out;
-    tl_event(p.tl, tl_n, 52, i);
-#pragma unroll
-    for (int jb = 0; jb < Cfg::CHUNK / 32; ++jb) {
-      uint32_t h0[4], l0[4], h1[4], l1[4];
-#pragma unroll
-      for (int g = 0; g < 4; ++g) {
-        const int j = 4 * jb + g;
-        float x[4];
-        fast_group<ACT>(d, j, p.inv_scale, __ldg(reinterpret_cast<const float2*>(p.bias + n0 + 8 * j + cp)), x);
-        split2(x[0], x[1], h0[g], l0[g]);
-        split2(x[2], x[3], h1[g], l1[g]);
-      }
-      quad_transpose(h0, l); quad_transpose(l0, l); quad_transpose(h1, l); quad_transpose(l1, l);
-      if (ok0) {
-        *reinterpret_cast<uint4*>(p.out_hi + o0 + 32 * jb) = make_uint4(h0[0], h0[1], h0[2], h0[3]);
-        *reinterpret_cast<uint4*>(p.out_lo + o0 + 32 * jb) = make_uint4(l0[0], l0[1], l0[2], l0[3]);
-      }
-      if (ok1) {
-        *reinterpret_cast<uint4*>(p.out_hi + o1 + 32 * jb) = make_uint4(h1[0], h1[1], h1[2], h1[3]);
-        *reinterpret_cast<uint4*>(p.out_lo + o1 + 32 * jb) = make_uint4(l1[0], l1[1], l1[2], l1[3]);
-      }
-    }
-    tl_event(p.tl, tl_n, 53, i);
+    tl_event(p.tl, tl_n, RES ? 54 : 52, i);
+    if constexpr (RES) {
+      const int64_t r0 = (int64_t)r_lo * p.ld_res + n0 + 8 * l, r1 = r0 + (int64_t)8 * p.ld_res;
+      float* const z0 = p.out_f32 + (int64_t)r_lo * p.ldc + n0 + 8 * l;
+      float* const z1 = z0 + (int64_t)8 * p.ldc;
+      auto store_row = [&](const __half* rh, const __half* rl, float* z, const uint32_t (&ve)[4], const uint32_t (&vo)[4]) {
+        const uint4 hv = *reinterpret_cast<const uint4*>(rh), lv = *reinterpret_cast<const uint4*>(rl);
+        const uint32_t hw[4] = {hv.x, hv.y, hv.z, hv.w}, lw[4] = {lv.x, lv.y, lv.z, lv.w};
+        float o[8];
+#pragma unroll
+        for (int g = 0; g < 4; ++g) {
+          const float2 h = __half22float2(*reinterpret_cast<const __half2*>(&hw[g]));
+          const float2 lo = __half22float2(*reinterpret_cast<const __half2*>(&lw[g]));
+          o[2 * g] = (__uint_as_float(ve[g]) + h.x) + lo.x;
+          o[2 * g + 1] = (__uint_as_float(vo[g]) + h.y) + lo.y;
+        }
+        reinterpret_cast<float4*>(z)[0] = make_float4(o[0], o[1], o[2], o[3]);
+        reinterpret_cast<float4*>(z)[1] = make_float4(o[4], o[5], o[6], o[7]);
+      };
+#pragma unroll
+      for (int jb = 0; jb < Cfg::CHUNK / 32; ++jb) {
+        uint32_t e0[4], o0[4], e1[4], o1[4];
+#pragma unroll
+        for (int g = 0; g < 4; ++g) {
+          const int j = 4 * jb + g;
+          float x[4];
+          fast_group<ACT_NONE>(d, j, p.inv_scale, __ldg(reinterpret_cast<const float2*>(p.bias + n0 + 8 * j + cp)), x);
+          e0[g] = __float_as_uint(x[0]); o0[g] = __float_as_uint(x[1]);
+          e1[g] = __float_as_uint(x[2]); o1[g] = __float_as_uint(x[3]);
+        }
+        quad_transpose(e0, l); quad_transpose(o0, l); quad_transpose(e1, l); quad_transpose(o1, l);
+        if (ok0) store_row(p.res_hi + r0 + 32 * jb, p.res_lo + r0 + 32 * jb, z0 + 32 * jb, e0, o0);
+        if (ok1) store_row(p.res_hi + r1 + 32 * jb, p.res_lo + r1 + 32 * jb, z1 + 32 * jb, e1, o1);
+      }
+      tl_event(p.tl, tl_n, 55, i);
+    } else {
+#pragma unroll
+      for (int jb = 0; jb < Cfg::CHUNK / 32; ++jb) {
+        uint32_t h0[4], l0[4], h1[4], l1[4];
+#pragma unroll
+        for (int g = 0; g < 4; ++g) {
+          const int j = 4 * jb + g;
+          float x[4];
+          fast_group<ACT>(d, j, p.inv_scale, __ldg(reinterpret_cast<const float2*>(p.bias + n0 + 8 * j + cp)), x);
+          split2(x[0], x[1], h0[g], l0[g]);
+          split2(x[2], x[3], h1[g], l1[g]);
+        }
+        quad_transpose(h0, l); quad_transpose(l0, l); quad_transpose(h1, l); quad_transpose(l1, l);
+        if (ok0) {
+          *reinterpret_cast<uint4*>(p.out_hi + o0 + 32 * jb) = make_uint4(h0[0], h0[1], h0[2], h0[3]);
+          *reinterpret_cast<uint4*>(p.out_lo + o0 + 32 * jb) = make_uint4(l0[0], l0[1], l0[2], l0[3]);
+        }
+        if (ok1) {
+          *reinterpret_cast<uint4*>(p.out_hi + o1 + 32 * jb) = make_uint4(h1[0], h1[1], h1[2], h1[3]);
+          *reinterpret_cast<uint4*>(p.out_lo + o1 + 32 * jb) = make_uint4(l1[0], l1[1], l1[2], l1[3]);
+        }
+      }
+      tl_event(p.tl, tl_n, 53, i);
+    }
   };
   auto step = [&](int i, float (&cur)[64], float (&prev)[64]) {
     const bool fresh = first_of_tile(i);
@@ -836,6 +934,18 @@
     epilogue(acc0, n - 1);
   }
   tl_event(p.tl, tl_n, 42);
+}
+
+template <int ACT>
+__global__ void __launch_bounds__(MMA_THREADS, 1)
+k_proj_tc(const __grid_constant__ CUtensorMap tmAh, const __grid_constant__ CUtensorMap tmAl,
+          const __grid_constant__ CUtensorMap tmWh, const __grid_constant__ CUtensorMap tmWl, const ProjParams p) {
+  proj_tc<ACT, false>(tmAh, tmAl, tmWh, tmWl, p);
+}
+__global__ void __launch_bounds__(MMA_THREADS, 1)
+k_proj_res_tc(const __grid_constant__ CUtensorMap tmAh, const __grid_constant__ CUtensorMap tmAl,
+              const __grid_constant__ CUtensorMap tmWh, const __grid_constant__ CUtensorMap tmWl, const ProjParams p) {
+  proj_tc<ACT_NONE, true>(tmAh, tmAl, tmWh, tmWl, p);
 }
 
 }
@@ -864,9 +974,10 @@
   opt_in(k_gemm_tc<256, EPI_FAST, ACT_LEAKY>, TileCfg<256>::SMEM_BYTES); opt_in(k_gemm_tc<128, EPI_FAST, ACT_LEAKY>, TileCfg<128>::SMEM_BYTES);
   opt_in(k_gemm_tc<256, EPI_F32>, TileCfg<256>::SMEM_BYTES); opt_in(k_gemm_tc<128, EPI_F32>, TileCfg<128>::SMEM_BYTES);
   opt_in(k_gemm_tc<256, EPI_F32, ACT_LEAKY>, TileCfg<256>::SMEM_BYTES); opt_in(k_gemm_tc<128, EPI_F32, ACT_LEAKY>, TileCfg<128>::SMEM_BYTES);
-  opt_in(k_ffn_tc, FfnCfg::SMEM_BYTES);
+  opt_in(k_ffn_tc, FfnCfg::SMEM_BYTES); opt_in(k_ffn_ln1_tc, FfnCfg::SMEM_BYTES);
   opt_in(k_proj_tc<ACT_NONE>, ProjCfg::SMEM_BYTES); opt_in(k_proj_tc<ACT_GELU>, ProjCfg::SMEM_BYTES);
   opt_in(k_proj_tc<ACT_QUICKGELU>, ProjCfg::SMEM_BYTES); opt_in(k_proj_tc<ACT_LEAKY>, ProjCfg::SMEM_BYTES);
+  opt_in(k_proj_res_tc, ProjCfg::SMEM_BYTES);
   if (!ok) {
     delete c;
     return nullptr;
@@ -889,6 +1000,14 @@
                     g.out_group != 0 || g.out_off != 0 || (g.w.N % 2) || (g.ldc % 2) || ((uintptr_t)g.out_f32 & 7) ||
                     ((uintptr_t)g.res_f32 & 7)))
     return false;
+  if (g.res_split.hi) {
+    const uintptr_t align = (uintptr_t)g.out_f32 | (uintptr_t)g.res_split.hi | (uintptr_t)g.res_split.lo();
+    if (!g.out_f32 || g.out.hi || g.res_f32 || g.K1 != 256 || g.K2 != 0 || g.act != ACT_NONE || !g.w.bias ||
+        g.addtab || g.zero_lengths || g.in_group < g.M || g.out_group != 0 || g.out_off != 0 ||
+        g.w.N % ProjCfg::CHUNK || g.res_split.cols < g.w.N || g.res_split.cols % 8 || g.ldc < g.w.N || g.ldc % 4 ||
+        (align & 15))
+      return false;
+  }
   return true;
 }
 
@@ -930,9 +1049,15 @@
   ProjParams p{};
   p.M = g.M; p.n_chunks = g.w.N / ProjCfg::CHUNK; p.items = (g.M + BM - 1) / BM * p.n_chunks;
   p.inv_scale = g.w.inv_scale; p.bias = g.w.bias;
-  p.out_hi = g.out.hi; p.out_lo = g.out.lo(); p.ld_out = g.out.cols; p.out_col0 = g.out_col0;
   p.tl = tc::mldb_timeline_buffer();
   const dim3 grid(p.items < c->sm_count ? p.items : c->sm_count);
+  if (g.res_split.hi) {
+    p.res_hi = g.res_split.hi; p.res_lo = g.res_split.lo(); p.ld_res = g.res_split.cols;
+    p.out_f32 = g.out_f32; p.ldc = g.ldc;
+    launch_pdl(k_proj_res_tc, grid, dim3(MMA_THREADS), ProjCfg::SMEM_BYTES, st, mAh, mAl, mWh, mWl, p);
+    return true;
+  }
+  p.out_hi = g.out.hi; p.out_lo = g.out.lo(); p.ld_out = g.out.cols; p.out_col0 = g.out_col0;
   switch (g.act) {
     case ACT_GELU: launch_pdl(k_proj_tc<ACT_GELU>, grid, dim3(MMA_THREADS), ProjCfg::SMEM_BYTES, st, mAh, mAl, mWh, mWl, p); break;
     case ACT_QUICKGELU: launch_pdl(k_proj_tc<ACT_QUICKGELU>, grid, dim3(MMA_THREADS), ProjCfg::SMEM_BYTES, st, mAh, mAl, mWh, mWl, p); break;
@@ -943,6 +1068,7 @@
 }
 
 bool tc_gemm(TcCtx* c, const GemmArgs& g, const LnArgs* ln, cudaStream_t st) {
+  if (!ln && g.res_split.hi) return tc_proj(c, g, st);
   const int bn = ln ? 256 : pick_bn(g);
   const bool fast = !ln && g.out.hi && !g.out_f32 && !g.addtab && !g.zero_lengths && g.in_group >= g.M &&
                     g.out_group == 0 && g.out_off == 0 && g.w.N % bn == 0 && g.w.bias != nullptr &&
@@ -1016,13 +1142,20 @@
   return planes_aligned16(go.a1) && planes_aligned16(l1.res);
 }
 
-static bool launch_ffn(TcCtx* c, const GemmArgs* go, const LnArgs* l1, const GemmArgs& g1, const GemmArgs& g2,
-                       const LnArgs& l2, float* scratch, int* flags, cudaStream_t st) {
+bool tc_ffn_ln1_supported(const TcCtx* c, const float* z, const LnArgs& l1, const GemmArgs& g1, const GemmArgs& g2,
+                          const LnArgs& l2) {
+  if (!tc_ffn_supported(c, g1, g2, l2)) return false;
+  return z && ((uintptr_t)z & 15) == 0 && l1.d == 256 && l1.gamma && l1.beta;
+}
+
+static bool launch_ffn(TcCtx* c, const GemmArgs* go, const LnArgs* l1, const float* z, const GemmArgs& g1,
+                       const GemmArgs& g2, const LnArgs& l2, float* scratch, int* flags, cudaStream_t st) {
   CUtensorMap mXh, mXl, mW1h, mW1l, mW2h, mW2l, mAh, mAl, mWoh, mWol, mYh, mYl;
   const int M = g1.M, m_tiles = (M + BM - 1) / BM;
   const ActBuf x = go ? l1->res : g1.a1;
-  bool ok = make_map(&mXh, x.hi, M, 256, BM) && make_map(&mXl, x.lo(), M, 256, BM) &&
-            make_map(&mW1h, g1.w.w, g1.w.N, g1.w.K, FfnCfg::CHUNK) &&
+  bool ok = z ? make_f32_map(&mXh, z, M, 256, BM) : make_map(&mXh, x.hi, M, 256, BM) && make_map(&mXl, x.lo(), M, 256, BM);
+  if (z) mXl = mXh;
+  ok = ok && make_map(&mW1h, g1.w.w, g1.w.N, g1.w.K, FfnCfg::CHUNK) &&
             make_map(&mW1l, g1.w.w + g1.w.plane_stride, g1.w.N, g1.w.K, FfnCfg::CHUNK) &&
             make_map(&mW2h, g2.w.w, g2.w.N, g2.w.K, 256) &&
             make_map(&mW2l, g2.w.w + g2.w.plane_stride, g2.w.N, g2.w.K, 256) &&
@@ -1038,7 +1171,8 @@
   p.M = M; p.m_tiles = m_tiles; p.n_chunks = g1.w.N / FfnCfg::CHUNK;
   p.tl = tc::mldb_timeline_buffer();
   p.prefix = go ? 1 : 0;
-  if (go) { p.inv_s0 = go->w.inv_scale; p.b0 = go->w.bias; p.gamma1 = l1->gamma; p.beta1 = l1->beta; }
+  if (go) { p.inv_s0 = go->w.inv_scale; p.b0 = go->w.bias; }
+  if (go || z) { p.gamma1 = l1->gamma; p.beta1 = l1->beta; }
   p.inv_s1 = g1.w.inv_scale; p.inv_s2 = g2.w.inv_scale;
   p.b1 = g1.w.bias; p.b2 = g2.w.bias; p.gamma = l2.gamma; p.beta = l2.beta;
   const int ncta_max = c->sm_count;
@@ -1050,14 +1184,18 @@
   }
   const int ncta = p.full > 0 ? ncta_max : p.left * p.parts;
   p.reverse = tc::snake_order();
-  launch_pdl(k_ffn_tc, dim3(ncta), dim3(MMA_THREADS), FfnCfg::SMEM_BYTES, st, mXh, mXl, mW1h, mW1l, mW2h, mW2l, mAh,
+  launch_pdl(z ? k_ffn_ln1_tc : k_ffn_tc, dim3(ncta), dim3(MMA_THREADS), FfnCfg::SMEM_BYTES, st, mXh, mXl, mW1h, mW1l, mW2h, mW2l, mAh,
              mAl, mWoh, mWol, mYh, mYl, p);
   return true;
 }
 bool tc_ffn(TcCtx* c, const GemmArgs& g1, const GemmArgs& g2, const LnArgs& l2, float* scratch, int* flags, cudaStream_t st) {
-  return launch_ffn(c, nullptr, nullptr, g1, g2, l2, scratch, flags, st);
+  return launch_ffn(c, nullptr, nullptr, nullptr, g1, g2, l2, scratch, flags, st);
+}
+bool tc_ffn_ln1(TcCtx* c, const float* z, const LnArgs& l1, const GemmArgs& g1, const GemmArgs& g2, const LnArgs& l2,
+                float* scratch, int* flags, cudaStream_t st) {
+  return launch_ffn(c, nullptr, &l1, z, g1, g2, l2, scratch, flags, st);
 }
 bool tc_tail(TcCtx* c, const GemmArgs& go, const LnArgs& l1, const GemmArgs& g1, const GemmArgs& g2, const LnArgs& l2,
              float* scratch, int* flags, cudaStream_t st) {
-  return launch_ffn(c, &go, &l1, g1, g2, l2, scratch, flags, st);
-}
+  return launch_ffn(c, &go, &l1, nullptr, g1, g2, l2, scratch, flags, st);
+}
diff --git a/mld_b200/csrc/gemm_tc.h b/mld_b200/csrc/gemm_tc.h
--- a/mld_b200/csrc/gemm_tc.h
+++ b/mld_b200/csrc/gemm_tc.h
@@ -14,5 +14,9 @@
                        const LnArgs& l2);
 bool tc_tail(TcCtx* c, const GemmArgs& go, const LnArgs& l1, const GemmArgs& g1, const GemmArgs& g2, const LnArgs& l2,
              float* scratch, int* flags, cudaStream_t st);
+bool tc_ffn_ln1_supported(const TcCtx* c, const float* z, const LnArgs& l1, const GemmArgs& g1, const GemmArgs& g2,
+                          const LnArgs& l2);
+bool tc_ffn_ln1(TcCtx* c, const float* z, const LnArgs& l1, const GemmArgs& g1, const GemmArgs& g2, const LnArgs& l2,
+                float* scratch, int* flags, cudaStream_t st);
 int tc_set_ffn_split(TcCtx* c, int on);
 int tc_set_ffn_fused(TcCtx* c, int on);
diff --git a/mld_b200/csrc/ops.cuh b/mld_b200/csrc/ops.cuh
--- a/mld_b200/csrc/ops.cuh
+++ b/mld_b200/csrc/ops.cuh
@@ -27,6 +27,7 @@
   const float* addtab = nullptr;
   const int32_t* zero_lengths = nullptr;
   const float* res_f32 = nullptr;
+  ActBuf res_split{};
   int wide_n = 0;
   int vec_f32 = 0;
 };
diff --git a/mld_b200/csrc/stack.cu b/mld_b200/csrc/stack.cu
--- a/mld_b200/csrc/stack.cu
+++ b/mld_b200/csrc/stack.cu
@@ -6,6 +6,11 @@
   if (h->use_tc && tc_gemm_supported(h->tc, g)) {
     if (!tc_gemm(h->tc, g, nullptr, st)) h->op_failed = true;
     kcount(h, MLDB_KSTAT_GEMM_TC);
+    return;
+  }
+  if (g.res_split.hi) {
+    mldb_set_err("GEMM with a split16 residual: no kernel for this shape");
+    h->op_failed = true;
     return;
   }
   simt_gemm(g, st);
@@ -114,22 +119,35 @@
   op_gemm_ln(h, g2, l2, cf32, st);
 }
 void op_tail(mldb_handle* h, const LinW& wo, const LnW& n1, const LinW& l1, const LinW& l2, const LnW& n2, ActBuf att,
-             ActBuf x, ActBuf x1, ActBuf hbuf, ActBuf xout, int M, int d, int ff, float* cf32, cudaStream_t st, int fuse) {
+             ActBuf x, ActBuf x1, ActBuf hbuf, ActBuf xout, int M, int d, int ff, float* cf32, cudaStream_t st, int fuse,
+             int part) {
   GemmArgs go; go.a1 = att; go.K1 = d; go.M = M; go.w = wo;
   LnArgs ln1; ln1.res = x; ln1.gamma = n1.g; ln1.beta = n1.b; ln1.M = M; ln1.d = d; ln1.out = x1;
   GemmArgs g1; g1.a1 = x1; g1.K1 = d; g1.M = M; g1.w = l1; g1.act = ACT_GELU; g1.out = hbuf;
   GemmArgs g2; g2.a1 = hbuf; g2.K1 = ff; g2.M = M; g2.w = l2;
   LnArgs ln2; ln2.res = x1; ln2.gamma = n2.g; ln2.beta = n2.b; ln2.M = M; ln2.d = d; ln2.out = xout;
-  constexpr int FUSE_MAX_TILES = 2;
-  const bool small = (M + 127) / 128 <= FUSE_MAX_TILES;
-  if (fuse && (fuse == 2 || small) && h->use_tc && tc_tail_supported(h->tc, go, ln1, g1, g2, ln2)) {
+  constexpr int FUSE_MAX_TILES = 2, SPLIT_MIN_TILES = 11;
+  const int tiles = (M + 127) / 128;
+  const bool small = tiles <= FUSE_MAX_TILES;
+  if (part == TAIL_ALL && fuse && (fuse == 2 || small) && h->use_tc && tc_tail_supported(h->tc, go, ln1, g1, g2, ln2)) {
     const int k = ffn_scratch_slot(h, st);
     if (!tc_tail(h->tc, go, ln1, g1, g2, ln2, h->ffn_scratch[k], h->ffn_flags[k], st)) h->op_failed = true;
     kcount(h, MLDB_KSTAT_FFN_TC);
     return;
   }
-  op_gemm_ln(h, go, ln1, cf32, st);
-  op_ffn(h, g1, g2, ln2, cf32, st);
+  GemmArgs gz = go; gz.res_split = x; gz.out_f32 = cf32; gz.ldc = d;
+  if ((fuse == 0 || tiles >= SPLIT_MIN_TILES) && h->use_tc && tc_gemm_supported(h->tc, gz) &&
+      tc_ffn_ln1_supported(h->tc, cf32, ln1, g1, g2, ln2)) {
+    if (part != TAIL_FFN) op_gemm(h, gz, st);
+    if (part != TAIL_OUTPROJ) {
+      const int k = ffn_scratch_slot(h, st);
+      if (!tc_ffn_ln1(h->tc, cf32, ln1, g1, g2, ln2, h->ffn_scratch[k], h->ffn_flags[k], st)) h->op_failed = true;
+      kcount(h, MLDB_KSTAT_FFN_TC);
+    }
+    return;
+  }
+  if (part != TAIL_FFN) op_gemm_ln(h, go, ln1, cf32, st);
+  if (part != TAIL_OUTPROJ) op_ffn(h, g1, g2, ln2, cf32, st);
 }
 void rows_to_split(mldb_handle* h, ActBuf X, const float* src, int ld_src, int M, int d, int in_group, int out_group,
                    int out_off, int src_bcast, const float* tab, int relu, cudaStream_t st) {
diff --git a/mld_b200/csrc/tc_common.cuh b/mld_b200/csrc/tc_common.cuh
--- a/mld_b200/csrc/tc_common.cuh
+++ b/mld_b200/csrc/tc_common.cuh
@@ -324,19 +324,21 @@
   return fn;
 }
 
-inline bool encode_plane_map(CUtensorMap* m, const __half* base, int rank, const cuuint64_t* dims,
-                             const cuuint64_t* strides, const cuuint32_t* box, const cuuint32_t* estr = nullptr) {
+inline bool encode_plane_map(CUtensorMap* m, const void* base, int rank, const cuuint64_t* dims,
+                             const cuuint64_t* strides, const cuuint32_t* box, const cuuint32_t* estr = nullptr,
+                             bool f32 = false) {
   const PFN_tmapEncodeTiled encode = tmap_encoder();
   if (!encode) return false;
   const cuuint32_t ones[5] = {1, 1, 1, 1, 1};
-  const CUresult r = encode(m, CU_TENSOR_MAP_DATA_TYPE_FLOAT16, (cuuint32_t)rank, (void*)base, dims, strides, box,
-                            estr ? estr : ones, CU_TENSOR_MAP_INTERLEAVE_NONE, CU_TENSOR_MAP_SWIZZLE_128B,
+  const CUresult r = encode(m, f32 ? CU_TENSOR_MAP_DATA_TYPE_FLOAT32 : CU_TENSOR_MAP_DATA_TYPE_FLOAT16,
+                            (cuuint32_t)rank, (void*)base, dims, strides, box, estr ? estr : ones,
+                            CU_TENSOR_MAP_INTERLEAVE_NONE, CU_TENSOR_MAP_SWIZZLE_128B,
                             CU_TENSOR_MAP_L2_PROMOTION_L2_256B, CU_TENSOR_MAP_FLOAT_OOB_FILL_NONE);
   if (r != CUDA_SUCCESS) {
     std::string shape;
     for (int i = rank - 1; i >= 0; --i) shape += std::to_string(dims[i]) + (i ? " x " : "");
     char buf[96];
-    snprintf(buf, sizeof buf, "(CUresult %d): fp16 plane at %p", (int)r, (const void*)base);
+    snprintf(buf, sizeof buf, "(CUresult %d): %s at %p", (int)r, f32 ? "fp32 matrix" : "fp16 plane", base);
     mldb_set_err("cuTensorMapEncodeTiled failed " + std::string(buf) + ", [" + shape + "], box " +
                  std::to_string(box[1]) + " rows");
   }
@@ -348,6 +350,12 @@
   const cuuint32_t box[2] = {64u, (cuuint32_t)box_rows};
   return encode_plane_map(m, base, 2, dims, strides, box);
 }
+inline bool make_f32_map(CUtensorMap* m, const float* base, int rows, int cols, int box_rows) {
+  const cuuint64_t dims[2] = {(cuuint64_t)cols, (cuuint64_t)rows};
+  const cuuint64_t strides[1] = {(cuuint64_t)cols * sizeof(float)};
+  const cuuint32_t box[2] = {32u, (cuuint32_t)box_rows};
+  return encode_plane_map(m, base, 2, dims, strides, box, nullptr, true);
+}
 inline bool make_seq_map(CUtensorMap* m, const __half* base, int nseq, int L, int cols, int box_rows) {
   const cuuint64_t dims[3] = {(cuuint64_t)cols, (cuuint64_t)L, (cuuint64_t)nseq};
   const cuuint64_t strides[2] = {(cuuint64_t)cols * sizeof(__half), (cuuint64_t)L * cols * sizeof(__half)};
```
